# Tamnemng/TAM-GCN

Measured on AMD Instinct MI355X. Metric: skeleton clips/sec (fwd+CE+bwd+grad all-reduce+SGD step), N-UCLA 20-joint x 64-frame, higher is better.
Workload: dtype f32 (exact fp32-input MFMA v_mfma_f32_16x16x4_f32 in every GEMM, forward and backward: the reference's arithmetic); 1 GPU; N-UCLA joint stream, 256 clips/GPU x (3,64,20,1), models.ctrgcn.Model fwd+CE+bwd+grad-allreduce+SGD step, train-mode BN; global_batch=256, streams=1, parallelism=dp1, launch=hipgraph, model_streams=0, rehearsal=False, allreduce=one flat bucket after backward

## Files before the change

include/tamgcn.h:

```cpp
#ifndef TAMGCN_H
#define TAMGCN_H

#ifdef __cplusplus
extern "C" {
#endif

#define TAMGCN_VERSION 401
#define TAMGCN_MAX_SUBSETS 3
#define TAMGCN_MAX_V 32

typedef struct tamgcn_src {
    const float* x1;
    const float* x2;
    const float* coef;
    int ctot;
    int coff;
    int act;
} tamgcn_src;

int         tamgcn_version(void);
const char* tamgcn_last_error(void);
const char* tamgcn_last_kernel(void);
int         tamgcn_get_split_mode(void);
int         tamgcn_set_split_mode(int mode);

int         tamgcn_ctrgc_lds_bytes(int S, int V, int R);

typedef struct tamgcn_conv_desc {
    tamgcn_src src;
    int N, K, T_in, V;
    const float* w;
    const float* bias;
    int M, KT, dil, stride, pad;
    int wmode;
    int up;
    float* y;
    int yctot, ycoff;
    int T_out;
    int T_y;
    int ostride;
    const float* add1;
    const float* add2;
    const float* bcast;
    float bcast_scale;
    const tamgcn_src* mask;
    const float* aux;
    const float* aux_center;
    int auxctot, auxcoff;
    float* stats_part;
    int stats_ctot, stats_coff;
    const float* post_coef;
    int post_ctot, post_act;
} tamgcn_conv_desc;

int tamgcn_conv_nparts(const tamgcn_conv_desc* d);
int tamgcn_conv(const tamgcn_conv_desc* d, void* stream);

typedef struct tamgcn_wgrad_desc {
    tamgcn_src gy;
    tamgcn_src src;
    int N, M, K, T_in, T_out, V, KT, dil, stride, pad;
    float* part;
    int nsplit;
} tamgcn_wgrad_desc;
int tamgcn_wgrad_max_split(const tamgcn_wgrad_desc* d);
int tamgcn_wgrad(const tamgcn_wgrad_desc* d, void* stream);

typedef struct tamgcn_conv_pair_desc {
    int N, T, V;
    int stride;
    tamgcn_src src;
    int K, M0, M1;
    const float* w0; const float* w1;
    const float* bias0; const float* bias1;
    float* y0; int yctot0, ycoff0;
    float* y1; int yctot1, ycoff1;
    float* stats_part0; int stats_ctot0, stats_coff0;
    float* stats_part1; int stats_ctot1, stats_coff1;
} tamgcn_conv_pair_desc;
int tamgcn_conv_pair(const tamgcn_conv_pair_desc* d, void* stream);

typedef struct tamgcn_wgrad_pair_desc {
    tamgcn_src gy0, gy1, src;
    int N, M0, M1, K, T, V;
    int stride;
    float* part;
    int nsplit;
} tamgcn_wgrad_pair_desc;
int tamgcn_wgrad_pair(const tamgcn_wgrad_pair_desc* d, void* stream);

typedef struct tamgcn_reduce_desc {
    const float* part; float* out;
    int nsplit, accumulate;
    long long stride_s, count;
    float scale;
} tamgcn_reduce_desc;
int tamgcn_reduce_multi(const tamgcn_reduce_desc* descs, int n, void* stream);

int tamgcn_reduce_sum(float* part, int nsplit, long long stride_s, long long count,
                      float scale, int accumulate, float* out, void* stream);

int tamgcn_bn_fwd_finalize(const float* part, int part_ctot, int part_coff, int nparts, double count,
                           const float* gamma, const float* beta,
                           float* running_mean, float* running_var, long long* num_batches_tracked,
                           float momentum, float eps, int training,
                           float* coef, float* save, int coef_ctot, int coef_coff, int C, void* stream);

int tamgcn_coef_diff(const float* coef_d, const float* coef_y, float* out, int C, int mode, void* stream);

int tamgcn_bn_bwd_finalize(const float* part, int part_ctot, int part_coff, int nparts, double count,
// ... 17 lines not shown

int tamgcn_tmean(const tamgcn_src* src, int N, int C, int T, int V, float* xbar, void* stream);

typedef struct tamgcn_ctrgc_desc {
    int N, Cin, Cout, S, R, T, V;
    tamgcn_src x;
    const float* pq;
    const float* w3;
    const float* b3;
    const float* w4;
    const float* b4;
    const float* A;
    const float* alpha;
    const float* E;
} tamgcn_ctrgc_desc;

int tamgcn_ctrgc_build_e(const tamgcn_ctrgc_desc* d, float* E, void* stream);

int tamgcn_ctrgc_fwd(const tamgcn_ctrgc_desc* d, float* y, float* stats_part, float* x3_out, void* stream);

int tamgcn_ctrgc_bwd_dx3(const tamgcn_ctrgc_desc* d, const tamgcn_src* dy,
                         float* dx3, float* db3_part, void* stream);

int tamgcn_ctrgc_bwd_de_acc(const tamgcn_ctrgc_desc* d, const tamgcn_src* dy, const float* x3,
                            float* dE, void* stream);
int tamgcn_ctrgc_bwd_de_tail(const tamgcn_ctrgc_desc* d, const float* dE,
                             float* dA_part, float* dw4_part, float* db4_part,
                             float* dalpha_part, float* dpq, int groups, void* stream);

int tamgcn_ctrgc_tiled_supported(int V);
int tamgcn_ctrgc_tiled_chunks(int V);
int tamgcn_ctrgc_tiled_build_e(const tamgcn_ctrgc_desc* d, float* E, void* stream);
int tamgcn_ctrgc_tiled_agg_fwd(const tamgcn_ctrgc_desc* d, const float* x3, const float* E, float* y, float* stats_part, void* stream);
int tamgcn_ctrgc_tiled_agg_bwd(const tamgcn_ctrgc_desc* d, const tamgcn_src* dy, const float* E, float* dx3, float* db3_part, void* stream);
int tamgcn_ctrgc_tiled_de_acc(const tamgcn_ctrgc_desc* d, const tamgcn_src* dy, const float* x3, float* dE, void* stream);
int tamgcn_ctrgc_tiled_de_tail(const tamgcn_ctrgc_desc* d, const float* dE, float* dA_part, float* dw4_part, float* db4_part,
                               float* dalpha_part, float* dpq, void* stream);

int tamgcn_vgen_supported(int V);
int tamgcn_vgen_lds_bytes(int S, int V, int R);
int tamgcn_vgen_build_e(const tamgcn_ctrgc_desc* d, float* E, void* stream);
int tamgcn_vgen_agg_fwd(const tamgcn_ctrgc_desc* d, const float* x3, const float* E, float* y, float* stats_part, void* stream);
int tamgcn_vgen_agg_bwd(const tamgcn_ctrgc_desc* d, const tamgcn_src* dy, const float* E, float* dx3, float* db3_part, void* stream);
int tamgcn_vgen_de_acc(const tamgcn_ctrgc_desc* d, const tamgcn_src* dy, const float* x3, float* dE, void* stream);
int tamgcn_vgen_de_tail(const tamgcn_ctrgc_desc* d, const float* dE, float* dA_part, float* dw4_part, float* db4_part,
                        float* dalpha_part, float* dpq, int groups, void* stream);

int tamgcn_ew_nparts(int N, int C, int T, int V);

int tamgcn_gcn_tail_fwd(const tamgcn_src* y, const tamgcn_src* o, const tamgcn_src* res,
                        int N, int C, int T, int V, float* g, void* stream);
int tamgcn_gcn_tail_bwd(const float* dg, const float* g, const tamgcn_src* o, const float* o_save,
                        int N, int C, int T, int V, float* dsum, float* doz, float* part, void* stream);
int tamgcn_gcn_mid_bwd(const float* dsum, const float* ddiff, const float* y_pre, const float* y_save,
                       const float* r_pre, const float* r_save,
                       int N, int C, int T, int V, float* dyb, float* dres, float* part, void* stream);

#define TAMGCN_TCONV_MAXB 6
typedef struct tamgcn_tconv_desc {
    tamgcn_src src;
    int N, T_in, T_out, V, Cb, nb, KT, stride, pool;
    int dil[TAMGCN_TCONV_MAXB];
    const float* w[TAMGCN_TCONV_MAXB];
    const float* bias[TAMGCN_TCONV_MAXB];
    float* y; int yctot, ycoff;
    float* stats_part; int stats_ctot;
    const tamgcn_src* mask; const float* center;
} tamgcn_tconv_desc;
int tamgcn_tconv_supported(int V, int Cb, int KT, int nb, const int* dil, int stride, int T_in);
int tamgcn_tconv_nparts(const tamgcn_tconv_desc* d, int backward);
int tamgcn_tconv_fwd(const tamgcn_tconv_desc* d, void* stream);
int tamgcn_tconv_bwd(const tamgcn_tconv_desc* d, void* stream);
int tamgcn_tconv_wgrad_max_split(const tamgcn_tconv_desc* d);
int tamgcn_tconv_wgrad(const tamgcn_tconv_desc* d, void* stream);

int tamgcn_maxpool_fwd(const tamgcn_src* src, int N, int C, int T_in, int V, int stride,
                       float* y, int yctot, int ycoff, int T_out, float* stats_part, void* stream);
int tamgcn_maxpool_post_fwd(const tamgcn_src* src, int N, int C, int T_in, int V, int stride,
                            float* y, int yctot, int ycoff, int T_out, const float* coef, const float* add, int relu, void* stream);
int tamgcn_maxpool_bwd(const tamgcn_src* gy, const tamgcn_src* src, const float* src_save, int N, int C, int T_in, int T_out, int V,
                       int stride, float* d, int dctot, int dcoff, float* part, void* stream);

int tamgcn_add_act_fwd(const tamgcn_src* a, const tamgcn_src* res, int relu,
                       int N, int C, int T, int V, float* out, float* rowmean, float* xbar, void* stream);
int tamgcn_add_act_bwd(const float* dout, const float* out, int relu, const float* a_pre, const float* a_save,
                       const float* r_pre, const float* r_save,
                       int N, int C, int T, int V, float* dz, float* part, void* stream);

int tamgcn_apply(const tamgcn_src* src, int N, int C, int T, int V, float* y, int yctot, int ycoff, void* stream);

int tamgcn_stem_stats(const float* x, const float* dout, const float* center, int N, int C, int T, int V, int M,
                      float* part, void* stream);
int tamgcn_stem_apply(const float* x, const float* dout, const float* coef, int N, int C, int T, int V, int M,
                      float* out, void* stream);
int tamgcn_head_pool_fwd(const float* x, int N, int C, int T, int V, int M, float* pooled, void* stream);
int tamgcn_head_pool_bwd(const float* dpooled, int N, int C, int T, int V, int M, float* dx, void* stream);
int tamgcn_head_fc_fwd(const float* pooled, const float* W, const float* b, int N, int C, int K, float* logits, void* stream);
int tamgcn_head_fc_bwd(const float* dlogits, const float* pooled, const float* W, int N, int C, int K,
                       float* dW, float* db, float* dpooled, void* stream);

int tamgcn_ce_fwd(const float* logits, const long long* labels, int N, int K, float* loss, float* g, void* stream);
int tamgcn_ce_bwd(const float* g, const float* dloss, int N, int K, float* dlogits, void* stream);

int tamgcn_score_fuse(const float* scores, const float* weights, int S, int N, int K, int softmax,
                      const long long* labels, float* fused, long long* pred, int* class_stats, void* stream);

#define TAMGCN_EVAL_MAX_TOPK 4
#define TAMGCN_SWEEP_MAX_ALPHAS 16
int tamgcn_eval_accumulate(const float* logits, const long long* labels, const long long* index, int B, int K,
                           int valid, const int* valid_dev, const int* topk, int nk, long long base, long long num_samples,
                           long long* counts, double* sums, int* confusion, float* scores, void* stream);
int tamgcn_score_sweep(const float* a, const float* b, const float* alphas, int A, int N, int K, int softmax,
                       const long long* labels, int* correct, void* stream);

int tamgcn_stream_derive(const float* x, int N, int C, int T, int V, int M, const int* parent, int mode, float* out, void* stream);
int tamgcn_feeder_transform(const double* raw, const long long* offsets, const double* rot, const int* idx, const int* parent,
                            int N, int V, int time_steps, int center_joint, int mode, float* out, void* stream);

int tamgcn_feeder_draw(const long long* offsets, long long n_clips, const long long* clip_ids, int B, const long long* labels,
                       long long* state, const double* cossin, int time_steps, int train, double* view, double* rot, int* idx,
                       long long* labels_out, void* stream);
int tamgcn_feeder_transform_indexed(const double* raw, const long long* offsets, long long n_clips, const long long* clip_ids,
                                    const double* rot, const int* idx, const int* parent, int B, int V, int time_steps,
                                    int center_joint, int mode, float* out, void* stream);

typedef struct tamgcn_f2_gcn_desc {
    int N, Cin, Cout, T, V, S, R, res_mode;
    const float* x;
    const float* w12; const float* b12;
    const float* w4; const float* b4;
    const float* A; const float* alpha;
    const float* w3; const float* b3;
    const float* sy; const float* ty;
    const float* wd; const float* bd;
    float* E;
    float* sum; float* diff;
    const float* xpart;
} tamgcn_f2_gcn_desc;
int tamgcn_f2_e(const tamgcn_f2_gcn_desc* d, void* stream);
int tamgcn_f2_gcn(const tamgcn_f2_gcn_desc* d, void* stream);
// ... 101 lines not shown
```

tam_gcn_amd/_lib.py:

```python
import ctypes as C
import os

_HERE = os.path.dirname(os.path.abspath(__file__))
LIB_PATH = os.path.join(_HERE, 'libtamgcn.so')

c_float_p = C.c_void_p


class Src(C.Structure):
    _fields_ = [('x1', C.c_void_p), ('x2', C.c_void_p), ('coef', C.c_void_p),
                ('ctot', C.c_int), ('coff', C.c_int), ('act', C.c_int)]


class ConvDesc(C.Structure):
    _fields_ = [('src', Src),
                ('N', C.c_int), ('K', C.c_int), ('T_in', C.c_int), ('V', C.c_int),
                ('w', C.c_void_p), ('bias', C.c_void_p),
                ('M', C.c_int), ('KT', C.c_int), ('dil', C.c_int), ('stride', C.c_int), ('pad', C.c_int),
                ('wmode', C.c_int), ('up', C.c_int),
                ('y', C.c_void_p), ('yctot', C.c_int), ('ycoff', C.c_int),
                ('T_out', C.c_int), ('T_y', C.c_int), ('ostride', C.c_int),
                ('add1', C.c_void_p), ('add2', C.c_void_p), ('bcast', C.c_void_p), ('bcast_scale', C.c_float),
                ('mask', C.POINTER(Src)),
                ('aux', C.c_void_p), ('aux_center', C.c_void_p), ('auxctot', C.c_int), ('auxcoff', C.c_int),
# ... 79 lines not shown
class F2TcnDesc(C.Structure):
    _fields_ = [(k, C.c_int) for k in ('N', 'Cin', 'Cout', 'T', 'V', 'stride', 'Cb', 'nb', 'ks', 'res_mode')] + \
               [('dil', C.c_int * 4), ('h', C.c_void_p), ('wt', C.c_void_p * 4), ('bt', C.c_void_p * 4)] + \
               [(k, C.c_void_p) for k in ('sp', 'tp', 'x', 'wr', 'br', 'out', 'xpart')]


class F2sGcnDesc(C.Structure):
    _fields_ = [(k, C.c_int) for k in ('N', 'Cin', 'Cout', 'T', 'V', 'K')] + \
               [(k, C.c_void_p) for k in ('x', 'Ae', 'wg', 'bg', 'h')]


class F2sTcnDesc(C.Structure):
    _fields_ = [(k, C.c_int) for k in ('N', 'Cin', 'Cout', 'T', 'V', 'KT', 'stride', 'res_mode')] + \
               [(k, C.c_void_p) for k in ('h', 'wt', 'bt', 'x', 'wr', 'br', 'out')]


class F2sTcnBwdDesc(C.Structure):
    _fields_ = [(k, C.c_int) for k in ('N', 'Cout', 'T', 'V', 'KT', 'stride')] + \
               [(k, C.c_void_p) for k in ('gout', 'out', 'h', 'wtb', 'dh')]


class F2sGcnBwdDesc(C.Structure):
    _fields_ = [(k, C.c_int) for k in ('N', 'Cin', 'Cout', 'T', 'V', 'K', 'stride', 'res_mode')] + \
               [(k, C.c_void_p) for k in ('dh', 'Ae', 'wgb', 'gout', 'out', 'wrb', 'dx')]


class OptimDesc(C.Structure):
    _fields_ = [('n', C.c_longlong),
                ('p', C.c_void_p), ('g', C.c_void_p), ('s0', C.c_void_p), ('s1', C.c_void_p),
                ('lr', C.c_void_p), ('step', C.c_void_p), ('scal', C.c_void_p),
                ('mode', C.c_int), ('nesterov', C.c_int),
                ('momentum', C.c_float), ('dampening', C.c_float), ('weight_decay', C.c_float), ('eps', C.c_float),
                ('beta1', C.c_double), ('beta2', C.c_double)]


class GradGuard(C.Structure):
    _fields_ = [('max_norm', C.c_float), ('skip_nonfinite', C.c_int), ('partial', C.c_void_p), ('n_partial', C.c_int),
                ('stat', C.c_void_p), ('skipped', C.c_void_p)]


_i, _p, _d, _f, _ll = C.c_int, C.c_void_p, C.c_double, C.c_float, C.c_longlong
_SP = C.POINTER(Src)
SIGNATURES = {
    'tamgcn_version': (_i, []),
    'tamgcn_last_error': (C.c_char_p, []),
    'tamgcn_last_kernel': (C.c_char_p, []),
    'tamgcn_ctrgc_lds_bytes': (_i, [_i, _i, _i]),
    'tamgcn_get_split_mode': (_i, []),
    'tamgcn_set_split_mode': (_i, [_i]),
    'tamgcn_conv_nparts': (_i, [C.POINTER(ConvDesc)]),
    'tamgcn_conv': (_i, [C.POINTER(ConvDesc), _p]),
    'tamgcn_wgrad_max_split': (_i, [C.POINTER(WgradDesc)]),
    'tamgcn_wgrad': (_i, [C.POINTER(WgradDesc), _p]),
    'tamgcn_conv_pair': (_i, [C.POINTER(ConvPairDesc), _p]),
    'tamgcn_wgrad_pair': (_i, [C.POINTER(WgradPairDesc), _p]),
    'tamgcn_stem_stats': (_i, [_p, _p, _p, _i, _i, _i, _i, _i, _p, _p]),
    'tamgcn_stem_apply': (_i, [_p, _p, _p, _i, _i, _i, _i, _i, _p, _p]),
    'tamgcn_head_pool_fwd': (_i, [_p, _i, _i, _i, _i, _i, _p, _p]),
    'tamgcn_head_pool_bwd': (_i, [_p, _i, _i, _i, _i, _i, _p, _p]),
    'tamgcn_head_fc_fwd': (_i, [_p, _p, _p, _i, _i, _i, _p, _p]),
    'tamgcn_head_fc_bwd': (_i, [_p, _p, _p, _i, _i, _i, _p, _p, _p, _p]),
    'tamgcn_reduce_multi': (_i, [C.POINTER(ReduceDesc), _i, _p]),
    'tamgcn_reduce_sum': (_i, [_p, _i, _ll, _ll, _f, _i, _p, _p]),
    'tamgcn_bn_fwd_finalize': (_i, [_p, _i, _i, _i, _d, _p, _p, _p, _p, _p, _f, _f, _i, _p, _p, _i, _i, _i, _p]),
    'tamgcn_bn_bwd_finalize': (_i, [_p, _i, _i, _i, _d, _p, _p, _i, _i, _i, _p, _p, _p, _p, _i, _i, _i, _p]),
    'tamgcn_bn_fwd_finalize_multi': (_i, [C.POINTER(BnFwdDesc), _i, _p]),
    'tamgcn_coef_diff': (_i, [_p, _p, _p, _i, _i, _p]),
    'tamgcn_bn_bwd_finalize_multi': (_i, [C.POINTER(BnBwdDesc), _i, _p]),
    'tamgcn_tmean': (_i, [_SP, _i, _i, _i, _i, _p, _p]),
    'tamgcn_ctrgc_build_e': (_i, [C.POINTER(CtrgcDesc), _p, _p]),
    'tamgcn_ctrgc_fwd': (_i, [C.POINTER(CtrgcDesc), _p, _p, _p, _p]),
    'tamgcn_ctrgc_bwd_dx3': (_i, [C.POINTER(CtrgcDesc), _SP, _p, _p, _p]),
    'tamgcn_ctrgc_bwd_de_acc': (_i, [C.POINTER(CtrgcDesc), _SP, _p, _p, _p]),
    'tamgcn_ctrgc_bwd_de_tail': (_i, [C.POINTER(CtrgcDesc), _p, _p, _p, _p, _p, _p, _i, _p]),
    'tamgcn_ctrgc_tiled_supported': (_i, [_i]),
    'tamgcn_ctrgc_tiled_chunks': (_i, [_i]),
    'tamgcn_ctrgc_tiled_build_e': (_i, [C.POINTER(CtrgcDesc), _p, _p]),
    'tamgcn_ctrgc_tiled_agg_fwd': (_i, [C.POINTER(CtrgcDesc), _p, _p, _p, _p, _p]),
    'tamgcn_ctrgc_tiled_agg_bwd': (_i, [C.POINTER(CtrgcDesc), _SP, _p, _p, _p, _p]),
    'tamgcn_ctrgc_tiled_de_acc': (_i, [C.POINTER(CtrgcDesc), _SP, _p, _p, _p]),
    'tamgcn_ctrgc_tiled_de_tail': (_i, [C.POINTER(CtrgcDesc), _p, _p, _p, _p, _p, _p, _p]),
    'tamgcn_vgen_supported': (_i, [_i]),
    'tamgcn_vgen_lds_bytes': (_i, [_i, _i, _i]),
    'tamgcn_vgen_build_e': (_i, [C.POINTER(CtrgcDesc), _p, _p]),
    'tamgcn_vgen_agg_fwd': (_i, [C.POINTER(CtrgcDesc), _p, _p, _p, _p, _p]),
    'tamgcn_vgen_agg_bwd': (_i, [C.POINTER(CtrgcDesc), _SP, _p, _p, _p, _p]),
    'tamgcn_vgen_de_acc': (_i, [C.POINTER(CtrgcDesc), _SP, _p, _p, _p]),
    'tamgcn_vgen_de_tail': (_i, [C.POINTER(CtrgcDesc), _p, _p, _p, _p, _p, _p, _i, _p]),
    'tamgcn_ew_nparts': (_i, [_i, _i, _i, _i]),
    'tamgcn_gcn_tail_fwd': (_i, [_SP, _SP, _SP, _i, _i, _i, _i, _p, _p]),
    'tamgcn_gcn_tail_bwd': (_i, [_p, _p, _SP, _p, _i, _i, _i, _i, _p, _p, _p, _p]),
    'tamgcn_gcn_mid_bwd': (_i, [_p, _p, _p, _p, _p, _p, _i, _i, _i, _i, _p, _p, _p, _p]),
    'tamgcn_tconv_supported': (_i, [_i, _i, _i, _i, C.POINTER(C.c_int), _i, _i]),
    'tamgcn_tconv_nparts': (_i, [C.POINTER(TconvDesc), _i]),
    'tamgcn_tconv_fwd': (_i, [C.POINTER(TconvDesc), _p]),
    'tamgcn_tconv_bwd': (_i, [C.POINTER(TconvDesc), _p]),
    'tamgcn_tconv_wgrad_max_split': (_i, [C.POINTER(TconvDesc)]),
    'tamgcn_tconv_wgrad': (_i, [C.POINTER(TconvDesc), _p]),
    'tamgcn_maxpool_fwd': (_i, [_SP, _i, _i, _i, _i, _i, _p, _i, _i, _i, _p, _p]),
    'tamgcn_maxpool_post_fwd': (_i, [_SP, _i, _i, _i, _i, _i, _p, _i, _i, _i, _p, _p, _i, _p]),
    'tamgcn_maxpool_bwd': (_i, [_SP, _SP, _p, _i, _i, _i, _i, _i, _i, _p, _i, _i, _p, _p]),
    'tamgcn_add_act_fwd': (_i, [_SP, _SP, _i, _i, _i, _i, _i, _p, _p, _p, _p]),
    'tamgcn_add_act_bwd': (_i, [_p, _p, _i, _p, _p, _p, _p, _i, _i, _i, _i, _p, _p, _p]),
    'tamgcn_apply': (_i, [_SP, _i, _i, _i, _i, _p, _i, _i, _p]),
    'tamgcn_score_fuse': (_i, [_p, _p, _i, _i, _i, _i, _p, _p, _p, _p, _p]),
    'tamgcn_ce_fwd': (_i, [_p, _p, _i, _i, _p, _p, _p]),
    'tamgcn_ce_bwd': (_i, [_p, _p, _i, _i, _p, _p]),
    'tamgcn_eval_accumulate': (_i, [_p, _p, _p, _i, _i, _i, _p, C.POINTER(C.c_int), _i, _ll, _ll, _p, _p, _p, _p, _p]),
    'tamgcn_score_sweep': (_i, [_p, _p, C.POINTER(C.c_float), _i, _i, _i, _i, _p, _p, _p]),
    'tamgcn_stream_derive': (_i, [_p, _i, _i, _i, _i, _i, _p, _i, _p, _p]),
    'tamgcn_feeder_transform': (_i, [_p, _p, _p, _p, _p, _i, _i, _i, _i, _i, _p, _p]),
    'tamgcn_feeder_draw': (_i, [_p, _ll, _p, _i, _p, _p, _p, _i, _i, _p, _p, _p, _p, _p]),
    'tamgcn_feeder_transform_indexed': (_i, [_p, _p, _ll, _p, _p, _p, _p, _i, _i, _i, _i, _i, _p, _p]),
    'tamgcn_f2_e': (_i, [C.POINTER(F2GcnDesc), _p]),
    'tamgcn_f2_gcn': (_i, [C.POINTER(F2GcnDesc), _p]),
    'tamgcn_f2_gemm': (_i, [C.POINTER(F2GemmDesc), _p]),
    'tamgcn_f2_tcn': (_i, [C.POINTER(F2TcnDesc), _p]),
    'tamgcn_f2v_e': (_i, [C.POINTER(F2GcnDesc), _p]),
    'tamgcn_f2v_gcn': (_i, [C.POINTER(F2GcnDesc), _p]),
    'tamgcn_f2v_gemm': (_i, [C.POINTER(F2GemmDesc), _p]),
    'tamgcn_f2v_tcn': (_i, [C.POINTER(F2TcnDesc), _p]),
    'tamgcn_f2_e_grouped': (_i, [C.POINTER(F2GcnDesc), _i, _p]),
    'tamgcn_f2_gcn_grouped': (_i, [C.POINTER(F2GcnDesc), _i, _p]),
    'tamgcn_f2_gemm_grouped': (_i, [C.POINTER(F2GemmDesc), _i, _p]),
    'tamgcn_f2_tcn_grouped': (_i, [C.POINTER(F2TcnDesc), _i, _p]),
    'tamgcn_f2v_e_grouped': (_i, [C.POINTER(F2GcnDesc), _i, _p]),
    'tamgcn_f2v_gcn_grouped': (_i, [C.POINTER(F2GcnDesc), _i, _p]),
    'tamgcn_f2v_gemm_grouped': (_i, [C.POINTER(F2GemmDesc), _i, _p]),
    'tamgcn_f2v_tcn_grouped': (_i, [C.POINTER(F2TcnDesc), _i, _p]),
    'tamgcn_f2s_supported': (_i, [_i, _i, _i, _i, _i, _i]),
    'tamgcn_f2s_gcn': (_i, [C.POINTER(F2sGcnDesc), _p]),
    'tamgcn_f2s_tcn': (_i, [C.POINTER(F2sTcnDesc), _p]),
    'tamgcn_f2s_tcn_bwd': (_i, [C.POINTER(F2sTcnBwdDesc), _p]),
    'tamgcn_f2s_gcn_bwd': (_i, [C.POINTER(F2sGcnBwdDesc), _p]),
    'tamgcn_saliency_joints': (_i, [_p, _p, _i, _i, _i, _i, _i, _p, _p, _p]),
    'tamgcn_saliency_accumulate': (_i, [_p, _p, _i, _i, _p, _p, _i, _i, _i, _p, _p, _p]),
    'tamgcn_stem_streams_eval': (_i, [_p, _p, _p, _p, _i, _i, _i, _i, _i, _i, _p, _p]),
    'tamgcn_head_fc_grouped': (_i, [_p, _p, _p, _i, _i, _i, _i, _p, _p]),
    'tamgcn_optim_step': (_i, [C.POINTER(OptimDesc), _p]),
    'tamgcn_optim_step_guarded': (_i, [C.POINTER(OptimDesc), C.POINTER(GradGuard), _p]),
}


class TamgcnLibraryError(RuntimeError):
    pass


_lib = None
ABI_VERSION = 401


def load():
    global _lib
    if _lib is not None:
        return _lib
    import torch
# ... 27 lines not shown
```

tam_gcn_amd/csrc/conv.hip:

```cpp
#include "common.h"

namespace {

constexpr int BM = 64;
constexpr int BK = 16;
constexpr int BKP = BK + 1;
constexpr int MAXCW = 5;
constexpr int MAXCOLS = 320;

TG_TRACE_DEFINE(tamgcn_trace_read)

struct ConvArgs {
    SrcDev src;
    int N, K, T_in, V;
    const float* w; const float* bias;
    int M, KT, dil, stride, pad;
    long long ws_m, ws_k, ws_t, w_off;
    int up, wmode;
    float* y; int yctot, ycoff, T_out, T_y, ostride;
    const float* add1; const float* add2; const float* bcast; float bcast_scale;
    SrcDev mask; int has_mask;
    const float* aux; const float* aux_center; int auxctot, auxcoff;
    float* stats_part; int stats_ctot, stats_coff, nparts;
    const float* post_coef; int post_ctot, post_act;
    int BT;
    int CW;
    int TIN;
    int lstride;
    int sB;
    int LB;
    int pitchB;
    int Vs, Vp, nsl;
};

struct PairArgs {
    int M0;
    const float* w1; const float* bias1;
    float* y1; int yctot1, ycoff1;
    float* stats1; int sctot1, scoff1;
};

__device__ __forceinline__ void conv_epilogue(const ConvArgs& a, f32x4 (&acc)[4][MAXCW], float* Ss, int n, int m0, int t0,
                                              int ncols, int cw0, int mt_act, int c_act, const int (&tl)[MAXCW],
                                              const int (&vv)[MAXCW], int j, int kq, int wave, int tid) {
    const int V = a.V;
    float s1[4][4], s2[4][4];
#pragma unroll
    for (int mt = 0; mt < 4; ++mt)
#pragma unroll
        for (int r = 0; r < 4; ++r) { s1[mt][r] = 0.f; s2[mt][r] = 0.f; }
#pragma unroll
    for (int mt = 0; mt < 4; ++mt) {
        if (mt >= mt_act) continue;
#pragma unroll
        for (int c = 0; c < MAXCW; ++c) {
            if (c >= c_act) continue;
            int col = (cw0 + c) * 16 + j;
            if (col >= ncols) continue;
            int t = (t0 + tl[c]) * a.ostride;
#pragma unroll
            for (int r = 0; r < 4; ++r) {
                int m = m0 + mt * 16 + kq * 4 + r;
                if (m >= a.M) continue;
                float val = acc[mt][c][r];
                if (a.bias) val += a.bias[m];
                if (a.post_coef) val = fmaf(a.post_coef[a.ycoff + m], val, a.post_coef[2 * a.post_ctot + a.ycoff + m]);
                long long idx = (((long long)n * a.yctot + a.ycoff + m) * a.T_y + t) * V + vv[c];
                if (a.bcast) val = fmaf(a.bcast[((long long)m * a.N + n) * V + vv[c]], a.bcast_scale, val);
                if (a.add1) val += a.add1[idx];
                if (a.add2) val += a.add2[idx];
                if (a.post_act == 1) val = fmaxf(val, 0.f);
                if (a.has_mask) {
                    int mch = a.mask.coff + m;
                    long long midx = (((long long)n * a.mask.ctot + mch) * a.T_y + t) * V + vv[c];
                    if (!(src_value(a.mask, midx, mch) > 0.f)) val = 0.f;
                }
                acc[mt][c][r] = val;
                if (a.stats_part) {
                    float x2 = val;
                    if (a.aux) x2 = a.aux[(((long long)n * a.auxctot + a.auxcoff + m) * a.T_y + t) * V + vv[c]] - a.aux_center[a.auxcoff + m];
                    s1[mt][r] += val;
                    s2[mt][r] = fmaf(val, x2, s2[mt][r]);
                }
            }
        }
    }
#pragma unroll
    for (int mt = 0; mt < 4; ++mt) {
        if (mt >= mt_act) continue;
#pragma unroll
        for (int c = 0; c < MAXCW; ++c) {
            if (c >= c_act) continue;
            int col = (cw0 + c) * 16 + j;
// ... 76 lines not shown
            int kk = e & (BK - 1);
            int i = (e >> 4) & (BM - 1);
            int tap = e >> 10;
            int m = m0 + i, k = k0 + kk;
            float wv = 0.f;
            if (m < a.M && k < a.K) wv = a.w[m * a.ws_m + k * a.ws_k + tap * a.ws_t + a.w_off];
            As[(tap * BM + i) * BKP + kk] = wv;
        }
        for (int pos = tid; pos < a.LB; pos += NTHREADS) {
            int slot = pos / V;
            int v = pos - slot * V;
            int th = tin0 + slot * a.lstride;
            bool ok = th >= 0;
            if (a.up > 1) { ok = ok && (th % a.up == 0); th /= a.up; }
            ok = ok && th < a.T_in;
            long long goff = src_n + (long long)th * V + v;
#pragma unroll 4
            for (int kk = 0; kk < BK; ++kk) {
                int k = k0 + kk;
                float xv = 0.f;
                if (ok && k < a.K) {
                    int ch = a.src.coff + k;
                    xv = src_value(a.src, goff + ch * chan_stride, ch);
                }
                Bs[kk * a.pitchB + pos] = xv;
            }
        }
        __syncthreads();
        for (int tap = 0; tap < a.KT; ++tap) {
            const int tapoff = tap * a.dil * V;
#pragma unroll
            for (int k4 = 0; k4 < BK / 4; ++k4) {
                float av[4];
#pragma unroll
                for (int mt = 0; mt < 4; ++mt)
                    av[mt] = As[(tap * BM + mt * 16 + j) * BKP + k4 * 4 + kq];
                const float* brow = Bs + (k4 * 4 + kq) * a.pitchB + tapoff;
#pragma unroll
                for (int c = 0; c < MAXCW; ++c) {
                    if (c < c_act) {
                        float bv = brow[boff[c]];
#pragma unroll
                        for (int mt = 0; mt < 4; ++mt)
                            if (mt < mt_act) acc[mt][c] = mfma16(av[mt], bv, acc[mt][c]);
                    }
                }
            }
        }
    }

    conv_epilogue(a, acc, Ss, n, m0, t0, ncols, cw0, mt_act, c_act, tl, vv, j, kq, wave, tid);
}

template <int NTH, bool PR = false>
__device__ __forceinline__ void staged_rows(const ConvArgs& a, const float* Tt, int PT, int RP, int r0, int BMT, int m0, int n, int t0,
                                            int ncols, float* Ss, int Vs, int v0, const PairArgs* pa = nullptr) {
    const int tid = threadIdx.x, V = a.V;
    const int TPR = NTH / RP;
    const int row = tid / TPR, seg = tid - row * TPR;
    const int m = m0 + r0 + row;
    const bool flat = Vs == V && a.ostride == 1;
    const bool vecok = flat || (Vs & 3) == 0;
    float p1 = 0.f, p2 = 0.f;
    const bool rowok = r0 + row < BMT && m < a.M;
    if (rowok) {
        float bia = a.bias ? a.bias[m] : 0.f;
        float* yp = a.y;
        const float ctr = a.aux ? a.aux_center[a.auxcoff + m] : 0.f;
        const float pc1 = a.post_coef ? a.post_coef[a.ycoff + m] : 1.f, pc0 = a.post_coef ? a.post_coef[2 * a.post_ctot + a.ycoff + m] : 0.f;
        const float plo = a.post_act == 1 ? 0.f : -__builtin_inff();
        long long ybase = ((long long)n * a.yctot + a.ycoff + m) * a.T_y * V;
        if constexpr (PR) {
            if (m >= pa->M0) {
                const int m1 = m - pa->M0;
                bia = pa->bias1 ? pa->bias1[m1] : 0.f; yp = pa->y1;
                ybase = ((long long)n * pa->yctot1 + pa->ycoff1 + m1) * a.T_y * V;
            }
        }
        const long long mbase = a.has_mask ? ((long long)n * a.mask.ctot + a.mask.coff + m) * a.T_y * V : 0;
        const long long abase = a.aux ? ((long long)n * a.auxctot + a.auxcoff + m) * a.T_y * V : 0;
        const float* bc = a.bcast ? a.bcast + ((long long)m * a.N + n) * V : nullptr;
        float mc1 = 1.f, mc2 = 0.f, mc0 = 0.f;
        if (a.has_mask && a.mask.coef) {
            int mch = a.mask.coff + m;
            mc1 = a.mask.coef[mch]; mc0 = a.mask.coef[2 * a.mask.ctot + mch];
            if (a.mask.x2) mc2 = a.mask.coef[a.mask.ctot + mch];
        }
        const int nc4 = (ncols + 3) >> 2;
        for (int c4 = seg; c4 < nc4; c4 += TPR) {
            const int col = c4 << 2;
            const int fr = col / Vs, v = col - fr * Vs;
            if ((vecok || v + 4 <= Vs) && col + 4 <= ncols) {
                const long long off = (long long)(t0 + fr) * a.ostride * V + v0 + v;
                float4 val = *reinterpret_cast<const float4*>(Tt + row * PT + col);
                val.x = fmaf(pc1, val.x + bia, pc0); val.y = fmaf(pc1, val.y + bia, pc0);
                val.z = fmaf(pc1, val.z + bia, pc0); val.w = fmaf(pc1, val.w + bia, pc0);
                if (bc) {
                    float4 b;
                    if ((V & 3) == 0) b = *reinterpret_cast<const float4*>(bc + v0 + v);
                    else { const int j0 = (v0 + v) % V; b = make_float4(bc[j0], bc[(j0 + 1) % V], bc[(j0 + 2) % V], bc[(j0 + 3) % V]); }
                    val.x = fmaf(b.x, a.bcast_scale, val.x); val.y = fmaf(b.y, a.bcast_scale, val.y);
                    val.z = fmaf(b.z, a.bcast_scale, val.z); val.w = fmaf(b.w, a.bcast_scale, val.w);
                }
                if (a.add1) { float4 t = *reinterpret_cast<const float4*>(a.add1 + ybase + off); val.x += t.x; val.y += t.y; val.z += t.z; val.w += t.w; }
                if (a.add2) { float4 t = *reinterpret_cast<const float4*>(a.add2 + ybase + off); val.x += t.x; val.y += t.y; val.z += t.z; val.w += t.w; }
                val.x = fmaxf(val.x, plo); val.y = fmaxf(val.y, plo); val.z = fmaxf(val.z, plo); val.w = fmaxf(val.w, plo);
                if (a.has_mask) {
                    float4 q = *reinterpret_cast<const float4*>(a.mask.x1 + mbase + off);
                    float4 q2 = make_float4(0.f, 0.f, 0.f, 0.f);
                    if (a.mask.x2) q2 = *reinterpret_cast<const float4*>(a.mask.x2 + mbase + off);
                    if (!(fmaf(mc1, q.x, fmaf(mc2, q2.x, mc0)) > 0.f)) val.x = 0.f;
                    if (!(fmaf(mc1, q.y, fmaf(mc2, q2.y, mc0)) > 0.f)) val.y = 0.f;
                    if (!(fmaf(mc1, q.z, fmaf(mc2, q2.z, mc0)) > 0.f)) val.z = 0.f;
                    if (!(fmaf(mc1, q.w, fmaf(mc2, q2.w, mc0)) > 0.f)) val.w = 0.f;
                }
                if (a.stats_part) {
                    float4 x2 = val;
                    if (a.aux) {
                        x2 = *reinterpret_cast<const float4*>(a.aux + abase + off);
                        x2.x -= ctr; x2.y -= ctr; x2.z -= ctr; x2.w -= ctr;
                    }
                    p1 += (val.x + val.y) + (val.z + val.w);
                    p2 = fmaf(val.x, x2.x, fmaf(val.y, x2.y, fmaf(val.z, x2.z, fmaf(val.w, x2.w, p2))));
                }
                *reinterpret_cast<float4*>(yp + ybase + off) = val;
            } else {
                for (int i = 0; i < 4 && col + i < ncols; ++i) {
                    const int ci = col + i, fi = ci / Vs, vi = ci - fi * Vs;
                    const long long off = (long long)(t0 + fi) * a.ostride * V + v0 + vi;
                    float val = fmaf(pc1, Tt[row * PT + ci] + bia, pc0);
                    if (bc) val = fmaf(bc[(v0 + vi) % V], a.bcast_scale, val);
                    if (a.add1) val += a.add1[ybase + off];
                    if (a.add2) val += a.add2[ybase + off];
                    val = fmaxf(val, plo);
                    if (a.has_mask) {
                        const float q = a.mask.x1[mbase + off], q2 = a.mask.x2 ? a.mask.x2[mbase + off] : 0.f;
                        if (!(fmaf(mc1, q, fmaf(mc2, q2, mc0)) > 0.f)) val = 0.f;
                    }
                    if (a.stats_part) {
                        const float x2 = a.aux ? a.aux[abase + off] - ctr : val;
                        p1 += val;
                        p2 = fmaf(val, x2, p2);
                    }
                    yp[ybase + off] = val;
                }
            }
        }
    }
    if (a.stats_part) {
        for (int o = 1; o < TPR; o <<= 1) { p1 += __shfl_xor(p1, o); p2 += __shfl_xor(p2, o); }
        if (seg == 0 && rowok) { Ss[r0 + row] = p1; Ss[4 * BM + r0 + row] = p2; }
    }
}

template <int BKV, int MT, int CWT>
__global__ __launch_bounds__(NTHREADS) void conv_kernel_vec(const ConvArgs a) {
    extern __shared__ __attribute__((aligned(16))) float smem[];
    constexpr int BKVP = BKV + 2;
    constexpr int BMT = MT * 16;
    constexpr int NPF = (BKV == 32) ? 10 : 8;
    float* As = smem;
    float* Bs = As + ((a.KT * BMT * BKVP + 3) & ~3);
    float* Ss = Bs + BKV * a.pitchB;
    float* cf = Ss + 2 * 4 * BM;

    const int tid = threadIdx.x, lane = tid & 63, wave = tid >> 6;
    const int j = lane & 15, kq = lane >> 4;
    const int tti = blockIdx.x / a.nsl, sl = blockIdx.x - tti * a.nsl;
    const int n = blockIdx.z, m0 = blockIdx.y * BMT, t0 = tti * a.BT;
    const int V = a.V, Vs = a.Vs, Vp = a.Vp, v0 = sl * Vs;
    const int bt = min(a.BT, a.T_out - t0);
    const int ncols = bt * Vs;
    const int cw0 = wave * CWT;

    for (int e = tid; e < a.K; e += NTHREADS) {
        int ch = a.src.coff + e;
        cf[e] = a.src.coef ? a.src.coef[ch] : 1.f;
        cf[a.K + e] = (a.src.coef && a.src.x2) ? a.src.coef[a.src.ctot + ch] : 0.f;
        cf[2 * a.K + e] = a.src.coef ? a.src.coef[2 * a.src.ctot + ch] : 0.f;
    }

    int boff[CWT], tl[CWT], vv[CWT];
#pragma unroll
    for (int c = 0; c < CWT; ++c) {
        int col = (cw0 + c) * 16 + j;
        if (col < ncols) { tl[c] = col / Vs; vv[c] = col - tl[c] * Vs; boff[c] = tl[c] * a.sB * Vp + vv[c]; }
        else { tl[c] = 0; vv[c] = 0; boff[c] = 0; }
    }
    f32x4 acc[MT][CWT];
#pragma unroll
    for (int mt = 0; mt < MT; ++mt)
// ... 134 lines not shown
            }
        }
        TG_T(tf); TG_ACC(6, tf - te);
    }
    TG_T(tg0);

    __syncthreads();
    float* Tt = smem;
    constexpr int PT = CWT * 64 + 4;
    const int avail = ((a.KT * BMT * BKVP + 3) & ~3) + BKV * a.pitchB;
    int RP = (avail / PT) & ~15;
    if (RP > BMT) RP = BMT;
    if (RP == 48) RP = 32;
    if (a.stats_part) {
        for (int e = tid; e < 2 * 4 * BM; e += NTHREADS) Ss[e] = 0.f;
    }
    for (int r0 = 0; r0 < BMT; r0 += RP) {
        __syncthreads();
#pragma unroll
        for (int mt = 0; mt < MT; ++mt) {
            const int rl = mt * 16 + kq * 4 - r0;
            if (rl >= 0 && rl < RP) {
#pragma unroll
                for (int c = 0; c < CWT; ++c) {
                    const int col = (cw0 + c) * 16 + j;
#pragma unroll
                    for (int r = 0; r < 4; ++r) Tt[(rl + r) * PT + col] = acc[mt][c][r];
                }
            }
        }
        __syncthreads();
        staged_rows<NTHREADS>(a, Tt, PT, RP, r0, BMT, m0, n, t0, ncols, Ss, Vs, v0);
    }
    if (a.stats_part) {
        __syncthreads();
        if (tid < 2 * BMT) {
            int st = tid / BMT, row = tid - st * BMT;
            int m = m0 + row;
            if (m < a.M) {
                int part = n * gridDim.x + blockIdx.x;
                a.stats_part[((long long)st * a.stats_ctot + a.stats_coff + m) * a.nparts + part] = Ss[st * 4 * BM + row];
            }
        }
    }
}



#ifndef TG_KO
#define TG_KO 0
#endif
constexpr int G_NT = 512, G_BMT = 64, G_PA = 80, G_PBMAX = 320, G_NST = 3, G_CWT = 5;

template <int NSRC, int BK, bool PRO, int NW, int PAIR = 0>
__global__ __launch_bounds__(NW * 64, NW == 8 ? 4 : 2) void conv1x1_glds_kernel(const ConvArgs a, int ntt, int nmt, const PairArgs pa) {
    constexpr int G_NT = NW * 64, G_MT = 16 / NW;
    extern __shared__ __attribute__((aligned(16))) float smem[];
    constexpr int STG = BK * G_PBMAX * NSRC + BK * G_PA;
    constexpr int NAI = BK / NW;
    constexpr int MAXB = (NSRC * (BK / 4) * 5 + NW - 1) / NW;
    float* cf = smem + G_NST * STG;
    float* Ss = cf + (PRO ? 3 * a.K : 0);

    const int tid = threadIdx.x, lane = tid & 63, wave = tid >> 6;
    const int j = lane & 15, kq = lane >> 4, wm = wave >> 2, wn = wave & 3;
    const int V = a.V, K = a.K, LB = a.LB;
    const int rot = ((LB & 31) + 16) & 31;
    int g, mtile;
    {
        const int L = blockIdx.x, ng = a.N * ntt;
        if ((ng & 7) == 0) { const int xcd = L & 7, i = L >> 3; mtile = i % nmt; g = (i / nmt) * 8 + xcd; }
        else { g = L / nmt; mtile = L - g * nmt; }
    }
    const int n = g / ntt, tt = g - n * ntt;
    const int m0 = mtile * G_BMT, t0 = tt * a.BT;
    const int bt = min(a.BT, a.T_out - t0);
    const int ncols = bt * V;
    const long long TV = (long long)a.T_in * V;

    const int NQ = (LB + 63) >> 6;
    const int ls = a.lstride;
    const float rV_ = 1.0f / (float)V;
    const int NI1 = (BK / 4) * NQ;
    int b_rel[MAXB], b_dst[MAXB];
    bool b_ok[MAXB], b_on[MAXB];
    int nissue = 0;
#pragma unroll
    for (int i = 0; i < MAXB; ++i) {
        const int id = wave + i * NW;
        const bool idok = id < NSRC * NI1;
        const int src = idok ? id / NI1 : 0;
        const int rem = id - src * NI1;
        const int grp = rem / NQ, q = rem - grp * NQ;
        const int f = q * 256 + lane * 4;
        const int r = f / LB, off = f - r * LB;
        int col = off + (r & 1) * rot;
        if (col >= LB) col -= LB;
        b_ok[i] = idok && r < 4 && col < ncols;
        const int scol = ls > 1 ? col + tg_rcp_div(col, rV_) * (ls - 1) * V : col;
        b_rel[i] = (int)((grp * 4 + r) * TV) + scol + src * 0x40000000;
        b_dst[i] = src * (BK * G_PBMAX) + grp * 4 * LB + q * 256;
        b_on[i] = __ballot(b_ok[i]) != 0ull;
        nissue += b_on[i] ? 1 : 0;
    }
    const float* xb1 = a.src.x1 + ((long long)n * a.src.ctot + a.src.coff) * TV + (long long)t0 * ls * V;
    const float* xb2 = NSRC == 2 ? a.src.x2 + ((long long)n * a.src.ctot + a.src.coff) * TV + (long long)t0 * ls * V : nullptr;
    constexpr int RPP = 256 / BK;
    constexpr int NAP0 = G_BMT / RPP;
// ... 169 lines not shown
        for (int s_ = 0; s_ + 1 < NK; ++s_) {
            rd((s_ & 1) ^ 1, stg, k0, s_ + 1);
            mm(s_ & 1);
            fin((s_ & 1) ^ 1);
        }
        tg_wait_vmcnt<15>(c + 2 < nch ? nissue : 0);
        asm volatile("s_waitcnt lgkmcnt(0)\n\ts_barrier" ::: "memory");
        if (c + 3 < nch) issue(c + 3);
        stg = stg == G_NST - 1 ? 0 : stg + 1;
        rd(NK & 1, stg, k0 + BK, 0);
        mm((NK - 1) & 1);
        fin(NK & 1);
    }
    {
        const int k0 = (nch - 1) * BK;
#pragma unroll
        for (int s_ = 0; s_ < NK; ++s_) {
            if (s_ + 1 < NK) rd((s_ & 1) ^ 1, stg, k0, s_ + 1);
            mm(s_ & 1);
            if (s_ + 1 < NK) fin((s_ & 1) ^ 1);
        }
    }
    TG_T(tg0);

#if TG_KO & 1
    {
        float ssum = 0.f;
        for (int mt = 0; mt < G_MT; ++mt)
            for (int c = 0; c < G_CWT; ++c) ssum += acc[mt][c][0] + acc[mt][c][1] + acc[mt][c][2] + acc[mt][c][3];
        if (ssum == 123.456f) a.y[tid] = ssum;
        return;
    }
#endif
    constexpr int PT = G_CWT * 64 + 4, RP = 32;
    float* Tt = smem;
    if (a.stats_part) {
        for (int e = tid; e < 2 * 4 * BM; e += G_NT) Ss[e] = 0.f;
    }
    for (int r0 = 0; r0 < G_BMT; r0 += RP) {
        __syncthreads();
#pragma unroll
        for (int mt = 0; mt < G_MT; ++mt) {
            const int rl = wm * (G_MT * 16) + mt * 16 - r0;
            if (rl >= 0 && rl < RP) {
#pragma unroll
                for (int c = 0; c < G_CWT; ++c) {
                    const int col = (wn * G_CWT + c) * 16 + j;
#pragma unroll
                    for (int r = 0; r < 4; ++r) Tt[(rl + kq * 4 + r) * PT + col] = acc[mt][c][r];
                }
            }
        }
        __syncthreads();
        staged_rows<G_NT, PAIR == 1>(a, Tt, PT, RP, r0, G_BMT, m0, n, t0, ncols, Ss, V, 0, &pa);
    }
    if (a.stats_part) {
        __syncthreads();
        if (tid < 2 * G_BMT) {
            int stt = tid / G_BMT, row = tid - stt * G_BMT;
            int m = m0 + row;
            if (PAIR == 1 && m < a.M && m >= pa.M0) pa.stats1[((long long)stt * pa.sctot1 + pa.scoff1 + m - pa.M0) * a.nparts + g] = Ss[stt * 4 * BM + row];
            else if (m < a.M) a.stats_part[((long long)stt * a.stats_ctot + a.stats_coff + m) * a.nparts + g] = Ss[stt * 4 * BM + row];
        }
    }
    TG_T(tg1); TG_ACC(7, tg1 - tg0); TG_ACC(8, tg1 - tt0); TG_ACC(9, 1);
}


constexpr int GS_BK = 32, GS_NST = 2;

template <int TERMS, bool WM0, int MT>
__global__ __launch_bounds__(G_NT) void conv1x1_glds_split_kernel(const ConvArgs a, int ntt, int nmt) {
    constexpr int GS_MT = MT, GS_BMT = 32 * MT, WROWS = 16 * MT;
    extern __shared__ __attribute__((aligned(16))) float smem[];
    constexpr int BK = GS_BK;
    constexpr int STG = BK * G_PBMAX + BK * GS_BMT;
    constexpr int MAXB = ((BK / 4) * 5 + 7) / 8;
    constexpr int NAP = BK * GS_BMT / 256 / 8;
    constexpr int QR = GS_BMT / 4, RPP = 64 / QR;
    float* cf = smem + GS_NST * STG;
    float* Ss = cf + 3 * a.K;
    float* Bc = Ss + 2 * 4 * BM;

    TG_T(tt0);
    const int tid = threadIdx.x, lane = tid & 63, wave = tid >> 6;
    const int j = lane & 15, kq = lane >> 4, wm = wave >> 2, wn = wave & 3;
    const int V = a.V, K = a.K, LB = a.LB;
    const int rot = ((LB & 31) + 16) & 31;
    int g, mtile;
    {
        const int L = blockIdx.x, ng = a.N * ntt;
        if ((ng & 7) == 0) { const int xcd = L & 7, i = L >> 3; mtile = i % nmt; g = (i / nmt) * 8 + xcd; }
        else { g = L / nmt; mtile = L - g * nmt; }
    }
    const int n = g / ntt, tt = g - n * ntt;
    const int m0 = mtile * GS_BMT, t0 = tt * a.BT;
    const int bt = min(a.BT, a.T_out - t0);
    const int ncols = bt * V;
    const long long TV = (long long)a.T_in * V;

    for (int e = tid; e < K; e += G_NT) {
        int ch = a.src.coff + e;
        cf[e] = a.src.coef ? a.src.coef[ch] : 1.f;
        cf[K + e] = (a.src.coef && a.src.x2) ? a.src.coef[a.src.ctot + ch] : 0.f;
        cf[2 * K + e] = a.src.coef ? a.src.coef[2 * a.src.ctot + ch] : 0.f;
    }
    const bool plain = !a.src.coef;
    const int nsrc = a.src.x2 ? 2 : 1;

    const int NQ = (LB + 63) >> 6, NI1 = (BK / 4) * NQ;
    int b_rel[MAXB], b_dst[MAXB];
    bool b_ok[MAXB], b_on[MAXB];
    int nissue = 0;
#pragma unroll
    for (int i = 0; i < MAXB; ++i) {
// ... 191 lines not shown
    const int q = 4 / gcd_i(V, 4);
    if (p->flat && q > 1 && BT >= q) BT -= BT % q;
    for (;;) {
        p->BT = BT;
        p->lstride = (d->KT == 1) ? d->stride : 1;
        p->sB = (d->KT == 1) ? 1 : d->stride;
        p->TIN = (d->KT == 1) ? BT : (BT - 1) * d->stride + (d->KT - 1) * d->dil + 1;
        p->LB = p->TIN * p->Vp;
        int pitch = p->LB;
        pitch += ((16 - (pitch & 31)) + 32) & 31;
        p->pitchB = pitch;
        p->CW = ceil_div(ceil_div(BT * p->Vs, 16), 4);
        p->vec = false; p->bk = BK;
        bool slots_short = false;
        if (vec_try && (p->LB & 3) == 0) {
            int lb4 = p->LB / 4;
            int bk = (d->KT == 1 && 32 * lb4 <= 10 * NTHREADS) ? 32 : 16;
            if (bk * lb4 <= ((bk == 32) ? 10 : 8) * NTHREADS) { p->vec = true; p->bk = bk; }
            else slots_short = true;
        }
        p->mt = d->M <= 16 ? 1 : d->M <= 32 ? 2 : (d->M % 64 == 0 ? 4 : (d->M % 48 == 0 ? 3 : 4));
        if (d->KT > 1 && p->mt == 4) p->mt = 2;
        p->cwt = p->CW <= 3 ? 3 : 5;
        if (p->vec) {
            size_t avail = (((size_t)d->KT * p->mt * 16 * (p->bk + 2) + 3) & ~(size_t)3) + (size_t)p->bk * pitch;
            if (avail < (size_t)16 * (p->cwt * 64 + 4)) p->vec = false;
        }
        p->lds = p->vec ? sizeof(float) * ((((size_t)d->KT * p->mt * 16 * (p->bk + 2) + 3) & ~(size_t)3) + (size_t)p->bk * pitch +
                                           2 * 4 * BM + 3 * (size_t)d->K)
                        : sizeof(float) * ((size_t)d->KT * BM * (BK + 1) + (size_t)BK * pitch + 2 * 4 * BM);
        if (slots_short && BT > 1) { BT = BT > 4 ? BT - 2 : BT - 1; if (p->flat && q > 1 && BT >= q) BT -= BT % q; continue; }
        if (p->lds <= 64 * 1024 || BT == 1) break;
        BT = (BT + 1) / 2;
        if (p->flat && q > 1 && BT >= q) BT -= BT % q;
    }
    if (!p->vec) { p->Vs = V; p->nsl = 1; if (p->Vp != V) {
        p->Vp = V; p->LB = p->TIN * V; int pitch = p->LB; pitch += ((16 - (pitch & 31)) + 32) & 31; p->pitchB = pitch;
        p->CW = ceil_div(ceil_div(p->BT * V, 16), 4);
        p->lds = sizeof(float) * ((size_t)d->KT * BM * (BK + 1) + (size_t)BK * pitch + 2 * 4 * BM); } }
    if (p->lds > 160 * 1024 || p->CW > MAXCW) return -1;
    p->ntt = ceil_div(d->T_out, p->BT);
    return 0;
}

}


extern "C" int tamgcn_conv_nparts(const tamgcn_conv_desc* d) {
    ConvPlan p;
    if (!d || plan_conv(d, &p)) return -1;
    return d->N * p.ntt * p.nsl;
}

extern "C" int tamgcn_conv(const tamgcn_conv_desc* d, void* stream) {
    TG_CHECK(d && d->src.x1 && d->w && d->y, "tamgcn_conv: null pointer");
    TG_CHECK(d->N > 0 && d->K > 0 && d->M > 0 && d->T_in > 0 && d->T_out > 0 && d->V > 0,
             "tamgcn_conv: bad dims N=%d K=%d M=%d T_in=%d T_out=%d V=%d", d->N, d->K, d->M, d->T_in, d->T_out, d->V);
    TG_CHECK(d->KT >= 1 && d->KT <= 9 && d->dil >= 1 && d->stride >= 1 && d->up >= 1 && d->ostride >= 1,
             "tamgcn_conv: bad taps KT=%d dil=%d stride=%d up=%d", d->KT, d->dil, d->stride, d->up);
    TG_CHECK(d->src.coff + d->K <= d->src.ctot && d->ycoff + d->M <= d->yctot, "tamgcn_conv: channel slice out of range");
    TG_CHECK((d->T_out - 1) * d->ostride < d->T_y, "tamgcn_conv: T_out*ostride exceeds T_y");
    TG_CHECK(!(d->N > 65535), "tamgcn_conv: N too large for grid.z");
    TG_CHECK((long long)d->N * d->yctot * d->T_y * d->V < (1LL << 32), "tamgcn_conv: output tensor exceeds 2^32 elements");
    ConvPlan p;
    TG_CHECK(plan_conv(d, &p) == 0, "tamgcn_conv: no tiling for V=%d KT=%d dil=%d stride=%d", d->V, d->KT, d->dil, d->stride);
    ConvArgs a;
    a.src = make_src(d->src);
    a.N = d->N; a.K = d->K; a.T_in = d->T_in; a.V = d->V;
    a.w = d->w; a.bias = d->bias; a.M = d->M; a.KT = d->KT; a.dil = d->dil; a.stride = d->stride; a.pad = d->pad;
    if (d->wmode == 0) { a.ws_m = (long long)d->K * d->KT; a.ws_k = d->KT; a.ws_t = 1; a.w_off = 0; }
    else { a.ws_m = d->KT; a.ws_k = (long long)d->M * d->KT; a.ws_t = -1; a.w_off = d->KT - 1; }
    a.up = d->up; a.wmode = d->wmode;
    a.y = d->y; a.yctot = d->yctot; a.ycoff = d->ycoff; a.T_out = d->T_out; a.T_y = d->T_y; a.ostride = d->ostride;
    a.add1 = d->add1; a.add2 = d->add2; a.bcast = d->bcast; a.bcast_scale = d->bcast_scale;
    a.has_mask = d->mask != nullptr; a.mask = d->mask ? make_src(*d->mask) : null_src();
    a.aux = d->aux; a.aux_center = d->aux_center; a.auxctot = d->auxctot; a.auxcoff = d->auxcoff;
    TG_CHECK(!d->aux || d->aux_center, "tamgcn_conv: aux needs aux_center");
    a.stats_part = d->stats_part; a.stats_ctot = d->stats_ctot; a.stats_coff = d->stats_coff;
    a.post_coef = d->post_coef; a.post_ctot = d->post_ctot; a.post_act = d->post_act;
    TG_CHECK(!d->post_coef || d->post_ctot >= d->ycoff + d->M, "tamgcn_conv: post_coef has %d channels, need %d", d->post_ctot, d->ycoff + d->M);
    a.nparts = d->N * p.ntt * p.nsl;
    a.BT = p.BT; a.CW = p.CW; a.TIN = p.TIN; a.lstride = p.lstride; a.sB = p.sB; a.LB = p.LB; a.pitchB = p.pitchB;
    a.Vs = p.Vs; a.Vp = p.Vp; a.nsl = p.nsl;
    dim3 grid(p.ntt, ceil_div(d->M, BM), d->N);
    const bool aligned16 = (((uintptr_t)d->src.x1 | (uintptr_t)(d->src.x2 ? d->src.x2 : d->src.x1) | (uintptr_t)d->w) & 15) == 0;
    const bool strided1x1 = d->KT == 1 && d->stride == 2 && d->up == 1 && d->pad == 0 && (d->V & 3) == 0 && d->T_out == (d->T_in - 1) / 2 + 1 &&
                            p.lstride == 2 && p.TIN == p.BT && p.nsl == 1 && p.Vp == d->V && !d->mask && !d->aux;
    const bool glds = p.vec && (p.flat || strided1x1) && d->K % 16 == 0 && p.LB >= 64 && p.LB <= G_PBMAX && (p.LB & 3) == 0 &&
                      aligned16 && (long long)d->K * d->T_in * d->V < (1LL << 30);
    const size_t lds_split = sizeof(float) * ((size_t)GS_NST * (GS_BK * G_PBMAX + GS_BK * 128) + 3 * (size_t)d->K + 2 * 4 * BM + 128);
    const bool big = glds && tamgcn_split_mode() >= 1 && d->src.act == 0 && d->M >= 128 && d->M % 4 == 0 && d->K % GS_BK == 0 &&
                     lds_split <= 160 * 1024 && !d->post_coef && d->wmode == 1 && !d->stats_part;
    if (big) {
        const int nmt = ceil_div(d->M, 128);
        const unsigned nblk = (unsigned)(d->N * p.ntt * nmt);
        tg_launch_lds<conv1x1_glds_split_kernel<2, false, 4>>(160 * 1024, dim3(nblk), dim3(G_NT), lds_split, (hipStream_t)stream, a, p.ntt, nmt);
        tamgcn_note_kernel("conv1x1_glds_split_kernel<2, false, 4>");
    } else if (glds) {
        const int nmt = ceil_div(d->M, G_BMT);
        const unsigned nblk = (unsigned)(d->N * p.ntt * nmt);
        static int nw_env = -1;
        if (nw_env < 0) { const char* e = getenv("TAMGCN_CONV_WAVES"); nw_env = e ? atoi(e) : 8; }
        const bool pro = d->src.coef || d->src.x2 || d->src.act;
#define TG_GLDS_CASE(NS_, BK_, PRO_, NW_)                                                                                 \
        {                                                                                                                   \
            tg_launch_lds<conv1x1_glds_kernel<NS_, BK_, PRO_, NW_>>(160 * 1024, dim3(nblk), dim3(NW_ * 64), glds_lds_bytes<NS_, BK_>(d->K, PRO_), \
                                                                    (hipStream_t)stream, a, p.ntt, nmt, PairArgs{});        \
            tamgcn_note_kernel("conv1x1_glds_kernel<%d, %d, %s, %d>", NS_, BK_, PRO_ ? "true" : "false", NW_);              \
        }
        if (nw_env != 4) {
            if (d->src.x2) TG_GLDS_CASE(2, 8, true, 8) else if (pro) TG_GLDS_CASE(1, 16, true, 8) else TG_GLDS_CASE(1, 16, false, 8)
        } else {
            if (d->src.x2) TG_GLDS_CASE(2, 8, true, 4) else if (pro) TG_GLDS_CASE(1, 16, true, 4) else TG_GLDS_CASE(1, 16, false, 4)
        }
#undef TG_GLDS_CASE
    } else if (p.vec) {
        dim3 gridv(p.ntt * p.nsl, ceil_div(d->M, 16 * p.mt), d->N);
#define TG_CONV_CASE(BKV_, MT_, CW_)                                                                              \
        if (p.bk == BKV_ && p.mt == MT_ && p.cwt == CW_) {                                                         \
            tg_launch_lds<conv_kernel_vec<BKV_, MT_, CW_>>(160 * 1024, gridv, dim3(NTHREADS), p.lds, (hipStream_t)stream, a); \
            tamgcn_note_kernel("conv_kernel_vec<%d, %d, %d>", BKV_, MT_, CW_);                                      \
        } else
        TG_CONV_CASE(32, 4, 5) TG_CONV_CASE(32, 3, 5) TG_CONV_CASE(32, 2, 5) TG_CONV_CASE(32, 1, 5)
        TG_CONV_CASE(32, 4, 3) TG_CONV_CASE(32, 3, 3) TG_CONV_CASE(32, 2, 3) TG_CONV_CASE(32, 1, 3)
        TG_CONV_CASE(16, 4, 5) TG_CONV_CASE(16, 3, 5) TG_CONV_CASE(16, 2, 5) TG_CONV_CASE(16, 1, 5)
        TG_CONV_CASE(16, 4, 3) TG_CONV_CASE(16, 3, 3) TG_CONV_CASE(16, 2, 3) TG_CONV_CASE(16, 1, 3)
        { tamgcn_set_error("tamgcn_conv: no instantiation bk=%d mt=%d cw=%d", p.bk, p.mt, p.cwt); return -1; }
#undef TG_CONV_CASE
    } else {
        tg_launch_lds<conv_kernel>(160 * 1024, grid, dim3(NTHREADS), p.lds, (hipStream_t)stream, a);
        tamgcn_note_kernel("conv_kernel");
    }
    TG_LAUNCH_CHECK("tamgcn_conv");
    return 0;
}


extern "C" int tamgcn_conv_pair(const tamgcn_conv_pair_desc* d, void* stream) {
    TG_CHECK(d, "tamgcn_conv_pair: null descriptor");
    TG_CHECK(d->src.x1 && d->w0 && d->w1 && d->y0 && d->y1, "tamgcn_conv_pair: null pointer");
    TG_CHECK(d->N > 0 && d->T > 0 && d->V > 0 && d->K > 0 && d->M0 > 0 && d->M1 >= 0,
             "tamgcn_conv_pair: bad dims N=%d T=%d V=%d K=%d M0=%d M1=%d", d->N, d->T, d->V, d->K, d->M0, d->M1);
    TG_CHECK(d->M1 > 0, "tamgcn_conv_pair: M1 = 0: nothing to pair (use tamgcn_conv)");
    TG_CHECK(d->stride == 1, "tamgcn_conv_pair: stride %d: only stride-1 1x1 convolutions pair up", d->stride);
    const bool two = d->src.x2 != nullptr;
    const int bk = two ? 8 : 16;
    TG_CHECK(d->K % 16 == 0, "tamgcn_conv_pair: K=%d is not a multiple of the chunk (%d rows; the kernel takes whole 16)", d->K, bk);
    TG_CHECK(d->src.coff >= 0 && d->src.coff + d->K <= d->src.ctot, "tamgcn_conv_pair: source channel slice out of range");
    TG_CHECK(d->ycoff0 >= 0 && d->ycoff0 + d->M0 <= d->yctot0 && d->ycoff1 >= 0 && d->ycoff1 + d->M1 <= d->yctot1,
             "tamgcn_conv_pair: destination slice out of range");
    TG_CHECK((d->stats_part0 != nullptr) == (d->stats_part1 != nullptr), "tamgcn_conv_pair: moments go with both parts or with neither");
    if (d->stats_part0) TG_CHECK(d->stats_coff0 >= 0 && d->stats_coff0 + d->M0 <= d->stats_ctot0 && d->stats_coff1 >= 0 && d->stats_coff1 + d->M1 <= d->stats_ctot1,
                                 "tamgcn_conv_pair: moment slice out of range");
    const int yct = d->yctot0 > d->yctot1 ? d->yctot0 : d->yctot1;
    TG_CHECK((long long)d->N * yct * d->T * d->V < (1LL << 32), "tamgcn_conv_pair: output tensor exceeds 2^32 elements");
    const int K = d->K, M = d->M0 + d->M1;
    tamgcn_conv_desc cd = {};
    cd.src = d->src; cd.N = d->N; cd.K = K; cd.T_in = d->T; cd.V = d->V; cd.w = d->w0; cd.M = M; cd.KT = 1; cd.dil = 1; cd.stride = 1;
    cd.wmode = 0; cd.up = 1; cd.y = d->y0; cd.yctot = d->yctot0; cd.T_out = d->T; cd.T_y = d->T; cd.ostride = 1;
    ConvPlan p;
    TG_CHECK(plan_conv(&cd, &p) == 0, "tamgcn_conv_pair: no tiling for V=%d", d->V);
    const uintptr_t al = (uintptr_t)d->src.x1 | (uintptr_t)(two ? d->src.x2 : d->src.x1) | (uintptr_t)d->w0 | (uintptr_t)d->w1;
    const bool glds = p.vec && p.flat && p.LB >= 64 && p.LB <= G_PBMAX && (p.LB & 3) == 0 && (al & 15) == 0 && K <= 1024 &&
                      (long long)K * d->T * d->V < (1LL << 30);
    TG_CHECK(glds, "tamgcn_conv_pair: V=%d T=%d K=%d is not a shape of the LDS-DMA GEMM (or an operand is not 16-byte aligned)", d->V, d->T, K);
    ConvArgs a = {};
    a.src = make_src(d->src);
    a.N = d->N; a.K = K; a.T_in = d->T; a.V = d->V;
    a.w = d->w0; a.bias = d->bias0; a.M = M; a.KT = 1; a.dil = 1; a.stride = 1; a.pad = 0;
    a.ws_m = K; a.ws_k = 1; a.ws_t = 1; a.w_off = 0;
    a.up = 1; a.wmode = 0;
    a.y = d->y0; a.yctot = d->yctot0; a.ycoff = d->ycoff0; a.T_out = d->T; a.T_y = d->T; a.ostride = 1;
    a.mask = null_src();
    a.stats_part = d->stats_part0; a.stats_ctot = d->stats_ctot0; a.stats_coff = d->stats_coff0;
    a.nparts = d->N * p.ntt * p.nsl;
    a.BT = p.BT; a.CW = p.CW; a.TIN = p.TIN; a.lstride = p.lstride; a.sB = p.sB; a.LB = p.LB; a.pitchB = p.pitchB;
    a.Vs = p.Vs; a.Vp = p.Vp; a.nsl = p.nsl;
    PairArgs pa = {};
    pa.M0 = d->M0; pa.w1 = d->w1; pa.bias1 = d->bias1;
    pa.y1 = d->y1; pa.yctot1 = d->yctot1; pa.ycoff1 = d->ycoff1;
    pa.stats1 = d->stats_part1; pa.sctot1 = d->stats_ctot1; pa.scoff1 = d->stats_coff1;
    const int nmt = ceil_div(M, G_BMT);
    const unsigned nblk = (unsigned)(d->N * p.ntt * nmt);
    const bool pro = d->src.coef || d->src.x2 || d->src.act;
#define TG_PAIR_CASE(NS_, BK_, PRO_)                                                                                      \
    {                                                                                                                   \
        tg_launch_lds<conv1x1_glds_kernel<NS_, BK_, PRO_, 8, 1>>(160 * 1024, dim3(nblk), dim3(8 * 64), glds_lds_bytes<NS_, BK_>(K, PRO_), \
// ... 9 lines not shown
```

tam_gcn_amd/csrc/elementwise.hip:

```cpp
#include "common.h"
#include <stdlib.h>

namespace {

constexpr int EW_THREADS = 256;

struct RowGeo { int tpr, rows; };
__device__ __forceinline__ bool row_coords(const RowGeo& g, int C, int& c, int& n, int& li) {
    const int rpb = EW_THREADS / g.tpr;
    const int row = blockIdx.x * rpb + threadIdx.x / g.tpr;
    li = threadIdx.x & (g.tpr - 1);
    const bool ok = row < g.rows;
    const int r = ok ? row : 0;
    n = r / C; c = r - n * C;
    return ok;
}
__device__ __forceinline__ float row_sum(float v, const RowGeo& g) {
    const int w = g.tpr < 64 ? g.tpr : 64;
    for (int o = 1; o < w; o <<= 1) v += __shfl_xor(v, o);
    if (g.tpr > 64) {
        __shared__ float red[EW_THREADS / 64];
        const int wave = threadIdx.x >> 6, wpr = g.tpr >> 6, first = wave & ~(wpr - 1);
        __syncthreads();
        if ((threadIdx.x & 63) == 0) red[wave] = v;
        __syncthreads();
        float t = red[first];
        for (int k = 1; k < wpr; ++k) t += red[first + k];
        v = t;
    }
    return v;
}
__device__ __forceinline__ void row_store_sums(const float* vals, int nst, float* part, int C, int N, int c, int n,
                                               const RowGeo& g, int li, bool ok) {
    for (int s = 0; s < nst; ++s) {
        const float v = row_sum(vals[s], g);
        if (li == 0 && ok) part[((long long)s * C + c) * N + n] = v;
    }
}

struct RowSrc {
    const float* x1; const float* x2; float c1, c2, c0; int act;
};
__device__ __forceinline__ RowSrc row_src(const SrcDev& s, long long base, int ch) {
    RowSrc r;
    r.x1 = s.x1 + base; r.x2 = s.x2 ? s.x2 + base : nullptr;
    r.c1 = s.coef ? s.coef[ch] : 1.f;
    r.c2 = (s.coef && s.x2) ? s.coef[s.ctot + ch] : 0.f;
    r.c0 = s.coef ? s.coef[2 * s.ctot + ch] : 0.f;
    r.act = s.act;
    return r;
}
__device__ __forceinline__ float row_val(const RowSrc& r, int i) {
    float v = fmaf(r.c1, r.x1[i], fmaf(r.c2, r.x2 ? r.x2[i] : 0.f, r.c0));
    return r.act == 1 ? fmaxf(v, 0.f) : v;
}
__device__ __forceinline__ float4 row_val4(const RowSrc& r, int i4) {
    float4 a = reinterpret_cast<const float4*>(r.x1)[i4];
    float4 b = r.x2 ? reinterpret_cast<const float4*>(r.x2)[i4] : make_float4(0.f, 0.f, 0.f, 0.f);
    float4 o;
    o.x = fmaf(r.c1, a.x, fmaf(r.c2, b.x, r.c0)); o.y = fmaf(r.c1, a.y, fmaf(r.c2, b.y, r.c0));
    o.z = fmaf(r.c1, a.z, fmaf(r.c2, b.z, r.c0)); o.w = fmaf(r.c1, a.w, fmaf(r.c2, b.w, r.c0));
    if (r.act == 1) { o.x = fmaxf(o.x, 0.f); o.y = fmaxf(o.y, 0.f); o.z = fmaxf(o.z, 0.f); o.w = fmaxf(o.w, 0.f); }
    return o;
}

__global__ __launch_bounds__(EW_THREADS) void gcn_tail_fwd_kernel(RowGeo geo, SrcDev y, SrcDev o, SrcDev res, int has_res,
                                                                  int C, int L, float* g) {
    int c, n, li;
    const bool rowok = row_coords(geo, C, c, n, li);
    if (!rowok) L = 0;
    const RowSrc ry = row_src(y, ((long long)n * y.ctot + y.coff + c) * L, y.coff + c);
    const RowSrc ro = row_src(o, ((long long)n * o.ctot + o.coff + c) * L, o.coff + c);
    RowSrc rr = ry;
    if (has_res) rr = row_src(res, ((long long)n * res.ctot + res.coff + c) * L, res.coff + c);
    float* gp = g + ((long long)n * C + c) * L;
    {
        for (int i = li; i < (L >> 2); i += geo.tpr) {
            float4 a = row_val4(ry, i), b = row_val4(ro, i);
            float4 r = has_res ? row_val4(rr, i) : make_float4(0.f, 0.f, 0.f, 0.f);
            float4 v;
            v.x = fmaxf(a.x + tanhf(b.x) + r.x, 0.f); v.y = fmaxf(a.y + tanhf(b.y) + r.y, 0.f);
            v.z = fmaxf(a.z + tanhf(b.z) + r.z, 0.f); v.w = fmaxf(a.w + tanhf(b.w) + r.w, 0.f);
            reinterpret_cast<float4*>(gp)[i] = v;
        }
    }
    {
        for (int i = (L & ~3) + li; i < L; i += geo.tpr) {
            float v = row_val(ry, i) + tanhf(row_val(ro, i));
            if (has_res) v += row_val(rr, i);
            gp[i] = fmaxf(v, 0.f);
        }
    }
}

__global__ __launch_bounds__(EW_THREADS) void gcn_tail_bwd_kernel(RowGeo geo, const float* dg, const float* g, SrcDev o, const float* o_save,
                                                                  int C, int L, int N, float* dsum, float* doz, float* part) {
    int c, n, li;
    const bool rowok = row_coords(geo, C, c, n, li);
    if (!rowok) L = 0;
    const long long b = ((long long)n * C + c) * L;
    const long long bo = ((long long)n * o.ctot + o.coff + c) * L;
    const RowSrc ro = row_src(o, bo, o.coff + c);
    float s[2] = {0.f, 0.f};
    const float mu = o_save[o.coff + c];
    {
        for (int i = li; i < (L >> 2); i += geo.tpr) {
            float4 gg = reinterpret_cast<const float4*>(g + b)[i], dd = reinterpret_cast<const float4*>(dg + b)[i];
            float4 ob = row_val4(ro, i), op = reinterpret_cast<const float4*>(o.x1 + bo)[i];
            float4 d, z;
            float t;
            d.x = gg.x > 0.f ? dd.x : 0.f; t = tanhf(ob.x); z.x = d.x * (1.f - t * t);
            d.y = gg.y > 0.f ? dd.y : 0.f; t = tanhf(ob.y); z.y = d.y * (1.f - t * t);
            d.z = gg.z > 0.f ? dd.z : 0.f; t = tanhf(ob.z); z.z = d.z * (1.f - t * t);
            d.w = gg.w > 0.f ? dd.w : 0.f; t = tanhf(ob.w); z.w = d.w * (1.f - t * t);
            reinterpret_cast<float4*>(dsum + b)[i] = d;
            reinterpret_cast<float4*>(doz + b)[i] = z;
            s[0] += (z.x + z.y) + (z.z + z.w);
            s[1] = fmaf(z.x, op.x - mu, fmaf(z.y, op.y - mu, fmaf(z.z, op.z - mu, fmaf(z.w, op.w - mu, s[1]))));
        }
    }
    {
        for (int i = (L & ~3) + li; i < L; i += geo.tpr) {
            float d = g[b + i] > 0.f ? dg[b + i] : 0.f;
            float off = tanhf(row_val(ro, i));
            float dz = d * (1.f - off * off);
            dsum[b + i] = d;
            doz[b + i] = dz;
            s[0] += dz;
            s[1] = fmaf(dz, o.x1[bo + i] - mu, s[1]);
        }
    }
    row_store_sums(s, 2, part, C, N, c, n, geo, li, rowok);
}

__global__ __launch_bounds__(EW_THREADS) void gcn_mid_bwd_kernel(RowGeo geo, const float* dsum, const float* ddiff, const float* y_pre, const float* y_save,
                                                                 const float* r_pre, const float* r_save, int C, int L, int N,
                                                                 float* dyb, float* dres, float* part) {
    int c, n, li;
    const bool rowok = row_coords(geo, C, c, n, li);
    if (!rowok) L = 0;
    const long long b = ((long long)n * C + c) * L;
    float s[4] = {0.f, 0.f, 0.f, 0.f};
    const float muy = y_save[c], mur = r_pre ? r_save[c] : 0.f;
    {
        for (int i = li; i < (L >> 2); i += geo.tpr) {
            float4 d = reinterpret_cast<const float4*>(dsum + b)[i], dd = reinterpret_cast<const float4*>(ddiff + b)[i];
            float4 yp = reinterpret_cast<const float4*>(y_pre + b)[i];
            float4 rp = r_pre ? reinterpret_cast<const float4*>(r_pre + b)[i] : make_float4(0.f, 0.f, 0.f, 0.f);
            float4 a = make_float4(d.x - dd.x, d.y - dd.y, d.z - dd.z, d.w - dd.w);
            float4 r = make_float4(d.x + dd.x, d.y + dd.y, d.z + dd.z, d.w + dd.w);
            reinterpret_cast<float4*>(dyb + b)[i] = a;
            if (dres) reinterpret_cast<float4*>(dres + b)[i] = r;
            s[0] += (a.x + a.y) + (a.z + a.w);
            s[1] = fmaf(a.x, yp.x - muy, fmaf(a.y, yp.y - muy, fmaf(a.z, yp.z - muy, fmaf(a.w, yp.w - muy, s[1]))));
            if (r_pre) {
                s[2] += (r.x + r.y) + (r.z + r.w);
                s[3] = fmaf(r.x, rp.x - mur, fmaf(r.y, rp.y - mur, fmaf(r.z, rp.z - mur, fmaf(r.w, rp.w - mur, s[3]))));
            }
        }
    }
    {
        for (int i = (L & ~3) + li; i < L; i += geo.tpr) {
            float d = dsum[b + i], dd = ddiff[b + i];
            float a = d - dd, r = d + dd;
            dyb[b + i] = a;
            s[0] += a;
            s[1] = fmaf(a, y_pre[b + i] - muy, s[1]);
            if (dres) dres[b + i] = r;
            if (r_pre) { s[2] += r; s[3] = fmaf(r, r_pre[b + i] - mur, s[3]); }
        }
    }
    row_store_sums(s, r_pre ? 4 : 2, part, C, N, c, n, geo, li, rowok);
}

__global__ __launch_bounds__(EW_THREADS) void maxpool_fwd_kernel(RowGeo geo, SrcDev src, int C, int T_in, int V, int stride,
                                                                 float* y, int yctot, int ycoff, int T_out, int N, float* part) {
    int c, n, li;
    const bool rowok = row_coords(geo, C, c, n, li);
    if (!rowok) T_out = 0;
    const long long bs = ((long long)n * src.ctot + src.coff + c) * T_in * V;
    float* yp = y + ((long long)n * yctot + ycoff + c) * T_out * V;
    float s[2] = {0.f, 0.f};
    for (int i = li; i < T_out * V; i += geo.tpr) {
        int t = i / V, v = i - t * V;
        float best = -INFINITY;
// ... 170 lines not shown
    auto ld4 = [&](const float* base, int start, float (&o)[4]) {
        if (start >= 0 && start + 4 <= L) {
            const float4 t = *reinterpret_cast<const float4*>(base + start);
            o[0] = t.x; o[1] = t.y; o[2] = t.z; o[3] = t.w;
        } else {
#pragma unroll
            for (int e = 0; e < 4; ++e) o[e] = (start + e >= 0 && start + e < L) ? base[start + e] : 0.f;
        }
    };
    float s[2] = {0.f, 0.f};
    for (int g = li; g < ngrp; g += geo.tpr) {
        const int p = g << 2;
        float xr[5][4], ga[3][4], gb[3][4];
#pragma unroll
        for (int k = 0; k < 5; ++k) ld4(sp, p + (k - 2) * V, xr[k]);
#pragma unroll
        for (int w = 0; w < 3; ++w) { ld4(g1p, p + (w - 1) * V, ga[w]); ld4(g2p, p + (w - 1) * V, gb[w]); }
        float xa[5][4];
#pragma unroll
        for (int k = 0; k < 5; ++k)
#pragma unroll
            for (int e = 0; e < 4; ++e) {
                const int q = p + e + (k - 2) * V;
                float val = fmaf(sc1, xr[k][e], sc0);
                if (src.act == 1) val = fmaxf(val, 0.f);
                xa[k][e] = (q >= 0 && q < L) ? val : -INFINITY;
            }
        float o[4] = {0.f, 0.f, 0.f, 0.f};
#pragma unroll
        for (int w = 0; w < 3; ++w)
#pragma unroll
            for (int e = 0; e < 4; ++e) {
                const int q = p + e + (w - 1) * V;
                const float x0 = xa[2][e];
                bool win;
                if (w == 0) win = xa[0][e] < x0 && xa[1][e] < x0;
                else if (w == 1) win = xa[1][e] < x0 && !(xa[3][e] > x0);
                else win = !(xa[3][e] > x0) && !(xa[4][e] > x0);
                if (q >= 0 && q < L && win && x0 > 0.f) o[e] += fmaf(gc1, ga[w][e], fmaf(gc2, gb[w][e], gc0));
            }
        if (p + 4 <= L) *reinterpret_cast<float4*>(dp + p) = make_float4(o[0], o[1], o[2], o[3]);
#pragma unroll
        for (int e = 0; e < 4; ++e)
            if (p + e < L) {
                if (p + 4 > L) dp[p + e] = o[e];
                s[0] += o[e];
                s[1] = fmaf(o[e], xr[2][e] - mu, s[1]);
            }
    }
    if (part) row_store_sums(s, 2, part, dctot, N, dcoff + c, n, geo, li, rowok);
}

__global__ __launch_bounds__(EW_THREADS) void add_act_fwd_kernel(RowGeo geo, SrcDev a, SrcDev res, int has_res, int relu,
                                                                 int C, int L, float* out, float* rowmean) {
    int c, n, li;
    const bool rowok = row_coords(geo, C, c, n, li);
    if (!rowok) L = 0;
    const RowSrc ra = row_src(a, ((long long)n * a.ctot + a.coff + c) * L, a.coff + c);
    RowSrc rr = ra;
    if (has_res) rr = row_src(res, ((long long)n * res.ctot + res.coff + c) * L, res.coff + c);
    float* op = out + ((long long)n * C + c) * L;
    const int Lrow = L;
    float acc = 0.f;
    {
        for (int i = li; i < (L >> 2); i += geo.tpr) {
            float4 v = row_val4(ra, i);
            if (has_res) { float4 r = row_val4(rr, i); v.x += r.x; v.y += r.y; v.z += r.z; v.w += r.w; }
            if (relu) { v.x = fmaxf(v.x, 0.f); v.y = fmaxf(v.y, 0.f); v.z = fmaxf(v.z, 0.f); v.w = fmaxf(v.w, 0.f); }
            reinterpret_cast<float4*>(op)[i] = v;
            acc += (v.x + v.y) + (v.z + v.w);
        }
    }
    {
        for (int i = (L & ~3) + li; i < L; i += geo.tpr) {
            float v = row_val(ra, i);
            if (has_res) v += row_val(rr, i);
            v = relu ? fmaxf(v, 0.f) : v;
            op[i] = v;
            acc += v;
        }
    }
    if (rowmean) {
        acc = row_sum(acc, geo);
        if (li == 0 && rowok) rowmean[(long long)n * C + c] = acc / (float)Lrow;
    }
}

__global__ __launch_bounds__(EW_THREADS) void add_act_bwd_kernel(RowGeo geo, const float* dout, const float* out, int relu,
                                                                 const float* a_pre, const float* a_save,
                                                                 const float* r_pre, const float* r_save,
                                                                 int C, int L, int N, float* dz, float* part) {
    int c, n, li;
    const bool rowok = row_coords(geo, C, c, n, li);
    if (!rowok) L = 0;
    const long long b = ((long long)n * C + c) * L;
    float s[4] = {0.f, 0.f, 0.f, 0.f};
    const float mua = a_pre ? a_save[c] : 0.f, mur = r_pre ? r_save[c] : 0.f;
    {
        for (int i = li; i < (L >> 2); i += geo.tpr) {
            float4 d = reinterpret_cast<const float4*>(dout + b)[i];
            if (relu) {
                float4 o = reinterpret_cast<const float4*>(out + b)[i];
                if (!(o.x > 0.f)) d.x = 0.f;
                if (!(o.y > 0.f)) d.y = 0.f;
                if (!(o.z > 0.f)) d.z = 0.f;
                if (!(o.w > 0.f)) d.w = 0.f;
            }
            if (dz) reinterpret_cast<float4*>(dz + b)[i] = d;
            s[0] += (d.x + d.y) + (d.z + d.w);
            if (a_pre) {
                float4 p = reinterpret_cast<const float4*>(a_pre + b)[i];
                s[1] = fmaf(d.x, p.x - mua, fmaf(d.y, p.y - mua, fmaf(d.z, p.z - mua, fmaf(d.w, p.w - mua, s[1]))));
            }
            if (r_pre) {
                float4 p = reinterpret_cast<const float4*>(r_pre + b)[i];
                s[2] += (d.x + d.y) + (d.z + d.w);
                s[3] = fmaf(d.x, p.x - mur, fmaf(d.y, p.y - mur, fmaf(d.z, p.z - mur, fmaf(d.w, p.w - mur, s[3]))));
            }
        }
    }
    {
        for (int i = (L & ~3) + li; i < L; i += geo.tpr) {
            float d = dout[b + i];
            if (relu && !(out[b + i] > 0.f)) d = 0.f;
            if (dz) dz[b + i] = d;
            s[0] += d;
            if (a_pre) s[1] = fmaf(d, a_pre[b + i] - mua, s[1]);
            if (r_pre) { s[2] += d; s[3] = fmaf(d, r_pre[b + i] - mur, s[3]); }
        }
    }
    row_store_sums(s, r_pre ? 4 : 2, part, C, N, c, n, geo, li, rowok);
}

__global__ __launch_bounds__(EW_THREADS) void apply_kernel(RowGeo geo, SrcDev src, int C, int L, float* y, int yctot, int ycoff) {
    int c, n, li;
    const bool rowok = row_coords(geo, C, c, n, li);
    if (!rowok) L = 0;
    const long long bs = ((long long)n * src.ctot + src.coff + c) * L;
    float* yp = y + ((long long)n * yctot + ycoff + c) * L;
    for (int i = li; i < L; i += geo.tpr) yp[i] = src_value(src, bs + i, src.coff + c);
}

__global__ __launch_bounds__(EW_THREADS) void add_act_fwd_tmean_kernel(SrcDev a, SrcDev res, int has_res, int relu, int N, int C, int T, int V,
                                                                       float* out, float* xbar) {
    const int row = blockIdx.x * (EW_THREADS / 64) + (threadIdx.x >> 6), lane = threadIdx.x & 63;
    const int sub = lane >> 4, l = lane & 15;
    const int V4 = V >> 2, F = 16 / V4;
    const bool rowok = row < N * C;
    const int r = rowok ? row : 0;
    const int n = r / C, c = r - n * C;
    const int f = l / V4, g = l - f * V4;
    const bool lane_on = rowok && f < F;
    const int L = T * V;
    const RowSrc ra = row_src(a, ((long long)n * a.ctot + a.coff + c) * L, a.coff + c);
    RowSrc rr = ra;
    if (has_res) rr = row_src(res, ((long long)n * res.ctot + res.coff + c) * L, res.coff + c);
    float* op = out + ((long long)n * C + c) * L;
    float4 acc = make_float4(0.f, 0.f, 0.f, 0.f);
    if (lane_on) {
        for (int t = f + F * sub; t < T; t += 4 * F) {
            const int i4 = t * V4 + g;
            float4 v = row_val4(ra, i4);
            if (has_res) { const float4 q = row_val4(rr, i4); v.x += q.x; v.y += q.y; v.z += q.z; v.w += q.w; }
            if (relu) { v.x = fmaxf(v.x, 0.f); v.y = fmaxf(v.y, 0.f); v.z = fmaxf(v.z, 0.f); v.w = fmaxf(v.w, 0.f); }
            reinterpret_cast<float4*>(op)[i4] = v;
            acc.x += v.x; acc.y += v.y; acc.z += v.z; acc.w += v.w;
        }
    }
    float4 tot = acc;
    for (int ff = 1; ff < F; ++ff) {
        const int srcl = (lane & 48) + ff * V4 + g;
        const float px = __shfl(acc.x, srcl), py = __shfl(acc.y, srcl), pz = __shfl(acc.z, srcl), pw = __shfl(acc.w, srcl);
        tot.x += px; tot.y += py; tot.z += pz; tot.w += pw;
    }
    tot.x += __shfl_xor(tot.x, 16); tot.y += __shfl_xor(tot.y, 16); tot.z += __shfl_xor(tot.z, 16); tot.w += __shfl_xor(tot.w, 16);
    tot.x += __shfl_xor(tot.x, 32); tot.y += __shfl_xor(tot.y, 32); tot.z += __shfl_xor(tot.z, 32); tot.w += __shfl_xor(tot.w, 32);
    if (lane_on && f == 0 && sub == 0) {
        const float inv = 1.0f / (float)T;
        *reinterpret_cast<float4*>(xbar + ((long long)c * N + n) * V + 4 * g) = make_float4(tot.x * inv, tot.y * inv, tot.z * inv, tot.w * inv);
    }
}

__global__ __launch_bounds__(EW_THREADS) void tmean_kernel(SrcDev src, int N, int C, int T, int V, float* xbar) {
    const int cpb = EW_THREADS / V;
    const int cl = threadIdx.x / V, v = threadIdx.x - cl * V;
    const int c = blockIdx.x * cpb + cl, n = blockIdx.y;
    if (cl >= cpb || c >= C) return;
    const long long b = ((long long)n * src.ctot + src.coff + c) * T * V + v;
    float s = 0.f;
    int t = 0;
    for (; t + 8 <= T; t += 8) {
        float x[8];
#pragma unroll
        for (int k = 0; k < 8; ++k) x[k] = src_value(src, b + (long long)(t + k) * V, src.coff + c);
#pragma unroll
        for (int k = 0; k < 8; ++k) s += x[k];
    }
    for (; t < T; ++t) s += src_value(src, b + (long long)t * V, src.coff + c);
    xbar[((long long)c * N + n) * V + v] = s / (float)T;
}

static bool grid_ok(int N, int C) { return N > 0 && C > 0 && (long long)N * C < (1LL << 31); }

static RowGeo row_geo(int N, int C, int L, bool vec_capable) {
    const int steps = vec_capable ? (L + 3) >> 2 : L;
    int tpr = 16;
    while (tpr < 64 && tpr * 5 < steps) tpr <<= 1;
    static int wide = -1;
    if (wide < 0) { const char* e = getenv("TAMGCN_EW_WIDE"); wide = e ? atoi(e) : 1; }
    if (wide && steps >= 448) tpr = 256;
    RowGeo g; g.tpr = tpr; g.rows = N * C;
    return g;
}
static dim3 row_grid(const RowGeo& g) { return dim3((unsigned)ceil_div(g.rows, EW_THREADS / g.tpr)); }

}

extern "C" int tamgcn_ew_nparts(int N, int C, int T, int V) { (void)C; (void)T; (void)V; return N; }

extern "C" int tamgcn_gcn_tail_fwd(const tamgcn_src* y, const tamgcn_src* o, const tamgcn_src* res,
                                   int N, int C, int T, int V, float* g, void* stream) {
    TG_CHECK(y && o && g && y->x1 && o->x1 && grid_ok(N, C), "tamgcn_gcn_tail_fwd: bad args");
    const RowGeo geo = row_geo(N, C, T * V, true);
    hipLaunchKernelGGL(gcn_tail_fwd_kernel, row_grid(geo), dim3(EW_THREADS), 0, (hipStream_t)stream,
                       geo, make_src(*y), make_src(*o), res ? make_src(*res) : null_src(), res ? 1 : 0, C, T * V, g);
    tamgcn_note_kernel("gcn_tail_fwd_kernel");
    TG_LAUNCH_CHECK("tamgcn_gcn_tail_fwd");
    return 0;
}

extern "C" int tamgcn_gcn_tail_bwd(const float* dg, const float* g, const tamgcn_src* o, const float* o_save,
                                   int N, int C, int T, int V, float* dsum, float* doz, float* part, void* stream) {
    TG_CHECK(dg && g && o && o->x1 && o_save && dsum && doz && part && grid_ok(N, C), "tamgcn_gcn_tail_bwd: bad args");
    const RowGeo geo = row_geo(N, C, T * V, true);
    hipLaunchKernelGGL(gcn_tail_bwd_kernel, row_grid(geo), dim3(EW_THREADS), 0, (hipStream_t)stream,
                       geo, dg, g, make_src(*o), o_save, C, T * V, N, dsum, doz, part);
    tamgcn_note_kernel("gcn_tail_bwd_kernel");
    TG_LAUNCH_CHECK("tamgcn_gcn_tail_bwd");
    return 0;
}

extern "C" int tamgcn_gcn_mid_bwd(const float* dsum, const float* ddiff, const float* y_pre, const float* y_save,
                                  const float* r_pre, const float* r_save,
                                  int N, int C, int T, int V, float* dyb, float* dres, float* part, void* stream) {
    TG_CHECK(dsum && ddiff && y_pre && y_save && dyb && part && grid_ok(N, C) && (!r_pre || r_save), "tamgcn_gcn_mid_bwd: bad args");
    const RowGeo geo = row_geo(N, C, T * V, true);
    hipLaunchKernelGGL(gcn_mid_bwd_kernel, row_grid(geo), dim3(EW_THREADS), 0, (hipStream_t)stream,
                       geo, dsum, ddiff, y_pre, y_save, r_pre, r_save, C, T * V, N, dyb, dres, part);
    tamgcn_note_kernel("gcn_mid_bwd_kernel");
    TG_LAUNCH_CHECK("tamgcn_gcn_mid_bwd");
    return 0;
}

extern "C" int tamgcn_maxpool_fwd(const tamgcn_src* src, int N, int C, int T_in, int V, int stride,
                                  float* y, int yctot, int ycoff, int T_out, float* stats_part, void* stream) {
    TG_CHECK(src && src->x1 && y && grid_ok(N, C) && stride >= 1, "tamgcn_maxpool_fwd: bad args");
    TG_CHECK(T_out == (T_in + 2 - 3) / stride + 1, "tamgcn_maxpool_fwd: T_out=%d inconsistent with T_in=%d stride=%d", T_out, T_in, stride);
    const RowGeo geo = row_geo(N, C, T_out * V, false);
    hipLaunchKernelGGL(maxpool_fwd_kernel, row_grid(geo), dim3(EW_THREADS), 0, (hipStream_t)stream,
                       geo, make_src(*src), C, T_in, V, stride, y, yctot, ycoff, T_out, N, stats_part);
    tamgcn_note_kernel("maxpool_fwd_kernel");
    TG_LAUNCH_CHECK("tamgcn_maxpool_fwd");
    return 0;
}

extern "C" int tamgcn_maxpool_post_fwd(const tamgcn_src* src, int N, int C, int T_in, int V, int stride,
                                       float* y, int yctot, int ycoff, int T_out, const float* coef, const float* add, int relu, void* stream) {
    TG_CHECK(src && src->x1 && y && coef && grid_ok(N, C) && stride >= 1, "tamgcn_maxpool_post_fwd: bad args");
    TG_CHECK(T_out == (T_in + 2 - 3) / stride + 1, "tamgcn_maxpool_post_fwd: T_out=%d inconsistent with T_in=%d stride=%d", T_out, T_in, stride);
    const RowGeo geo = row_geo(N, C, T_out * V, false);
    hipLaunchKernelGGL(maxpool_post_fwd_kernel, row_grid(geo), dim3(EW_THREADS), 0, (hipStream_t)stream,
                       geo, make_src(*src), C, T_in, V, stride, y, yctot, ycoff, T_out, coef, add, relu);
    tamgcn_note_kernel("maxpool_post_fwd_kernel");
    TG_LAUNCH_CHECK("tamgcn_maxpool_post_fwd");
    return 0;
}

extern "C" int tamgcn_maxpool_bwd(const tamgcn_src* gy, const tamgcn_src* src, const float* src_save, int N, int C, int T_in, int T_out, int V,
                                  int stride, float* d, int dctot, int dcoff, float* part, void* stream) {
    TG_CHECK(gy && src && gy->x1 && src->x1 && src_save && d && grid_ok(N, C) && stride >= 1, "tamgcn_maxpool_bwd: bad args");
    const RowGeo geo = row_geo(N, C, T_in * V, false);
    const size_t lds = sizeof(float) * (size_t)(EW_THREADS / geo.tpr) * ((size_t)T_in * V + (size_t)T_out * V);
    const bool al16 = ((((uintptr_t)gy->x1 | (uintptr_t)(gy->x2 ? gy->x2 : gy->x1) | (uintptr_t)src->x1 | (uintptr_t)d) & 15) == 0);
    static int vec_env = -1;
    if (vec_env < 0) { const char* e = getenv("TAMGCN_POOL_VEC"); vec_env = e ? atoi(e) : 1; }
    const bool gy_lin = gy->act == 0;
    if (vec_env && gy_lin && (V & 3) == 0 && (stride == 1 || stride == 2) && al16 && !src->x2 && T_out == (T_in - 1) / stride + 1) {
        if (stride == 1)
            hipLaunchKernelGGL(maxpool_bwd_vec_kernel<1>, row_grid(geo), dim3(EW_THREADS), 0, (hipStream_t)stream,
                               geo, make_src(*gy), make_src(*src), src_save, C, T_in, T_out, V, d, dctot, dcoff, N, part);
        else
            hipLaunchKernelGGL(maxpool_bwd_vec_kernel<2>, row_grid(geo), dim3(EW_THREADS), 0, (hipStream_t)stream,
                               geo, make_src(*gy), make_src(*src), src_save, C, T_in, T_out, V, d, dctot, dcoff, N, part);
        tamgcn_note_kernel("maxpool_bwd_vec_kernel<%d>", stride);
        TG_LAUNCH_CHECK("tamgcn_maxpool_bwd");
        return 0;
    }
    if (vec_env && gy_lin && stride == 1 && !src->x2 && T_out == T_in && (long long)T_in * V < (1LL << 30)) {
        hipLaunchKernelGGL(maxpool_bwd_flat_kernel, row_grid(geo), dim3(EW_THREADS), 0, (hipStream_t)stream,
                           geo, make_src(*gy), make_src(*src), src_save, C, T_in, V, d, dctot, dcoff, N, part);
        tamgcn_note_kernel("maxpool_bwd_flat_kernel");
        TG_LAUNCH_CHECK("tamgcn_maxpool_bwd");
        return 0;
    }
    if (lds <= 64 * 1024)
        hipLaunchKernelGGL(maxpool_bwd_kernel<1>, row_grid(geo), dim3(EW_THREADS), lds, (hipStream_t)stream,
                           geo, make_src(*gy), make_src(*src), src_save, C, T_in, T_out, V, stride, d, dctot, dcoff, N, part);
    else
        hipLaunchKernelGGL(maxpool_bwd_kernel<0>, row_grid(geo), dim3(EW_THREADS), 0, (hipStream_t)stream,
                           geo, make_src(*gy), make_src(*src), src_save, C, T_in, T_out, V, stride, d, dctot, dcoff, N, part);
    tamgcn_note_kernel("maxpool_bwd_kernel<%d>", lds <= 64 * 1024 ? 1 : 0);
    TG_LAUNCH_CHECK("tamgcn_maxpool_bwd");
    return 0;
}

extern "C" int tamgcn_add_act_fwd(const tamgcn_src* a, const tamgcn_src* res, int relu,
                                  int N, int C, int T, int V, float* out, float* rowmean, float* xbar, void* stream) {
    TG_CHECK(a && a->x1 && out && grid_ok(N, C), "tamgcn_add_act_fwd: bad args");
    if (xbar) {
        TG_CHECK(!rowmean && (V & 3) == 0 && V <= 64, "tamgcn_add_act_fwd: the frame-mean output needs V %% 4 == 0, V <= 64 and no row-mean output");
        const bool al16 = (((uintptr_t)a->x1 | (uintptr_t)(a->x2 ? a->x2 : a->x1) | (uintptr_t)out | (uintptr_t)xbar |
                            (uintptr_t)(res ? res->x1 : a->x1) | (uintptr_t)((res && res->x2) ? res->x2 : a->x1)) & 15) == 0;
        TG_CHECK(al16, "tamgcn_add_act_fwd: the frame-mean form needs 16-byte aligned operands");
        hipLaunchKernelGGL(add_act_fwd_tmean_kernel, dim3((unsigned)ceil_div(N * C, EW_THREADS / 64)), dim3(EW_THREADS), 0, (hipStream_t)stream,
                           make_src(*a), res ? make_src(*res) : null_src(), res ? 1 : 0, relu, N, C, T, V, out, xbar);
        tamgcn_note_kernel("add_act_fwd_tmean_kernel");
        TG_LAUNCH_CHECK("tamgcn_add_act_fwd");
        return 0;
    }
    const RowGeo geo = row_geo(N, C, T * V, true);
    hipLaunchKernelGGL(add_act_fwd_kernel, row_grid(geo), dim3(EW_THREADS), 0, (hipStream_t)stream,
                       geo, make_src(*a), res ? make_src(*res) : null_src(), res ? 1 : 0, relu, C, T * V, out, rowmean);
    tamgcn_note_kernel("add_act_fwd_kernel");
    TG_LAUNCH_CHECK("tamgcn_add_act_fwd");
    return 0;
}

extern "C" int tamgcn_add_act_bwd(const float* dout, const float* out, int relu, const float* a_pre, const float* a_save,
                                  const float* r_pre, const float* r_save,
                                  int N, int C, int T, int V, float* dz, float* part, void* stream) {
    TG_CHECK(dout && part && grid_ok(N, C) && (!relu || out) && (!a_pre || a_save) && (!r_pre || r_save), "tamgcn_add_act_bwd: bad args");
    const RowGeo geo = row_geo(N, C, T * V, true);
    hipLaunchKernelGGL(add_act_bwd_kernel, row_grid(geo), dim3(EW_THREADS), 0, (hipStream_t)stream,
                       geo, dout, out, relu, a_pre, a_save, r_pre, r_save, C, T * V, N, dz, part);
    tamgcn_note_kernel("add_act_bwd_kernel");
    TG_LAUNCH_CHECK("tamgcn_add_act_bwd");
    return 0;
}

extern "C" int tamgcn_apply(const tamgcn_src* src, int N, int C, int T, int V, float* y, int yctot, int ycoff, void* stream) {
    TG_CHECK(src && src->x1 && y && grid_ok(N, C), "tamgcn_apply: bad args");
    const RowGeo geo = row_geo(N, C, T * V, false);
    hipLaunchKernelGGL(apply_kernel, row_grid(geo), dim3(EW_THREADS), 0, (hipStream_t)stream,
                       geo, make_src(*src), C, T * V, y, yctot, ycoff);
    tamgcn_note_kernel("apply_kernel");
    TG_LAUNCH_CHECK("tamgcn_apply");
    return 0;
}

extern "C" int tamgcn_tmean(const tamgcn_src* src, int N, int C, int T, int V, float* xbar, void* stream) {
    TG_CHECK(src && src->x1 && xbar && grid_ok(N, C) && V <= EW_THREADS, "tamgcn_tmean: bad args");
    int cpb = EW_THREADS / V;
    hipLaunchKernelGGL(tmean_kernel, dim3(ceil_div(C, cpb), N), dim3(EW_THREADS), 0, (hipStream_t)stream,
                       make_src(*src), N, C, T, V, xbar);
    tamgcn_note_kernel("tmean_kernel");
    TG_LAUNCH_CHECK("tamgcn_tmean");
    return 0;
}
```

tam_gcn_amd/functional.py:

```python
import contextlib
import os
import threading

import torch

from . import ops
from .ops import S, RELU


_SIDE = {}
_SIDE_LOCK = threading.Lock()
USE_SIDE_STREAMS = os.environ.get('TAMGCN_SIDE_STREAMS', '1') != '0'

def _side_streams(device, main, k):
    key = (device.index, main.cuda_stream, k)
    got = _SIDE.get(key)
    if got is None:
        with _SIDE_LOCK:
            got = _SIDE.get(key)
            if got is None:
                taken = {main.cuda_stream}
                for (d, m, _), ss in _SIDE.items():
                    if d == device.index:
                        taken.add(m)
# ... 174 lines not shown
    ev = None
    if EVAL_FUSED and not training and not save:
        bns = [P.bn, P.bno] + ([P.bnd] if P.mode == 'conv' else [])

        def build():
            cy, sy = _eval_coefs([(P.bn, 0)], Cout, x)
            co, so = _eval_coefs([(P.bno, 0)], Cout, x)
            cd, sd_ = _eval_coefs([(P.bnd, 0)], Cout, x) if P.mode == 'conv' else (None, None)
            cdiff = ops.coef_diff(cd, cy, {'conv': 0, 'identity': 1}.get(P.mode, 2))
            return dict(y=(cy, sy), o=(co, so), d=(cd, sd_), diff=cdiff)
        ev = _eval_cached(P.bn.m, 'unit_gcn', bns, build)
    if P.mode == 'conv':
        with fk.on(0):
            d_pre, dpart = ops.conv(xs, K=Cin, w=P.Wd, bias=P.bd, M=Cout, stats=training)
            if ev is not None:
                coef_d, save_d = ev['d']
    xbar = taken_xbar(x, Cin)
    if xbar is None:
        xbar = ops.tmean(xs, Cin)
    pq, _ = ops.conv(S(xbar.view(1, Cin, N, V)), K=Cin, w=P.W12, bias=P.B12, M=S_ * 2 * R)
    pq = pq.view(S_ * 2 * R, N, V)
    E = ops.ctrgc_build_E(xs, pq, P.W3, P.B3, P.W4, P.B4, P.PA, P.alpha, Cin, Cout, S_, R)
    y_pre, ypart, x3 = ops.ctrgc_fwd(xs, pq, P.W3, P.B3, P.W4, P.B4, P.PA, P.alpha, Cin, Cout, S_, R, stats=training,
                                     keep_x3=save, E=E)
    fk.__exit__()
    if ev is not None:
        coef_y, save_y = ev['y']
    else:
        bb = ops.BNBatch()
        coef_y, save_y = _coef(Cout, x)
        P.bn.fwd(ypart, 0, count, training, coef_y, save_y, 0, batch=bb)
        if P.mode == 'conv':
            coef_d, save_d = _coef(Cout, x)
            P.bnd.fwd(dpart, 0, count, training, coef_d, save_d, 0, batch=bb)
        bb.flush()
    if P.mode == 'conv':
        res = S(d_pre, coef=coef_d)
        coef_diff = ev['diff'] if ev is not None else ops.coef_diff(coef_d, coef_y, 0)
        diff = S(d_pre, y_pre, coef_diff)
    elif P.mode == 'identity':
        res = xs
        coef_diff = ev['diff'] if ev is not None else ops.coef_diff(None, coef_y, 1)
        diff = S(x, y_pre, coef_diff)
    else:
        res = None
        coef_diff = ev['diff'] if ev is not None else ops.coef_diff(None, coef_y, 2)
        diff = S(y_pre, None, coef_diff)
    o_pre, opart = ops.conv(diff, K=Cout, w=P.Wo, bias=P.bo, M=Cout, stats=training)
    if ev is not None:
        coef_o, save_o = ev['o']
    else:
        coef_o, save_o = _coef(Cout, x)
        P.bno.fwd(opart, 0, count, training, coef_o, save_o, 0)
    g = ops.gcn_tail_fwd(S(y_pre, coef=coef_y), S(o_pre, coef=coef_o), res)
    sv = None
    if save:
        sv = dict(x=x, xbar=xbar, pq=pq, x3=x3, E=E, y_pre=y_pre, d_pre=d_pre, o_pre=o_pre, g=g, coef_y=coef_y, save_y=save_y,
                  coef_d=coef_d, save_d=save_d, coef_o=coef_o, save_o=save_o, coef_diff=coef_diff,
                  training=training)
    return g, sv


def gcn_backward(P, sv, dg, need_dx=True, extra_dx=None):
    with ops.ReduceBatch():
        return _gcn_backward(P, sv, dg, need_dx, extra_dx)


def _gcn_backward(P, sv, dg, need_dx=True, extra_dx=None):
    x, xbar, pq, y_pre, d_pre, o_pre, g = sv['x'], sv['xbar'], sv['pq'], sv['y_pre'], sv['d_pre'], sv['o_pre'], sv['g']
    training = sv['training']
    N, Cin, T, V = x.shape
    S_, R, Cout = P.S, P.R, P.Cout
    count = N * T * V
    G = {}
    fk = Fork(x.device, 2)
    fk.__enter__()
    dsum, doz, part_o = ops.gcn_tail_bwd(dg, g, S(o_pre, coef=sv['coef_o']), sv['save_o'])
    coefb_o = torch.empty(3, Cout, device=x.device)
    G['bno.w'], G['bno.b'], G['bo'] = P.bno.bwd(part_o, 0, count, sv['save_o'], 0, training, coefb_o, 0, want_dbias=True)
    gyo = S(doz, o_pre, coefb_o)
    ddiff, _ = ops.conv(gyo, K=Cout, w=P.Wo, bias=None, M=Cout, wmode=1)
    if P.mode == 'conv':
        diff = S(d_pre, y_pre, sv['coef_diff'])
    elif P.mode == 'identity':
        diff = S(x, y_pre, sv['coef_diff'])
    else:
        diff = S(y_pre, None, sv['coef_diff'])
    with fk.on(0):
        G['Wo'] = ops.wgrad(gyo, diff, M=Cout, K=Cout)
    dyb, dres, part2 = ops.gcn_mid_bwd(dsum, ddiff, y_pre, sv['save_y'], d_pre if P.mode == 'conv' else None,
                                       sv['save_d'], want_dres=P.mode != 'zero')
    coefb_y = torch.empty(3, Cout, device=x.device)
    bb = ops.BNBatch()
    G['bn.w'], G['bn.b'], _ = P.bn.bwd(part2, 0, count, sv['save_y'], 0, training, coefb_y, 0, batch=bb)
    coefb_d = None
    if P.mode == 'conv':
        coefb_d = torch.empty(3, Cout, device=x.device)
        G['bnd.w'], G['bnd.b'], G['bd'] = P.bnd.bwd(part2[2:4], 0, count, sv['save_d'], 0, training, coefb_d, 0,
                                                     want_dbias=True, batch=bb)
    bb.flush()
    dy = S(dyb, y_pre, coefb_y)
    xs = S(x)
    cargs = (xs, pq, P.W3, P.B3, P.W4, P.B4, P.PA, P.alpha, Cin, Cout, S_, R, dy)
    fk.refork()
    with fk.on(1):
        G['PA'], G['W4'], G['B4'], G['alpha'], dpq = ops.ctrgc_bwd_de(*cargs, x3=sv['x3'], per_subset=True)
        dpq4 = S(dpq.view(1, S_ * 2 * R, N, V))
        G['W12'] = ops.wgrad(dpq4, S(xbar.view(1, Cin, N, V)), M=S_ * 2 * R, K=Cin, rows=[R] * (2 * S_))
        G['B12'] = dpq.sum((1, 2))
        dxbar = None
        if need_dx:
            dxbar, _ = ops.conv(dpq4, K=S_ * 2 * R, w=P.W12, bias=None, M=Cin, wmode=1)
    dx3, G['B3'] = ops.ctrgc_bwd_dx3(*cargs, E=sv['E'], per_subset=True)
    fk.refork()
    with fk.on(0):
        G['W3'] = ops.wgrad(S(dx3), xs, M=S_ * Cout, K=Cin, rows=[Cout] * S_)
    fk.join(1)
    dx = None
    if need_dx:
        dx, _ = ops.conv(S(dx3), K=S_ * Cout, w=P.W3, bias=None, M=Cin, wmode=1,
                         bcast=dxbar.view(Cin, N, V), bcast_scale=1.0 / T,
                         add1=dres if P.mode == 'identity' else None, add2=extra_dx)
    if P.mode == 'conv':
        gyd = S(dres, d_pre, coefb_d)
        fk.refork()
        with fk.on(0):
            G['Wd'] = ops.wgrad(gyd, xs, M=Cout, K=Cin)
        if need_dx:
            ops.conv(gyd, K=Cout, w=P.Wd, bias=None, M=Cin, wmode=1, add1=dx, y=dx)
    fk.__exit__()
# ... 39 lines not shown
    fk = Fork(g.device, 2)
    fk.__enter__()
    cat_pre = ops.empty(N, Cout, T2, V, like=g)
    coef_c, save_c = _coef(Cout, g)
    bo = ops.BNBatch()
    pair = ops.TCN_PAIR and s == 1 and Ch + Cb == Cout and ops.pair_supported((g, P.Win, P.Wl, cat_pre), N, (Cin, Cout), T, V)
    if pair:
        h_pre, hpart, _, lpart = ops.conv_pair(gs, P.Win, P.Wl, bias0=P.bin, bias1=P.bl, y1=cat_pre, ycoff1=Ch, stats=training)
        P.bn_l.fwd(lpart, Ch, cnt2, training, coef_c, save_c, Ch, batch=bo)
    else:
        with fk.on(1):
            _, lpart = ops.conv(gs, K=Cin, w=P.Wl, bias=P.bl, M=Cb, stride=s, y=cat_pre, ycoff=(nb + 1) * Cb, T_out=T2,
                                stats=training)
            P.bn_l.fwd(lpart, (nb + 1) * Cb, cnt2, training, coef_c, save_c, (nb + 1) * Cb, batch=bo)
        h_pre, hpart = ops.conv(gs, K=Cin, w=P.Win, bias=P.bin, M=Ch, stats=training)
    coef_h, save_h = _coef(Ch, g)
    bi = ops.BNBatch()
    for b in range(nb + 1):
        P.bn_in[b].fwd(hpart, b * Cb, cnt1, training, coef_h, save_h, b * Cb, batch=bi)
    bi.flush()
    fk.refork()
    if ops.tconv_supported(V, Cb, P.ks, P.dils, s, T):
        part = ops.tconv_fwd(S(h_pre, coef=coef_h, act=RELU), Cb, P.ks[0], P.dils, s, P.Wt, P.bt, True, cat_pre, 0, stats=training)
        for b in range(nb):
            P.bn_t[b].fwd(part, b * Cb, cnt2, training, coef_c, save_c, b * Cb, batch=bo)
        P.bn_pool.fwd(part, nb * Cb, cnt2, training, coef_c, save_c, nb * Cb, batch=bo)
    else:
        for b in range(nb):
            k, d = P.ks[b], P.dils[b]
            with (fk.on(b) if b > 0 else contextlib.nullcontext()):
                _, part = ops.conv(S(h_pre, coef=coef_h, coff=b * Cb, act=RELU), K=Cb, w=P.Wt[b], bias=P.bt[b], M=Cb,
                                   KT=k, dil=d, stride=s, pad=_tpad(k, d), y=cat_pre, ycoff=b * Cb, T_out=T2,
                                   stats=training)
                P.bn_t[b].fwd(part, b * Cb, cnt2, training, coef_c, save_c, b * Cb, batch=bo)
        with fk.on(0):
            part = ops.maxpool_fwd(S(h_pre, coef=coef_h, coff=nb * Cb, act=RELU), Cb, s, cat_pre, nb * Cb, stats=training)
            P.bn_pool.fwd(part, nb * Cb, cnt2, training, coef_c, save_c, nb * Cb, batch=bo)
    r_pre = coef_r = save_r = None
    if xres is None:
        xres = g
    if P.rmode == 'identity':
        res = S(xres)
    elif P.rmode == 'conv':
        rk = P.rk
        r_pre, rpart = ops.conv(S(xres), K=xres.shape[1], w=P.Wr, bias=P.br, M=Cout, KT=rk, stride=s,
                                pad=(rk - 1) // 2, T_out=T2, stats=training)
        coef_r, save_r = _coef(Cout, g)
        P.bnr.fwd(rpart, 0, cnt2, training, coef_r, save_r, 0, batch=bo)
        res = S(r_pre, coef=coef_r)
    else:
        res = None
    fk.__exit__()
    bo.flush()
    if pool is not None:
        out, rm = ops.add_act_fwd(S(cat_pre, coef=coef_c), res, P.relu, Cout, rowmean=True)
        pool.append(rm)
    else:
        if training or save:
            out, xb = ops.add_act_fwd(S(cat_pre, coef=coef_c), res, P.relu, Cout, xbar=True)
            attach_xbar(out, xb)
        else:
            out = ops.add_act_fwd(S(cat_pre, coef=coef_c), res, P.relu, Cout)
    sv = None
    if save:
        sv = dict(g=g, xres=xres, h_pre=h_pre, cat_pre=cat_pre, r_pre=r_pre, out=out, coef_h=coef_h, save_h=save_h,
                  coef_c=coef_c, save_c=save_c, coef_r=coef_r, save_r=save_r, training=training)
    return out, sv


def _tcn_forward_eval(g, P, xres):
    N, Cin, T, V = g.shape
    Cb, nb, s, Cout = P.Cb, P.nb, P.stride, P.Cout
    T2 = (T - 1) // s + 1
    Ch = (nb + 1) * Cb
    gs = S(g)
    bns = list(P.bn_in) + list(P.bn_t) + [P.bn_pool, P.bn_l] + ([P.bnr] if P.rmode == 'conv' else [])

    def build():
        ch, _ = _eval_coefs([(P.bn_in[b], b * Cb) for b in range(nb + 1)], Ch, g)
        cc, _ = _eval_coefs([(P.bn_t[b], b * Cb) for b in range(nb)] + [(P.bn_pool, nb * Cb), (P.bn_l, (nb + 1) * Cb)], Cout, g)
        cr = _eval_coefs([(P.bnr, 0)], Cout, g)[0] if P.rmode == 'conv' else None
        return ch, cc, cr
    coef_h, coef_c, coef_r = _eval_cached(P.bn_l.m, 'ms_tcn', bns, build)
    if xres is None:
        xres = g
    res = None
    if P.rmode == 'identity':
        res = xres
    elif P.rmode == 'conv':
        rk = P.rk
        res, _ = ops.conv(S(xres), K=xres.shape[1], w=P.Wr, bias=P.br, M=Cout, KT=rk, stride=s, pad=(rk - 1) // 2, T_out=T2,
                          post_coef=coef_r)
    h_pre, _ = ops.conv(gs, K=Cin, w=P.Win, bias=P.bin, M=Ch)
    out = ops.empty(N, Cout, T2, V, like=g)
    fk = Fork(g.device, 2)
    fk.__enter__()
    with fk.on(1):
        ops.conv(gs, K=Cin, w=P.Wl, bias=P.bl, M=Cb, stride=s, y=out, ycoff=(nb + 1) * Cb, T_out=T2, post_coef=coef_c,
                 post_act=P.relu, add1=res)
    for b in range(nb):
        k, d = P.ks[b], P.dils[b]
        with (fk.on(b) if b > 0 else contextlib.nullcontext()):
            ops.conv(S(h_pre, coef=coef_h, coff=b * Cb, act=RELU), K=Cb, w=P.Wt[b], bias=P.bt[b], M=Cb, KT=k, dil=d, stride=s,
                     pad=_tpad(k, d), y=out, ycoff=b * Cb, T_out=T2, post_coef=coef_c, post_act=P.relu, add1=res)
    with fk.on(0):
        ops.maxpool_post_fwd(S(h_pre, coef=coef_h, coff=nb * Cb, act=RELU), Cb, s, out, nb * Cb, coef_c, res, P.relu)
    fk.__exit__()
    return out


def tcn_backward(P, sv, dout, need_dg=True, need_dxres=True):
    with ops.ReduceBatch():
        return _tcn_backward(P, sv, dout, need_dg, need_dxres)


def _tcn_backward(P, sv, dout, need_dg=True, need_dxres=True):
    g, xres, h_pre, cat_pre, r_pre, out = sv['g'], sv['xres'], sv['h_pre'], sv['cat_pre'], sv['r_pre'], sv['out']
    training = sv['training']
    N, Cin, T, V = g.shape
    Cb, nb, s, Cout = P.Cb, P.nb, P.stride, P.Cout
    T2 = cat_pre.shape[2]
    cnt1, cnt2 = N * T * V, N * T2 * V
    Ch = (nb + 1) * Cb
    G = {}
    fk = Fork(g.device, 2)
    fk.__enter__()
    dz, part = ops.add_act_bwd(dout, out, P.relu, cat_pre, sv['save_c'], r_pre, sv['save_r'], want_dz=bool(P.relu))
    if dz is None:
        dz = dout
    coefb_c = torch.empty(3, Cout, device=g.device)
    bo = ops.BNBatch()
    G['bn_t'] = []
    G['bt'] = []
    for b in range(nb):
        dgam, dbet, dbias = P.bn_t[b].bwd(part, b * Cb, cnt2, sv['save_c'], b * Cb, training, coefb_c, b * Cb, True, batch=bo)
        G['bn_t'].append((dgam, dbet))
        G['bt'].append(dbias)
    dgam, dbet, _ = P.bn_pool.bwd(part, nb * Cb, cnt2, sv['save_c'], nb * Cb, training, coefb_c, nb * Cb, batch=bo)
    G['bn_pool'] = (dgam, dbet)
    dgam, dbet, G['bl'] = P.bn_l.bwd(part, (nb + 1) * Cb, cnt2, sv['save_c'], (nb + 1) * Cb, training, coefb_c,
                                     (nb + 1) * Cb, True, batch=bo)
    G['bn_l'] = (dgam, dbet)
    coefb_r = None
    if P.rmode == 'conv':
        coefb_r = torch.empty(3, Cout, device=g.device)
        dgam, dbet, G['br'] = P.bnr.bwd(part[2:4], 0, cnt2, sv['save_r'], 0, training, coefb_r, 0, True, batch=bo)
        G['bnr'] = (dgam, dbet)
    bo.flush()

    def gcat(coff):
        return S(dz, cat_pre, coefb_c, coff=coff)

    dh = ops.empty(N, Ch, T, V, like=g)
    coefb_h = torch.empty(3, Ch, device=g.device)
    G['Wt'] = []
    G['bn_in'] = []
    dbin = []
    marks = []
    bi = ops.BNBatch()
    fused = ops.tconv_supported(V, Cb, P.ks, P.dils, s, T)
    fused_w = fused and ops.tconv_wgrad_pays(V, Cb, s)
    if fused:
        hp_all = ops.tconv_bwd(gcat(0), Cb, P.ks[0], P.dils, s, P.Wt, S(h_pre, coef=sv['coef_h']), sv['save_h'], dh, 0)
    for b in range(nb):
        k, d = P.ks[b], P.dils[b]
        pad = _tpad(k, d)
        if fused:
            hp = hp_all
        else:
            with (fk.on(b) if b > 0 else contextlib.nullcontext()):
                _, hp = ops.conv(gcat(b * Cb), K=Cb, w=P.Wt[b], bias=None, M=Cb, KT=k, dil=d, stride=1,
                                 pad=(k - 1) * d - pad, wmode=1, up=s, y=dh, ycoff=b * Cb, T_out=T,
                                 mask=S(h_pre, coef=sv['coef_h'], coff=b * Cb), aux=h_pre, aux_center=sv['save_h'], auxcoff=b * Cb,
                                 stats=True)
        dgam, dbet, dbias = P.bn_in[b].bwd(hp, b * Cb, cnt1, sv['save_h'], b * Cb, training, coefb_h, b * Cb, True, batch=bi)
        if b > 0 and not fused:
            marks.append(fk.mark(b))
        G['bn_in'].append((dgam, dbet))
        dbin.append(dbias)
        if not fused_w:
            with fk.on(b):
                G['Wt'].append(ops.wgrad(gcat(b * Cb), S(h_pre, coef=sv['coef_h'], coff=b * Cb, act=RELU), M=Cb, K=Cb,
                                         KT=k, dil=d, stride=s, pad=pad))
    if fused_w:
        with fk.on(0):
            G['Wt'] = ops.tconv_wgrad(gcat(0), S(h_pre, coef=sv['coef_h'], act=RELU), Cb, P.ks[0], P.dils, s)
    hp = ops.maxpool_bwd(gcat(nb * Cb), S(h_pre, coef=sv['coef_h'], coff=nb * Cb, act=RELU), sv['save_h'], Cb, s, dh,
                         nb * Cb)
    dgam, dbet, dbias = P.bn_in[nb].bwd(hp, nb * Cb, cnt1, sv['save_h'], nb * Cb, training, coefb_h, nb * Cb, True, batch=bi)
    G['bn_in'].append((dgam, dbet))
    dbin.append(dbias)
    for ev in marks:
        fk.wait(ev)
    bi.flush()
    G['bin'] = dbin
    gs = S(g)
    gyh = S(dh, h_pre, coefb_h)
    fk.refork()
    nsp = None
    if ops.TCN_PAIR and s == 1 and Ch + Cb == Cout and Ch % 8 == 0 and \
            ops.pair_supported((g, dh, h_pre, dz, cat_pre), N, (Cin, Cout), T, V):
        nsp = ops.wgrad_pair_nsplit(gyh, gcat(Ch), gs, Ch, Cb, Cin)
    if nsp is not None:
        with fk.on(0):
            gw = ops.wgrad_pair(gyh, gcat(Ch), gs, Ch, Cb, Cin, rows=[Cb] * (nb + 2), nsplit=nsp)
            G['Win'], G['Wl'] = gw[:nb + 1], gw[nb + 1]
    else:
        with fk.on(0):
            G['Win'] = ops.wgrad(gyh, gs, M=Ch, K=Cin, rows=[Cb] * (nb + 1))
        with fk.on(1):
            G['Wl'] = ops.wgrad(gcat((nb + 1) * Cb), gs, M=Cb, K=Cin, stride=s)
    dg = None
    if need_dg:
        dg, _ = ops.conv(gyh, K=Ch, w=P.Win, bias=None, M=Cin, wmode=1)
        ops.conv(gcat((nb + 1) * Cb), K=Cb, w=P.Wl, bias=None, M=Cin, wmode=1, y=dg, T_out=T2, ostride=s, add1=dg)
    dxres = None
    if P.rmode == 'identity':
        dxres = dz
    elif P.rmode == 'conv':
        gyr = S(dz, r_pre, coefb_r)
        rk = P.rk
        rpad = (rk - 1) // 2
        fk.refork()
        with fk.on(1):
            G['Wr'] = ops.wgrad(gyr, S(xres), M=Cout, K=xres.shape[1], KT=rk, stride=s, pad=rpad)
        if need_dxres:
            Tx = xres.shape[2]
            if rk == 1:
                dxres = ops.zeros_like(xres) if s > 1 else ops.empty_like(xres)
                ops.conv(gyr, K=Cout, w=P.Wr, bias=None, M=xres.shape[1], wmode=1, y=dxres, T_out=T2, ostride=s)
            else:
                dxres, _ = ops.conv(gyr, K=Cout, w=P.Wr, bias=None, M=xres.shape[1], KT=rk, stride=1,
                                    pad=(rk - 1) - rpad, wmode=1, up=s, T_out=Tx)
    fk.__exit__()
    return dg, dxres, G


_CALL = threading.local()


class _Fn(torch.autograd.Function):
    @classmethod
    def run(cls, *args):
        prev = getattr(_CALL, 'grad', True)
        _CALL.grad = torch.is_grad_enabled()
        try:
            return cls.apply(*args)
        finally:
            _CALL.grad = prev


def _needs(ctx):
    return getattr(_CALL, 'grad', True) and any(ctx.needs_input_grad)


class UnitGCNFn(_Fn):
    @staticmethod
    def forward(ctx, mod, x, *params):
        P = mod._pack(params)
        g, sv = gcn_forward(x, P, mod.training, save=_needs(ctx))
        ctx.mod, ctx.P, ctx.sv = mod, P, sv
        return g

    @staticmethod
    def backward(ctx, dg):
        dx, G = gcn_backward(ctx.P, ctx.sv, dg.contiguous(), need_dx=ctx.needs_input_grad[1])
        ctx.sv = None
        return (None, dx) + tuple(ctx.mod._route(G))


class MSTCNFn(_Fn):
    @staticmethod
    def forward(ctx, mod, x, *params):
        P = mod._pack(params)
        out, sv = tcn_forward(x, P, mod.training, save=_needs(ctx))
        ctx.mod, ctx.P, ctx.sv = mod, P, sv
        return out

    @staticmethod
    def backward(ctx, dout):
        need = ctx.needs_input_grad[1]
        dg, dxres, G = tcn_backward(ctx.P, ctx.sv, dout.contiguous(), need_dg=need, need_dxres=need)
        ctx.sv = None
        if need and dxres is not None:
            dg = dg + dxres
        return (None, dg) + tuple(ctx.mod._route(G))


class TCNGCNUnitFn(_Fn):

    @staticmethod
    def forward(ctx, mod, x, ngcn, emit, *params):
        Pg = mod.gcn1._pack(params[:ngcn])
        Pt = mod._pack_tcn(params[ngcn:])
        save = _needs(ctx)
        training = mod.training
        g, svg = gcn_forward(x, Pg, training, save)
        pool = [] if emit else None
        out, svt = tcn_forward(g, Pt, training, save, xres=x, pool=pool)
        ctx.mod, ctx.Pg, ctx.Pt, ctx.svg, ctx.svt, ctx.ngcn = mod, Pg, Pt, svg, svt, ngcn
        if not emit:
            return out
        rm = pool[0] if pool else out.new_empty(0, out.shape[1])
        ctx.mark_non_differentiable(rm)
        return out, rm

    @staticmethod
    def backward(ctx, dout, _drm=None):
        need_dx = ctx.needs_input_grad[1]
        dg, dxres, Gt = tcn_backward(ctx.Pt, ctx.svt, dout.contiguous(), need_dg=True, need_dxres=need_dx)
        ctx.svt = None
        dx, Gg = gcn_backward(ctx.Pg, ctx.svg, dg, need_dx=need_dx, extra_dx=dxres)
        ctx.svg = None
        return (None, dx, None, None) + tuple(ctx.mod.gcn1._route(Gg)) + tuple(ctx.mod._route_tcn(Gt))


class CTRGCFn(_Fn):
    @staticmethod
    def forward(ctx, x, A, alpha, w1, b1, w2, b2, w3, b3, w4, b4):
        N, Cin, T, V = x.shape
        Cout, R = w3.shape[0], w1.shape[0]
        W12 = torch.cat((w1.reshape(R, Cin), w2.reshape(R, Cin)))
        B12 = torch.cat((b1, b2))
        W3, W4 = w3.reshape(Cout, Cin), w4.reshape(1, Cout, R)
        A3 = A.reshape(1, V, V).contiguous()
        al = alpha.reshape(1).to(torch.float32).contiguous()
        xs = S(x)
        xbar = ops.tmean(xs, Cin)
        pq, _ = ops.conv(S(xbar.view(1, Cin, N, V)), K=Cin, w=W12, bias=B12, M=2 * R)
        pq = pq.view(2 * R, N, V)
        save = _needs(ctx)
        E = ops.ctrgc_build_E(xs, pq, W3, b3, W4, b4.reshape(1, Cout), A3, al, Cin, Cout, 1, R)
        y, _, x3 = ops.ctrgc_fwd(xs, pq, W3, b3, W4, b4.reshape(1, Cout), A3, al, Cin, Cout, 1, R, stats=False, keep_x3=save, E=E)
        ctx.sv = (x, xbar, pq, W12, W3, b3, W4, b4.reshape(1, Cout), A3, al, E, x3) if save else None
        ctx.shapes = (A.shape, alpha.shape, w1.shape, w3.shape, w4.shape)
        return y

    @staticmethod
    def backward(ctx, dy):
        x, xbar, pq, W12, W3, b3, W4, b4, A3, al, E, x3 = ctx.sv
        ctx.sv = None
        N, Cin, T, V = x.shape
        Cout, R = W3.shape[0], W4.shape[2]
        xs = S(x)
        dx3, db3, dA, dW4, db4, dal, dpq = ops.ctrgc_bwd(xs, pq, W3, b3, W4, b4, A3, al, Cin, Cout, 1, R,
                                                         S(dy.contiguous()), x3=x3, E=E)
        dpq4 = S(dpq.view(1, 2 * R, N, V))
        dW12 = ops.wgrad(dpq4, S(xbar.view(1, Cin, N, V)), M=2 * R, K=Cin)
        dB12 = dpq.sum((1, 2))
        dW3 = ops.wgrad(S(dx3), xs, M=Cout, K=Cin)
        dx = None
        if ctx.needs_input_grad[0]:
            dxbar, _ = ops.conv(dpq4, K=2 * R, w=W12, bias=None, M=Cin, wmode=1)
            dx, _ = ops.conv(S(dx3), K=Cout, w=W3, bias=None, M=Cin, wmode=1, bcast=dxbar.view(Cin, N, V),
                             bcast_scale=1.0 / T)
        As, als, w1s, w3s, w4s = ctx.shapes
        return (dx, dA.reshape(As), dal.reshape(als), dW12[:R].reshape(w1s), dB12[:R], dW12[R:].reshape(w1s),
                dB12[R:], dW3.reshape(w3s), db3, dW4.reshape(w4s), db4.reshape(Cout))


class ConvBNFn(_Fn):
    @staticmethod
    def forward(ctx, cfg, x, w, b, gamma, beta):
        k, s, d, pad, bnmod = cfg
        bn = BN(bnmod)
# ... 279 lines not shown
```

tam_gcn_amd/ops.py:

```python
import ctypes as C
import os
import threading

import torch

from . import _lib
from ._lib import Src, ConvDesc, WgradDesc, CtrgcDesc, ReduceDesc, TconvDesc, TCONV_MAXB

RELU = 1


def _stream():
    return C.c_void_p(torch.cuda.current_stream().cuda_stream)


def _ptr(t):
    if t is None:
        return None
    if not (t.is_cuda and t.is_contiguous()):
        raise RuntimeError('tam_gcn_amd: expected a contiguous HIP (cuda) tensor; there is no CPU path')
    if t.dtype not in (torch.float32, torch.int64, torch.int32, torch.float64):
        raise RuntimeError(f'tam_gcn_amd: unsupported dtype {t.dtype}')
    return t.data_ptr()


class S:
    __slots__ = ('x1', 'x2', 'coef', 'coff', 'act', 'ctot')

    def __init__(self, x1, x2=None, coef=None, coff=0, act=0):
        self.x1, self.x2, self.coef, self.coff, self.act = x1, x2, coef, coff, act
        self.ctot = x1.shape[1]
        if x2 is not None and x2.shape != x1.shape:
            raise RuntimeError('tam_gcn_amd: x1/x2 geometry mismatch')
        if coef is not None and tuple(coef.shape) != (3, self.ctot):
            raise RuntimeError(f'tam_gcn_amd: coef shape {tuple(coef.shape)} != (3,{self.ctot})')

    def c(self):
        return Src(_ptr(self.x1), _ptr(self.x2), _ptr(self.coef), self.ctot, self.coff, self.act)


def _lib_():
    return _lib.load()


CHUNK_ELEMS = int(os.environ.get("TAMGCN_CHUNK_ELEMS", str(2 ** 32 - 1)))


def n_chunks(N, per_clip):
    c = max(1, CHUNK_ELEMS // max(1, per_clip))
    return [(i, min(N, i + c)) for i in range(0, N, c)]


def _slice_src(src, n0, n1):
    return S(src.x1[n0:n1], None if src.x2 is None else src.x2[n0:n1], src.coef, src.coff, src.act)


SLACK = 4


def empty(*shape, like):
    n = 1
    for d_ in shape:
        n *= d_
    return torch.empty(n + SLACK, device=like.device, dtype=torch.float32)[:n].view(shape)


def empty_like(t):
    return empty(*t.shape, like=t)


def zeros_like(t):
    return empty(*t.shape, like=t).zero_()


def with_slack(t):
    if t is None or t.shape[-1] % 4 == 0:
        return t
    st = t.untyped_storage()
    if st.nbytes() - (t.storage_offset() + t.numel()) * t.element_size() >= 4 * SLACK:
        return t
    out = empty(*t.shape, like=t)
    out.copy_(t)
    return out


def conv(src, K, w, bias, M, KT=1, dil=1, stride=1, pad=0, wmode=0, up=1,
         y=None, ycoff=0, T_out=None, T_y=None, ostride=1, add1=None, add2=None,
         bcast=None, bcast_scale=0.0, mask=None, aux=None, aux_center=None, auxcoff=0, stats=False,
         post_coef=None, post_act=0):
    if src.x1.shape[-1] % 4:
        src = S(with_slack(src.x1), with_slack(src.x2), src.coef, src.coff, src.act)
    x = src.x1
    N, _, T_in, V = x.shape
    if T_out is None:
        T_out = (T_in + 2 * pad - dil * (KT - 1) - 1) // stride + 1
    if y is None:
        if T_y is None:
            T_y = T_out
        y = empty(N, M, T_y, V, like=x)
    else:
        T_y = y.shape[2]
    per_clip = max(x.shape[1] * T_in * V, y.shape[1] * T_y * V)
    if N > 1 and N * per_clip > CHUNK_ELEMS:
        if stats or mask is not None or aux is not None:
            raise RuntimeError('tam_gcn_amd: a convolution over >= 2^31 elements cannot carry BatchNorm moments / a mask')
        for n0, n1 in n_chunks(N, per_clip):
            conv(_slice_src(src, n0, n1), K, w, bias, M, KT, dil, stride, pad, wmode, up, y=y[n0:n1], ycoff=ycoff, T_out=T_out,
                 ostride=ostride, add1=None if add1 is None else add1[n0:n1], add2=None if add2 is None else add2[n0:n1],
                 bcast=None if bcast is None else bcast[:, n0:n1].contiguous(), bcast_scale=bcast_scale,
                 post_coef=post_coef, post_act=post_act)
        return y, None
    d = ConvDesc()
    d.src = src.c()
    d.N, d.K, d.T_in, d.V = N, K, T_in, V
    d.w, d.bias = _ptr(w), _ptr(bias)
    d.M, d.KT, d.dil, d.stride, d.pad = M, KT, dil, stride, pad
    d.wmode, d.up = wmode, up
    d.y, d.yctot, d.ycoff = _ptr(y), y.shape[1], ycoff
    d.T_out, d.T_y, d.ostride = T_out, T_y, ostride
    d.add1, d.add2, d.bcast, d.bcast_scale = _ptr(add1), _ptr(add2), _ptr(bcast), bcast_scale
    mc = None
    if mask is not None:
        mc = mask.c()
        d.mask = C.pointer(mc)
    if aux is not None:
        d.aux, d.aux_center, d.auxctot, d.auxcoff = _ptr(aux), _ptr(aux_center), aux.shape[1], auxcoff
    if post_coef is not None:
        d.post_coef, d.post_ctot = _ptr(post_coef), post_coef.shape[1]
    d.post_act = int(post_act)
    part = None
    lib = _lib_()
    if stats:
        nparts = lib.tamgcn_conv_nparts(C.byref(d))
        if nparts <= 0:
            raise RuntimeError('tamgcn_conv: no tiling for this shape')
        part = empty(2, y.shape[1], nparts, like=x)
        d.stats_part, d.stats_ctot, d.stats_coff = _ptr(part), y.shape[1], ycoff
    _lib.check(lib.tamgcn_conv(C.byref(d), _stream()), 'tamgcn_conv')
    return y, part


TCN_PAIR = os.environ.get('TAMGCN_TCN_PAIR', '1') != '0'


def pair_supported(tensors, N, chans, T, V):
    if V % 4 or V > 32 or T * V < 64 or any(c % 16 or c > 512 for c in chans) or N * max(chans) * T * V > CHUNK_ELEMS:
        return False
    return all(t is None or (t.is_cuda and t.is_contiguous() and t.data_ptr() % 16 == 0) for t in tensors)


def conv_pair(src, w0, w1, bias0=None, bias1=None, y0=None, ycoff0=0, y1=None, ycoff1=0, stats=False):
    x = src.x1
    N, _, T, V = x.shape
    M0, M1, K = w0.shape[0], w1.shape[0], w0.shape[1]
    if w1.shape[1] != K:
        raise RuntimeError('tamgcn_conv_pair: the two weight matrices have the same K')
    d = _lib.ConvPairDesc()
    d.N, d.T, d.V, d.stride = N, T, V, 1
    d.src = src.c()
    d.w0, d.w1 = _ptr(w0), _ptr(w1)
    d.K, d.M0, d.M1 = K, M0, M1
    d.bias0, d.bias1 = _ptr(bias0), _ptr(bias1)
    if y0 is None:
        y0 = empty(N, M0, T, V, like=x)
    if y1 is None:
        y1 = empty(N, M1, T, V, like=x)
    if y0.shape[2:] != x.shape[2:] or y1.shape[2:] != x.shape[2:]:
        raise RuntimeError('tamgcn_conv_pair: destination geometry differs from the source (stride-1 1x1 only)')
    d.y0, d.yctot0, d.ycoff0 = _ptr(y0), y0.shape[1], ycoff0
    d.y1, d.yctot1, d.ycoff1 = _ptr(y1), y1.shape[1], ycoff1
    lib = _lib_()
    part0 = part1 = None
    if stats:
        cd = ConvDesc()
        cd.src = d.src
        cd.N, cd.K, cd.T_in, cd.V, cd.M, cd.KT, cd.dil, cd.stride, cd.up = N, K, T, V, M0 + M1, 1, 1, 1, 1
        cd.T_out, cd.T_y, cd.ostride = T, T, 1
        nparts = lib.tamgcn_conv_nparts(C.byref(cd))
        if nparts <= 0:
            raise RuntimeError('tamgcn_conv_pair: no tiling for this shape')
        part0 = empty(2, y0.shape[1], nparts, like=x)
        part1 = empty(2, y1.shape[1], nparts, like=x)
        d.stats_part0, d.stats_ctot0, d.stats_coff0 = _ptr(part0), y0.shape[1], ycoff0
        d.stats_part1, d.stats_ctot1, d.stats_coff1 = _ptr(part1), y1.shape[1], ycoff1
    _lib.check(lib.tamgcn_conv_pair(C.byref(d), _stream()), 'tamgcn_conv_pair')
    return y0, part0, y1, part1


def _wgrad_desc(gy, src, M, K, KT=1, dil=1, stride=1, pad=0):
    d = WgradDesc()
    d.gy, d.src = gy.c(), src.c()
    d.N, d.M, d.K, d.T_in, d.T_out, d.V = gy.x1.shape[0], M, K, src.x1.shape[2], gy.x1.shape[2], gy.x1.shape[3]
# ... 415 lines not shown
    return dE


def ctrgc_bwd_de_tail(dE, pq, w4, b4, alpha, R, per_subset=False, groups=1):
    N, S, Cout, V, _ = dE.shape
    d = CtrgcDesc()
    d.N, d.Cout, d.S, d.R, d.V = N, Cout, S, R, V
    d.pq, d.w4, d.b4, d.alpha = _ptr(pq), _ptr(w4), _ptr(b4), _ptr(alpha)
    like = dE
    ps = per_subset
    if ctrgc_route(V) == 'tiled':
        if groups != 1:
            raise RuntimeError('tam_gcn_amd: the tiled dE tail (V in {32, 64}) has no channel groups')
        NUC = _lib_().tamgcn_ctrgc_tiled_chunks(V)
        dA_part = empty(N, S, V, V, like=like)
        dw4_part = empty(N * NUC, S, Cout, R, like=like)
        db4_part = empty(N * NUC, S, Cout, like=like)
        dal_part = empty(N * S * NUC, 1, like=like)
        dpq = empty(NUC, S * 2 * R, N, V, like=like)
        _lib.check(_lib_().tamgcn_ctrgc_tiled_de_tail(C.byref(d), _ptr(dE), _ptr(dA_part), _ptr(dw4_part), _ptr(db4_part), _ptr(dal_part),
                                                      _ptr(dpq), _stream()), 'tamgcn_ctrgc_tiled_de_tail')
        return (reduce_sum(dA_part, N), reduce_sum(dw4_part, N * NUC, chunks=[(Cout, R, 1, 1)] * S if ps else None),
                reduce_sum(db4_part, N * NUC, chunks=[(Cout,)] * S if ps else None), reduce_sum(dal_part, N * S * NUC),
                reduce_sum(dpq, NUC, immediate=True))
    if R > 32:
        raise RuntimeError('tam_gcn_amd: CTRGC with R > 32 rel-channels is not built')
    G = groups
    dA_part = empty(N * G, S, V, V, like=like)
    dw4_part = empty(N, S, Cout, R, like=like)
    db4_part = empty(N, S, Cout, like=like)
    dal_part = empty(N * S * G, 1, like=like)
    dpq = empty(G, S * 2 * R, N, V, like=like)
    name = 'tamgcn_vgen_de_tail' if ctrgc_route(V) == 'vgen' else 'tamgcn_ctrgc_bwd_de_tail'
    _lib.check(getattr(_lib_(), name)(C.byref(d), _ptr(dE), _ptr(dA_part), _ptr(dw4_part), _ptr(db4_part),
                                      _ptr(dal_part), _ptr(dpq), G, _stream()), name)
    dpq = dpq[0] if G == 1 else reduce_sum(dpq, G, immediate=True)
    return (reduce_sum(dA_part, N * G), reduce_sum(dw4_part, N, chunks=[(Cout, R, 1, 1)] * S if ps else None),
            reduce_sum(db4_part, N, chunks=[(Cout,)] * S if ps else None), reduce_sum(dal_part, N * S * G), dpq)


def ctrgc_bwd_de(x, pq, w3, b3, w4, b4, A, alpha, Cin, Cout, S, R, dy, x3=None, per_subset=False):
    if x3 is None:
        x3 = _x3_gemm(x, w3, b3, Cin, Cout, S)
    dE = ctrgc_bwd_de_acc(dy, x3, Cout, S)
    return ctrgc_bwd_de_tail(dE, pq, w4, b4, alpha, R, per_subset=per_subset)


def ctrgc_bwd(x, pq, w3, b3, w4, b4, A, alpha, Cin, Cout, S, R, dy, x3=None, E=None):
    dx3, db3 = ctrgc_bwd_dx3(x, pq, w3, b3, w4, b4, A, alpha, Cin, Cout, S, R, dy, E=E)
    dA, dw4, db4, dal, dpq = ctrgc_bwd_de(x, pq, w3, b3, w4, b4, A, alpha, Cin, Cout, S, R, dy, x3)
    return dx3, db3, dA, dw4, db4, dal, dpq


def gcn_tail_fwd(y, o, res):
    N, _, T, V = y.x1.shape
    Cc = y.ctot
    g = empty(N, Cc, T, V, like=y.x1)
    yc, oc = y.c(), o.c()
    rc = res.c() if res is not None else None
    _lib.check(_lib_().tamgcn_gcn_tail_fwd(C.byref(yc), C.byref(oc), C.byref(rc) if rc is not None else None,
                                           N, Cc, T, V, _ptr(g), _stream()), 'tamgcn_gcn_tail_fwd')
    return g


def gcn_tail_bwd(dg, g, o, o_save):
    N, Cc, T, V = g.shape
    dsum, doz = empty_like(g), empty_like(g)
    part = empty(2, Cc, N, like=g)
    oc = o.c()
    _lib.check(_lib_().tamgcn_gcn_tail_bwd(_ptr(dg), _ptr(g), C.byref(oc), _ptr(o_save), N, Cc, T, V, _ptr(dsum), _ptr(doz),
                                           _ptr(part), _stream()), 'tamgcn_gcn_tail_bwd')
    return dsum, doz, part


def gcn_mid_bwd(dsum, ddiff, y_pre, y_save, r_pre, r_save, want_dres):
    N, Cc, T, V = dsum.shape
    dyb = empty_like(dsum)
    dres = empty_like(dsum) if want_dres else None
    part = empty(4 if r_pre is not None else 2, Cc, N, like=dsum)
    _lib.check(_lib_().tamgcn_gcn_mid_bwd(_ptr(dsum), _ptr(ddiff), _ptr(y_pre), _ptr(y_save), _ptr(r_pre), _ptr(r_save), N, Cc, T, V,
                                          _ptr(dyb), _ptr(dres), _ptr(part), _stream()), 'tamgcn_gcn_mid_bwd')
    return dyb, dres, part


def maxpool_fwd(src, C_, stride, y, ycoff, stats):
    N, _, T_in, V = src.x1.shape
    T_out = y.shape[2]
    part = empty(2, y.shape[1], N, like=y) if stats else None
    sc = src.c()
    _lib.check(_lib_().tamgcn_maxpool_fwd(C.byref(sc), N, C_, T_in, V, stride, _ptr(y), y.shape[1], ycoff, T_out,
                                          _ptr(part), _stream()), 'tamgcn_maxpool_fwd')
    return part


def maxpool_post_fwd(src, C_, stride, y, ycoff, coef, add, relu):
    N, _, T_in, V = src.x1.shape
    sc = src.c()
    _lib.check(_lib_().tamgcn_maxpool_post_fwd(C.byref(sc), N, C_, T_in, V, stride, _ptr(y), y.shape[1], ycoff, y.shape[2],
                                               _ptr(coef), _ptr(add), int(relu), _stream()), 'tamgcn_maxpool_post_fwd')


def maxpool_bwd(gy, src, src_save, C_, stride, d, dcoff):
    N, _, T_in, V = src.x1.shape
    T_out = gy.x1.shape[2]
    part = empty(2, d.shape[1], N, like=d)
    gc, sc = gy.c(), src.c()
    _lib.check(_lib_().tamgcn_maxpool_bwd(C.byref(gc), C.byref(sc), _ptr(src_save), N, C_, T_in, T_out, V, stride, _ptr(d),
                                          d.shape[1], dcoff, _ptr(part), _stream()), 'tamgcn_maxpool_bwd')
    return part


XBAR_FOLD = os.environ.get('TAMGCN_XBAR_FOLD', '1') != '0'


def add_act_fwd(a, res, relu, C_, rowmean=False, xbar=False):
    N, _, T, V = a.x1.shape
    out = empty(N, C_, T, V, like=a.x1)
    rm = torch.empty(N, C_, device=out.device, dtype=torch.float32) if rowmean else None
    xb = None
    if xbar and not rowmean and XBAR_FOLD and V % 4 == 0 and V <= 64:
        xb = empty(C_, N, V, like=a.x1)
    ac = a.c()
    rc = res.c() if res is not None else None
    _lib.check(_lib_().tamgcn_add_act_fwd(C.byref(ac), C.byref(rc) if rc is not None else None, int(relu),
                                          N, C_, T, V, _ptr(out), _ptr(rm), _ptr(xb), _stream()), 'tamgcn_add_act_fwd')
    if xbar:
        return out, xb
    return (out, rm) if rowmean else out


def add_act_bwd(dout, out, relu, a_pre, a_save, r_pre, r_save, want_dz):
    N, Cc, T, V = dout.shape
    dz = empty_like(dout) if want_dz else None
    part = empty(4 if r_pre is not None else 2, Cc, N, like=dout)
    _lib.check(_lib_().tamgcn_add_act_bwd(_ptr(dout), _ptr(out), int(relu), _ptr(a_pre), _ptr(a_save), _ptr(r_pre), _ptr(r_save), N, Cc, T, V,
                                          _ptr(dz), _ptr(part), _stream()), 'tamgcn_add_act_bwd')
    return dz, part


def apply(src, C_, y=None, ycoff=0):
    N, _, T, V = src.x1.shape
    if y is None:
        y = empty(N, C_, T, V, like=src.x1)
    sc = src.c()
    _lib.check(_lib_().tamgcn_apply(C.byref(sc), N, C_, T, V, _ptr(y), y.shape[1], ycoff, _stream()), 'tamgcn_apply')
    return y


def stem_stats(x5, dout=None, center=None):
    N, C_, T, V, M = x5.shape
    part = empty(2, C_ * V * M, N, like=x5)
    _lib.check(_lib_().tamgcn_stem_stats(_ptr(x5), _ptr(dout), _ptr(center), N, C_, T, V, M, _ptr(part), _stream()), 'tamgcn_stem_stats')
    return part


def stem_apply(x5, coef, dout=None):
    N, C_, T, V, M = x5.shape
    out = empty(N * M, C_, T, V, like=x5) if dout is None else torch.empty_like(x5)
    _lib.check(_lib_().tamgcn_stem_apply(_ptr(x5), _ptr(dout), _ptr(coef), N, C_, T, V, M, _ptr(out), _stream()), 'tamgcn_stem_apply')
    return out


def head_pool_fwd(x, M):
    NM, C_, T, V = x.shape
    pooled = empty(NM // M, C_, like=x)
    _lib.check(_lib_().tamgcn_head_pool_fwd(_ptr(x), NM // M, C_, T, V, M, _ptr(pooled), _stream()), 'tamgcn_head_pool_fwd')
    return pooled


def head_pool_bwd(dpooled, M, T, V):
    N, C_ = dpooled.shape
    dx = empty(N * M, C_, T, V, like=dpooled)
    _lib.check(_lib_().tamgcn_head_pool_bwd(_ptr(dpooled), N, C_, T, V, M, _ptr(dx), _stream()), 'tamgcn_head_pool_bwd')
    return dx


def head_fc_fwd(pooled, W, b):
    N, C_ = pooled.shape
    K = W.shape[0]
    logits = empty(N, K, like=pooled)
    _lib.check(_lib_().tamgcn_head_fc_fwd(_ptr(pooled), _ptr(W), _ptr(b), N, C_, K, _ptr(logits), _stream()), 'tamgcn_head_fc_fwd')
    return logits


def head_fc_grouped(pooled, W, b, G):
    GN, C_ = pooled.shape
    K = W.shape[1]
    scores = empty(G, GN // G, K, like=pooled)
    _lib.check(_lib_().tamgcn_head_fc_grouped(_ptr(pooled), _ptr(W), _ptr(b), G, GN // G, C_, K, _ptr(scores), _stream()), 'tamgcn_head_fc_grouped')
# ... 206 lines not shown
```

Measured before the change: 9264 clips/s.

## Save ReLU sign bitmasks in forward and fuse masking into backward conv epilogue

The forward ReLU kernels (GCN tail and add+act) now also write a packed 1-bit-per-element sign mask. The backward kernels read these bits instead of the full fp32 activation tensor. In addition, the input-gradient conv of the TCN backward applies the GCN-tail ReLU mask directly in its epilogue, so the following elementwise backward pass can skip the masking. The intent is to cut backward memory traffic and one pass over dg, at the cost of extra bit writes in forward, a new kernel template specialization, and shape/env-dependent routing.

New measurement: 9372 clips/s, median of 6. 1.01x the previous value.

```diff
diff --git a/include/tamgcn.h b/include/tamgcn.h
--- a/include/tamgcn.h
+++ b/include/tamgcn.h
@@ -56,6 +56,8 @@
 int tamgcn_conv_nparts(const tamgcn_conv_desc* d);
 int tamgcn_conv(const tamgcn_conv_desc* d, void* stream);
 
+int tamgcn_conv_signmask(const tamgcn_conv_desc* d, const unsigned char* bits, int bctot, int bcoff, void* stream);
+
 typedef struct tamgcn_wgrad_desc {
     tamgcn_src gy;
     tamgcn_src src;
@@ -179,6 +181,10 @@
                         int N, int C, int T, int V, float* g, void* stream);
 int tamgcn_gcn_tail_bwd(const float* dg, const float* g, const tamgcn_src* o, const float* o_save,
                         int N, int C, int T, int V, float* dsum, float* doz, float* part, void* stream);
+int tamgcn_gcn_tail_fwd_bits(const tamgcn_src* y, const tamgcn_src* o, const tamgcn_src* res,
+                             int N, int C, int T, int V, float* g, unsigned char* bits, void* stream);
+int tamgcn_gcn_tail_bwd_bits(const float* dg, const unsigned char* bits, const tamgcn_src* o, const float* o_save,
+                             int N, int C, int T, int V, float* dsum, float* doz, float* part, void* stream);
 int tamgcn_gcn_mid_bwd(const float* dsum, const float* ddiff, const float* y_pre, const float* y_save,
                        const float* r_pre, const float* r_save,
                        int N, int C, int T, int V, float* dyb, float* dres, float* part, void* stream);
@@ -213,6 +219,11 @@
 int tamgcn_add_act_bwd(const float* dout, const float* out, int relu, const float* a_pre, const float* a_save,
                        const float* r_pre, const float* r_save,
                        int N, int C, int T, int V, float* dz, float* part, void* stream);
+int tamgcn_add_act_fwd_bits(const tamgcn_src* a, const tamgcn_src* res,
+                            int N, int C, int T, int V, float* out, float* rowmean, float* xbar, unsigned char* bits, void* stream);
+int tamgcn_add_act_bwd_bits(const float* dout, const unsigned char* bits, const float* a_pre, const float* a_save,
+                            const float* r_pre, const float* r_save,
+                            int N, int C, int T, int V, float* dz, float* part, void* stream);
 
 int tamgcn_apply(const tamgcn_src* src, int N, int C, int T, int V, float* y, int yctot, int ycoff, void* stream);
 
diff --git a/tam_gcn_amd/_lib.py b/tam_gcn_amd/_lib.py
--- a/tam_gcn_amd/_lib.py
+++ b/tam_gcn_amd/_lib.py
@@ -155,6 +155,7 @@
     'tamgcn_conv': (_i, [C.POINTER(ConvDesc), _p]),
     'tamgcn_wgrad_max_split': (_i, [C.POINTER(WgradDesc)]),
     'tamgcn_wgrad': (_i, [C.POINTER(WgradDesc), _p]),
+    'tamgcn_conv_signmask': (_i, [C.POINTER(ConvDesc), _p, _i, _i, _p]),
     'tamgcn_conv_pair': (_i, [C.POINTER(ConvPairDesc), _p]),
     'tamgcn_wgrad_pair': (_i, [C.POINTER(WgradPairDesc), _p]),
     'tamgcn_stem_stats': (_i, [_p, _p, _p, _i, _i, _i, _i, _i, _p, _p]),
@@ -193,6 +194,8 @@
     'tamgcn_ew_nparts': (_i, [_i, _i, _i, _i]),
     'tamgcn_gcn_tail_fwd': (_i, [_SP, _SP, _SP, _i, _i, _i, _i, _p, _p]),
     'tamgcn_gcn_tail_bwd': (_i, [_p, _p, _SP, _p, _i, _i, _i, _i, _p, _p, _p, _p]),
+    'tamgcn_gcn_tail_fwd_bits': (_i, [_SP, _SP, _SP, _i, _i, _i, _i, _p, _p, _p]),
+    'tamgcn_gcn_tail_bwd_bits': (_i, [_p, _p, _SP, _p, _i, _i, _i, _i, _p, _p, _p, _p]),
     'tamgcn_gcn_mid_bwd': (_i, [_p, _p, _p, _p, _p, _p, _i, _i, _i, _i, _p, _p, _p, _p]),
     'tamgcn_tconv_supported': (_i, [_i, _i, _i, _i, C.POINTER(C.c_int), _i, _i]),
     'tamgcn_tconv_nparts': (_i, [C.POINTER(TconvDesc), _i]),
@@ -205,6 +208,8 @@
     'tamgcn_maxpool_bwd': (_i, [_SP, _SP, _p, _i, _i, _i, _i, _i, _i, _p, _i, _i, _p, _p]),
     'tamgcn_add_act_fwd': (_i, [_SP, _SP, _i, _i, _i, _i, _i, _p, _p, _p, _p]),
     'tamgcn_add_act_bwd': (_i, [_p, _p, _i, _p, _p, _p, _p, _i, _i, _i, _i, _p, _p, _p]),
+    'tamgcn_add_act_fwd_bits': (_i, [_SP, _SP, _i, _i, _i, _i, _p, _p, _p, _p, _p]),
+    'tamgcn_add_act_bwd_bits': (_i, [_p, _p, _p, _p, _p, _p, _i, _i, _i, _i, _p, _p, _p]),
     'tamgcn_apply': (_i, [_SP, _i, _i, _i, _i, _p, _i, _i, _p]),
     'tamgcn_score_fuse': (_i, [_p, _p, _i, _i, _i, _i, _p, _p, _p, _p, _p]),
     'tamgcn_ce_fwd': (_i, [_p, _p, _i, _i, _p, _p, _p]),
diff --git a/tam_gcn_amd/csrc/conv.hip b/tam_gcn_amd/csrc/conv.hip
--- a/tam_gcn_amd/csrc/conv.hip
+++ b/tam_gcn_amd/csrc/conv.hip
@@ -39,6 +39,9 @@
     float* y1; int yctot1, ycoff1;
     float* stats1; int sctot1, scoff1;
 };
+struct SignArgs {
+    const unsigned char* bits; int ctot, coff;
+};
 
 __device__ __forceinline__ void conv_epilogue(const ConvArgs& a, f32x4 (&acc)[4][MAXCW], float* Ss, int n, int m0, int t0,
                                               int ncols, int cw0, int mt_act, int c_act, const int (&tl)[MAXCW],
@@ -221,9 +224,9 @@
     conv_epilogue(a, acc, Ss, n, m0, t0, ncols, cw0, mt_act, c_act, tl, vv, j, kq, wave, tid);
 }
 
-template <int NTH, bool PR = false>
+template <int NTH, int PR = 0, typename SIDE = PairArgs>
 __device__ __forceinline__ void staged_rows(const ConvArgs& a, const float* Tt, int PT, int RP, int r0, int BMT, int m0, int n, int t0,
-                                            int ncols, float* Ss, int Vs, int v0, const PairArgs* pa = nullptr) {
+                                            int ncols, float* Ss, int Vs, int v0, const SIDE* pa = nullptr) {
     const int tid = threadIdx.x, V = a.V;
     const int TPR = NTH / RP;
     const int row = tid / TPR, seg = tid - row * TPR;
@@ -239,7 +242,7 @@
         const float pc1 = a.post_coef ? a.post_coef[a.ycoff + m] : 1.f, pc0 = a.post_coef ? a.post_coef[2 * a.post_ctot + a.ycoff + m] : 0.f;
         const float plo = a.post_act == 1 ? 0.f : -__builtin_inff();
         long long ybase = ((long long)n * a.yctot + a.ycoff + m) * a.T_y * V;
-        if constexpr (PR) {
+        if constexpr (PR == 1) {
             if (m >= pa->M0) {
                 const int m1 = m - pa->M0;
                 bia = pa->bias1 ? pa->bias1[m1] : 0.f; yp = pa->y1;
@@ -247,6 +250,8 @@
             }
         }
         const long long mbase = a.has_mask ? ((long long)n * a.mask.ctot + a.mask.coff + m) * a.T_y * V : 0;
+        const unsigned char* sb = nullptr;
+        if constexpr (PR == 2) sb = pa->bits + ((long long)n * pa->ctot + pa->coff + m) * ((a.T_y * V + 3) >> 2);
         const long long abase = a.aux ? ((long long)n * a.auxctot + a.auxcoff + m) * a.T_y * V : 0;
         const float* bc = a.bcast ? a.bcast + ((long long)m * a.N + n) * V : nullptr;
         float mc1 = 1.f, mc2 = 0.f, mc0 = 0.f;
@@ -256,7 +261,17 @@
             if (a.mask.x2) mc2 = a.mask.coef[a.mask.ctot + mch];
         }
         const int nc4 = (ncols + 3) >> 2;
-        for (int c4 = seg; c4 < nc4; c4 += TPR) {
+        unsigned snib = 0;
+        if constexpr (PR == 2) {
+            const unsigned char* sp = sb + ((t0 * V) >> 2);
+#pragma unroll
+            for (int k = 0; k < 6; ++k) {
+                const int c = seg + k * TPR;
+                snib |= (unsigned)sp[c < nc4 ? c : nc4 - 1] << (4 * k);
+            }
+        }
+        int it = 0;
+        for (int c4 = seg; c4 < nc4; c4 += TPR, ++it) {
             const int col = c4 << 2;
             const int fr = col / Vs, v = col - fr * Vs;
             if ((vecok || v + 4 <= Vs) && col + 4 <= ncols) {
@@ -282,6 +297,13 @@
                     if (!(fmaf(mc1, q.y, fmaf(mc2, q2.y, mc0)) > 0.f)) val.y = 0.f;
                     if (!(fmaf(mc1, q.z, fmaf(mc2, q2.z, mc0)) > 0.f)) val.z = 0.f;
                     if (!(fmaf(mc1, q.w, fmaf(mc2, q2.w, mc0)) > 0.f)) val.w = 0.f;
+                }
+                if constexpr (PR == 2) {
+                    const unsigned q = it < 6 ? snib >> (4 * it) : sb[off >> 2];
+                    if (!(q & 1u)) val.x = 0.f;
+                    if (!(q & 2u)) val.y = 0.f;
+                    if (!(q & 4u)) val.z = 0.f;
+                    if (!(q & 8u)) val.w = 0.f;
                 }
                 if (a.stats_part) {
                     float4 x2 = val;
@@ -306,6 +328,9 @@
                         const float q = a.mask.x1[mbase + off], q2 = a.mask.x2 ? a.mask.x2[mbase + off] : 0.f;
                         if (!(fmaf(mc1, q, fmaf(mc2, q2, mc0)) > 0.f)) val = 0.f;
                     }
+                    if constexpr (PR == 2) {
+                        if (!((sb[off >> 2] >> (off & 3)) & 1u)) val = 0.f;
+                    }
                     if (a.stats_part) {
                         const float x2 = a.aux ? a.aux[abase + off] - ctr : val;
                         p1 += val;
@@ -546,8 +571,10 @@
 #endif
 constexpr int G_NT = 512, G_BMT = 64, G_PA = 80, G_PBMAX = 320, G_NST = 3, G_CWT = 5;
 
+template <int PAIR> struct GldsSide { typedef PairArgs type; };
+template <> struct GldsSide<2> { typedef SignArgs type; };
 template <int NSRC, int BK, bool PRO, int NW, int PAIR = 0>
-__global__ __launch_bounds__(NW * 64, NW == 8 ? 4 : 2) void conv1x1_glds_kernel(const ConvArgs a, int ntt, int nmt, const PairArgs pa) {
+__global__ __launch_bounds__(NW * 64, NW == 8 ? 4 : 2) void conv1x1_glds_kernel(const ConvArgs a, int ntt, int nmt, const typename GldsSide<PAIR>::type pa) {
     constexpr int G_NT = NW * 64, G_MT = 16 / NW;
     extern __shared__ __attribute__((aligned(16))) float smem[];
     constexpr int STG = BK * G_PBMAX * NSRC + BK * G_PA;
@@ -823,15 +850,19 @@
             }
         }
         __syncthreads();
-        staged_rows<G_NT, PAIR == 1>(a, Tt, PT, RP, r0, G_BMT, m0, n, t0, ncols, Ss, V, 0, &pa);
+        staged_rows<G_NT, PAIR>(a, Tt, PT, RP, r0, G_BMT, m0, n, t0, ncols, Ss, V, 0, &pa);
     }
     if (a.stats_part) {
         __syncthreads();
         if (tid < 2 * G_BMT) {
             int stt = tid / G_BMT, row = tid - stt * G_BMT;
             int m = m0 + row;
-            if (PAIR == 1 && m < a.M && m >= pa.M0) pa.stats1[((long long)stt * pa.sctot1 + pa.scoff1 + m - pa.M0) * a.nparts + g] = Ss[stt * 4 * BM + row];
-            else if (m < a.M) a.stats_part[((long long)stt * a.stats_ctot + a.stats_coff + m) * a.nparts + g] = Ss[stt * 4 * BM + row];
+            if constexpr (PAIR == 1) {
+                if (m < a.M && m >= pa.M0) pa.stats1[((long long)stt * pa.sctot1 + pa.scoff1 + m - pa.M0) * a.nparts + g] = Ss[stt * 4 * BM + row];
+                else if (m < a.M) a.stats_part[((long long)stt * a.stats_ctot + a.stats_coff + m) * a.nparts + g] = Ss[stt * 4 * BM + row];
+            } else {
+                if (m < a.M) a.stats_part[((long long)stt * a.stats_ctot + a.stats_coff + m) * a.nparts + g] = Ss[stt * 4 * BM + row];
+            }
         }
     }
     TG_T(tg1); TG_ACC(7, tg1 - tg0); TG_ACC(8, tg1 - tt0); TG_ACC(9, 1);
@@ -1129,7 +1160,7 @@
     return d->N * p.ntt * p.nsl;
 }
 
-extern "C" int tamgcn_conv(const tamgcn_conv_desc* d, void* stream) {
+static int conv_launch(const tamgcn_conv_desc* d, const SignArgs* sg, void* stream) {
     TG_CHECK(d && d->src.x1 && d->w && d->y, "tamgcn_conv: null pointer");
     TG_CHECK(d->N > 0 && d->K > 0 && d->M > 0 && d->T_in > 0 && d->T_out > 0 && d->V > 0,
              "tamgcn_conv: bad dims N=%d K=%d M=%d T_in=%d T_out=%d V=%d", d->N, d->K, d->M, d->T_in, d->T_out, d->V);
@@ -1168,7 +1199,17 @@
     const size_t lds_split = sizeof(float) * ((size_t)GS_NST * (GS_BK * G_PBMAX + GS_BK * 128) + 3 * (size_t)d->K + 2 * 4 * BM + 128);
     const bool big = glds && tamgcn_split_mode() >= 1 && d->src.act == 0 && d->M >= 128 && d->M % 4 == 0 && d->K % GS_BK == 0 &&
                      lds_split <= 160 * 1024 && !d->post_coef && d->wmode == 1 && !d->stats_part;
-    if (big) {
+    if (sg) {
+        static int nw8 = -1;
+        if (nw8 < 0) { const char* e = getenv("TAMGCN_CONV_WAVES"); nw8 = (e && atoi(e) == 4) ? 0 : 1; }
+        TG_CHECK(glds && !big && p.flat && d->src.x2 && nw8 && (d->V & 3) == 0 && !d->mask && !d->post_coef,
+                 "tamgcn_conv_signmask: not the two-source stride-1 LDS-DMA GEMM with V %% 4 == 0 (K=%d M=%d T=%d V=%d)", d->K, d->M, d->T_in, d->V);
+        const int nmt = ceil_div(d->M, G_BMT);
+        const unsigned nblk = (unsigned)(d->N * p.ntt * nmt);
+        tg_launch_lds<conv1x1_glds_kernel<2, 8, true, 8, 2>>(160 * 1024, dim3(nblk), dim3(8 * 64), glds_lds_bytes<2, 8>(d->K, true),
+                                                             (hipStream_t)stream, a, p.ntt, nmt, *sg);
+        tamgcn_note_kernel("conv1x1_glds_kernel<2, 8, true, 8, 2>");
+    } else if (big) {
         const int nmt = ceil_div(d->M, 128);
         const unsigned nblk = (unsigned)(d->N * p.ntt * nmt);
         tg_launch_lds<conv1x1_glds_split_kernel<2, false, 4>>(160 * 1024, dim3(nblk), dim3(G_NT), lds_split, (hipStream_t)stream, a, p.ntt, nmt);
@@ -1210,6 +1251,16 @@
     }
     TG_LAUNCH_CHECK("tamgcn_conv");
     return 0;
+}
+
+extern "C" int tamgcn_conv(const tamgcn_conv_desc* d, void* stream) { return conv_launch(d, nullptr, stream); }
+
+extern "C" int tamgcn_conv_signmask(const tamgcn_conv_desc* d, const unsigned char* bits, int bctot, int bcoff, void* stream) {
+    TG_CHECK(d && bits, "tamgcn_conv_signmask: null pointer");
+    TG_CHECK(bcoff >= 0 && bcoff + d->M <= bctot, "tamgcn_conv_signmask: mask channel slice out of range");
+    TG_CHECK(d->ostride == 1 && d->T_out == d->T_y, "tamgcn_conv_signmask: the output covers every frame of y (ostride 1)");
+    const SignArgs sg = {bits, bctot, bcoff};
+    return conv_launch(d, &sg, stream);
 }
 
 
diff --git a/tam_gcn_amd/csrc/elementwise.hip b/tam_gcn_amd/csrc/elementwise.hip
--- a/tam_gcn_amd/csrc/elementwise.hip
+++ b/tam_gcn_amd/csrc/elementwise.hip
@@ -38,6 +38,22 @@
     }
 }
 
+__device__ __forceinline__ unsigned sign4(const float4& v) {
+    return (v.x > 0.f ? 1u : 0u) | (v.y > 0.f ? 2u : 0u) | (v.z > 0.f ? 4u : 0u) | (v.w > 0.f ? 8u : 0u);
+}
+__device__ __forceinline__ void sign_tail_store(unsigned tb, unsigned char* brow, int L, int li) {
+    tb |= __shfl_xor(tb, 1);
+    tb |= __shfl_xor(tb, 2);
+    if (li == 0 && (L & 3)) brow[L >> 2] = (unsigned char)tb;
+}
+__device__ __forceinline__ float4 sign_mask4(float4 d, unsigned q) {
+    if (!(q & 1u)) d.x = 0.f;
+    if (!(q & 2u)) d.y = 0.f;
+    if (!(q & 4u)) d.z = 0.f;
+    if (!(q & 8u)) d.w = 0.f;
+    return d;
+}
+
 struct RowSrc {
     const float* x1; const float* x2; float c1, c2, c0; int act;
 };
@@ -65,7 +81,7 @@
 }
 
 __global__ __launch_bounds__(EW_THREADS) void gcn_tail_fwd_kernel(RowGeo geo, SrcDev y, SrcDev o, SrcDev res, int has_res,
-                                                                  int C, int L, float* g) {
+                                                                  int C, int L, float* g, unsigned char* bits) {
     int c, n, li;
     const bool rowok = row_coords(geo, C, c, n, li);
     if (!rowok) L = 0;
@@ -74,6 +90,8 @@
     RowSrc rr = ry;
     if (has_res) rr = row_src(res, ((long long)n * res.ctot + res.coff + c) * L, res.coff + c);
     float* gp = g + ((long long)n * C + c) * L;
+    unsigned char* brow = bits ? bits + ((long long)n * C + c) * ((L + 3) >> 2) : nullptr;
+    unsigned tb = 0;
     {
         for (int i = li; i < (L >> 2); i += geo.tpr) {
             float4 a = row_val4(ry, i), b = row_val4(ro, i);
@@ -82,38 +100,52 @@
             v.x = fmaxf(a.x + tanhf(b.x) + r.x, 0.f); v.y = fmaxf(a.y + tanhf(b.y) + r.y, 0.f);
             v.z = fmaxf(a.z + tanhf(b.z) + r.z, 0.f); v.w = fmaxf(a.w + tanhf(b.w) + r.w, 0.f);
             reinterpret_cast<float4*>(gp)[i] = v;
+            if (brow) brow[i] = (unsigned char)sign4(v);
         }
     }
     {
         for (int i = (L & ~3) + li; i < L; i += geo.tpr) {
             float v = row_val(ry, i) + tanhf(row_val(ro, i));
             if (has_res) v += row_val(rr, i);
-            gp[i] = fmaxf(v, 0.f);
-        }
-    }
-}
-
-__global__ __launch_bounds__(EW_THREADS) void gcn_tail_bwd_kernel(RowGeo geo, const float* dg, const float* g, SrcDev o, const float* o_save,
-                                                                  int C, int L, int N, float* dsum, float* doz, float* part) {
+            v = fmaxf(v, 0.f);
+            gp[i] = v;
+            if (v > 0.f) tb |= 1u << (i & 3);
+        }
+    }
+    if (bits) sign_tail_store(tb, brow, L, li);
+}
+
+template <int SIGN>
+__device__ __forceinline__ void gcn_tail_bwd_body(const RowGeo& geo, const float* dg, const float* g, const unsigned char* bits, const SrcDev& o,
+                                                  const float* o_save, int C, int L, int N, float* dsum, float* doz, float* part) {
     int c, n, li;
     const bool rowok = row_coords(geo, C, c, n, li);
     if (!rowok) L = 0;
     const long long b = ((long long)n * C + c) * L;
     const long long bo = ((long long)n * o.ctot + o.coff + c) * L;
+    const unsigned char* brow = SIGN == 1 ? bits + ((long long)n * C + c) * ((L + 3) >> 2) : nullptr;
     const RowSrc ro = row_src(o, bo, o.coff + c);
     float s[2] = {0.f, 0.f};
     const float mu = o_save[o.coff + c];
     {
         for (int i = li; i < (L >> 2); i += geo.tpr) {
-            float4 gg = reinterpret_cast<const float4*>(g + b)[i], dd = reinterpret_cast<const float4*>(dg + b)[i];
+            float4 dd = reinterpret_cast<const float4*>(dg + b)[i];
             float4 ob = row_val4(ro, i), op = reinterpret_cast<const float4*>(o.x1 + bo)[i];
             float4 d, z;
             float t;
-            d.x = gg.x > 0.f ? dd.x : 0.f; t = tanhf(ob.x); z.x = d.x * (1.f - t * t);
-            d.y = gg.y > 0.f ? dd.y : 0.f; t = tanhf(ob.y); z.y = d.y * (1.f - t * t);
-            d.z = gg.z > 0.f ? dd.z : 0.f; t = tanhf(ob.z); z.z = d.z * (1.f - t * t);
-            d.w = gg.w > 0.f ? dd.w : 0.f; t = tanhf(ob.w); z.w = d.w * (1.f - t * t);
-            reinterpret_cast<float4*>(dsum + b)[i] = d;
+            if (SIGN == 0) {
+                float4 gg = reinterpret_cast<const float4*>(g + b)[i];
+                d.x = gg.x > 0.f ? dd.x : 0.f; d.y = gg.y > 0.f ? dd.y : 0.f; d.z = gg.z > 0.f ? dd.z : 0.f; d.w = gg.w > 0.f ? dd.w : 0.f;
+            } else if (SIGN == 1) {
+                d = sign_mask4(dd, brow[i]);
+            } else {
+                d = dd;
+            }
+            t = tanhf(ob.x); z.x = d.x * (1.f - t * t);
+            t = tanhf(ob.y); z.y = d.y * (1.f - t * t);
+            t = tanhf(ob.z); z.z = d.z * (1.f - t * t);
+            t = tanhf(ob.w); z.w = d.w * (1.f - t * t);
+            if (SIGN != 2) reinterpret_cast<float4*>(dsum + b)[i] = d;
             reinterpret_cast<float4*>(doz + b)[i] = z;
             s[0] += (z.x + z.y) + (z.z + z.w);
             s[1] = fmaf(z.x, op.x - mu, fmaf(z.y, op.y - mu, fmaf(z.z, op.z - mu, fmaf(z.w, op.w - mu, s[1]))));
@@ -121,16 +153,24 @@
     }
     {
         for (int i = (L & ~3) + li; i < L; i += geo.tpr) {
-            float d = g[b + i] > 0.f ? dg[b + i] : 0.f;
+            float d = dg[b + i];
+            if (SIGN == 0) d = g[b + i] > 0.f ? d : 0.f;
+            if (SIGN == 1) d = ((brow[i >> 2] >> (i & 3)) & 1) ? d : 0.f;
             float off = tanhf(row_val(ro, i));
             float dz = d * (1.f - off * off);
-            dsum[b + i] = d;
+            if (SIGN != 2) dsum[b + i] = d;
             doz[b + i] = dz;
             s[0] += dz;
             s[1] = fmaf(dz, o.x1[bo + i] - mu, s[1]);
         }
     }
     row_store_sums(s, 2, part, C, N, c, n, geo, li, rowok);
+}
+__global__ __launch_bounds__(EW_THREADS) void gcn_tail_bwd_kernel(RowGeo geo, const float* dg, const float* g, const unsigned char* bits, SrcDev o,
+                                                                  const float* o_save, int C, int L, int N, float* dsum, float* doz, float* part) {
+    if (g) gcn_tail_bwd_body<0>(geo, dg, g, nullptr, o, o_save, C, L, N, dsum, doz, part);
+    else if (bits) gcn_tail_bwd_body<1>(geo, dg, nullptr, bits, o, o_save, C, L, N, dsum, doz, part);
+    else gcn_tail_bwd_body<2>(geo, dg, nullptr, nullptr, o, o_save, C, L, N, nullptr, doz, part);
 }
 
 __global__ __launch_bounds__(EW_THREADS) void gcn_mid_bwd_kernel(RowGeo geo, const float* dsum, const float* ddiff, const float* y_pre, const float* y_save,
@@ -407,7 +447,7 @@
 }
 
 __global__ __launch_bounds__(EW_THREADS) void add_act_fwd_kernel(RowGeo geo, SrcDev a, SrcDev res, int has_res, int relu,
-                                                                 int C, int L, float* out, float* rowmean) {
+                                                                 int C, int L, float* out, float* rowmean, unsigned char* bits) {
     int c, n, li;
     const bool rowok = row_coords(geo, C, c, n, li);
     if (!rowok) L = 0;
@@ -415,6 +455,8 @@
     RowSrc rr = ra;
     if (has_res) rr = row_src(res, ((long long)n * res.ctot + res.coff + c) * L, res.coff + c);
     float* op = out + ((long long)n * C + c) * L;
+    unsigned char* brow = bits ? bits + ((long long)n * C + c) * ((L + 3) >> 2) : nullptr;
+    unsigned tb = 0;
     const int Lrow = L;
     float acc = 0.f;
     {
@@ -423,6 +465,7 @@
             if (has_res) { float4 r = row_val4(rr, i); v.x += r.x; v.y += r.y; v.z += r.z; v.w += r.w; }
             if (relu) { v.x = fmaxf(v.x, 0.f); v.y = fmaxf(v.y, 0.f); v.z = fmaxf(v.z, 0.f); v.w = fmaxf(v.w, 0.f); }
             reinterpret_cast<float4*>(op)[i] = v;
+            if (brow) brow[i] = (unsigned char)sign4(v);
             acc += (v.x + v.y) + (v.z + v.w);
         }
     }
@@ -432,29 +475,34 @@
             if (has_res) v += row_val(rr, i);
             v = relu ? fmaxf(v, 0.f) : v;
             op[i] = v;
+            if (v > 0.f) tb |= 1u << (i & 3);
             acc += v;
         }
     }
+    if (bits) sign_tail_store(tb, brow, L, li);
     if (rowmean) {
         acc = row_sum(acc, geo);
         if (li == 0 && rowok) rowmean[(long long)n * C + c] = acc / (float)Lrow;
     }
 }
 
-__global__ __launch_bounds__(EW_THREADS) void add_act_bwd_kernel(RowGeo geo, const float* dout, const float* out, int relu,
-                                                                 const float* a_pre, const float* a_save,
-                                                                 const float* r_pre, const float* r_save,
-                                                                 int C, int L, int N, float* dz, float* part) {
+template <bool BITS>
+__device__ __forceinline__ void add_act_bwd_body(const RowGeo& geo, const float* dout, const float* out, const unsigned char* bits, int relu,
+                                                 const float* a_pre, const float* a_save, const float* r_pre, const float* r_save,
+                                                 int C, int L, int N, float* dz, float* part) {
     int c, n, li;
     const bool rowok = row_coords(geo, C, c, n, li);
     if (!rowok) L = 0;
     const long long b = ((long long)n * C + c) * L;
+    const unsigned char* brow = BITS ? bits + ((long long)n * C + c) * ((L + 3) >> 2) : nullptr;
     float s[4] = {0.f, 0.f, 0.f, 0.f};
     const float mua = a_pre ? a_save[c] : 0.f, mur = r_pre ? r_save[c] : 0.f;
     {
         for (int i = li; i < (L >> 2); i += geo.tpr) {
             float4 d = reinterpret_cast<const float4*>(dout + b)[i];
-            if (relu) {
+            if (BITS) {
+                d = sign_mask4(d, brow[i]);
+            } else if (relu) {
                 float4 o = reinterpret_cast<const float4*>(out + b)[i];
                 if (!(o.x > 0.f)) d.x = 0.f;
                 if (!(o.y > 0.f)) d.y = 0.f;
@@ -477,7 +525,8 @@
     {
         for (int i = (L & ~3) + li; i < L; i += geo.tpr) {
             float d = dout[b + i];
-            if (relu && !(out[b + i] > 0.f)) d = 0.f;
+            if (BITS) { if (!((brow[i >> 2] >> (i & 3)) & 1)) d = 0.f; }
+            else if (relu && !(out[b + i] > 0.f)) d = 0.f;
             if (dz) dz[b + i] = d;
             s[0] += d;
             if (a_pre) s[1] = fmaf(d, a_pre[b + i] - mua, s[1]);
@@ -486,6 +535,13 @@
     }
     row_store_sums(s, r_pre ? 4 : 2, part, C, N, c, n, geo, li, rowok);
 }
+__global__ __launch_bounds__(EW_THREADS) void add_act_bwd_kernel(RowGeo geo, const float* dout, const float* out, const unsigned char* bits, int relu,
+                                                                 const float* a_pre, const float* a_save,
+                                                                 const float* r_pre, const float* r_save,
+                                                                 int C, int L, int N, float* dz, float* part) {
+    if (bits) add_act_bwd_body<true>(geo, dout, nullptr, bits, 1, a_pre, a_save, r_pre, r_save, C, L, N, dz, part);
+    else add_act_bwd_body<false>(geo, dout, out, nullptr, relu, a_pre, a_save, r_pre, r_save, C, L, N, dz, part);
+}
 
 __global__ __launch_bounds__(EW_THREADS) void apply_kernel(RowGeo geo, SrcDev src, int C, int L, float* y, int yctot, int ycoff) {
     int c, n, li;
@@ -497,7 +553,7 @@
 }
 
 __global__ __launch_bounds__(EW_THREADS) void add_act_fwd_tmean_kernel(SrcDev a, SrcDev res, int has_res, int relu, int N, int C, int T, int V,
-                                                                       float* out, float* xbar) {
+                                                                       float* out, float* xbar, unsigned char* bits) {
     const int row = blockIdx.x * (EW_THREADS / 64) + (threadIdx.x >> 6), lane = threadIdx.x & 63;
     const int sub = lane >> 4, l = lane & 15;
     const int V4 = V >> 2, F = 16 / V4;
@@ -511,6 +567,7 @@
     RowSrc rr = ra;
     if (has_res) rr = row_src(res, ((long long)n * res.ctot + res.coff + c) * L, res.coff + c);
     float* op = out + ((long long)n * C + c) * L;
+    unsigned char* brow = bits ? bits + ((long long)n * C + c) * (L >> 2) : nullptr;
     float4 acc = make_float4(0.f, 0.f, 0.f, 0.f);
     if (lane_on) {
         for (int t = f + F * sub; t < T; t += 4 * F) {
@@ -519,6 +576,7 @@
             if (has_res) { const float4 q = row_val4(rr, i4); v.x += q.x; v.y += q.y; v.z += q.z; v.w += q.w; }
             if (relu) { v.x = fmaxf(v.x, 0.f); v.y = fmaxf(v.y, 0.f); v.z = fmaxf(v.z, 0.f); v.w = fmaxf(v.w, 0.f); }
             reinterpret_cast<float4*>(op)[i4] = v;
+            if (brow) brow[i4] = (unsigned char)sign4(v);
             acc.x += v.x; acc.y += v.y; acc.z += v.z; acc.w += v.w;
         }
     }
@@ -573,15 +631,24 @@
 
 extern "C" int tamgcn_ew_nparts(int N, int C, int T, int V) { (void)C; (void)T; (void)V; return N; }
 
+static int gcn_tail_fwd_launch(const char* who, const tamgcn_src* y, const tamgcn_src* o, const tamgcn_src* res,
+                               int N, int C, int T, int V, float* g, unsigned char* bits, void* stream) {
+    TG_CHECK(y && o && g && y->x1 && o->x1 && grid_ok(N, C), "%s: bad args", who);
+    const RowGeo geo = row_geo(N, C, T * V, true);
+    hipLaunchKernelGGL(gcn_tail_fwd_kernel, row_grid(geo), dim3(EW_THREADS), 0, (hipStream_t)stream,
+                       geo, make_src(*y), make_src(*o), res ? make_src(*res) : null_src(), res ? 1 : 0, C, T * V, g, bits);
+    tamgcn_note_kernel("gcn_tail_fwd_kernel");
+    TG_LAUNCH_CHECK(who);
+    return 0;
+}
 extern "C" int tamgcn_gcn_tail_fwd(const tamgcn_src* y, const tamgcn_src* o, const tamgcn_src* res,
                                    int N, int C, int T, int V, float* g, void* stream) {
-    TG_CHECK(y && o && g && y->x1 && o->x1 && grid_ok(N, C), "tamgcn_gcn_tail_fwd: bad args");
-    const RowGeo geo = row_geo(N, C, T * V, true);
-    hipLaunchKernelGGL(gcn_tail_fwd_kernel, row_grid(geo), dim3(EW_THREADS), 0, (hipStream_t)stream,
-                       geo, make_src(*y), make_src(*o), res ? make_src(*res) : null_src(), res ? 1 : 0, C, T * V, g);
-    tamgcn_note_kernel("gcn_tail_fwd_kernel");
-    TG_LAUNCH_CHECK("tamgcn_gcn_tail_fwd");
-    return 0;
+    return gcn_tail_fwd_launch("tamgcn_gcn_tail_fwd", y, o, res, N, C, T, V, g, nullptr, stream);
+}
+extern "C" int tamgcn_gcn_tail_fwd_bits(const tamgcn_src* y, const tamgcn_src* o, const tamgcn_src* res,
+                                        int N, int C, int T, int V, float* g, unsigned char* bits, void* stream) {
+    TG_CHECK(bits, "tamgcn_gcn_tail_fwd_bits: no sign-bit output (use tamgcn_gcn_tail_fwd)");
+    return gcn_tail_fwd_launch("tamgcn_gcn_tail_fwd_bits", y, o, res, N, C, T, V, g, bits, stream);
 }
 
 extern "C" int tamgcn_gcn_tail_bwd(const float* dg, const float* g, const tamgcn_src* o, const float* o_save,
@@ -589,9 +656,22 @@
     TG_CHECK(dg && g && o && o->x1 && o_save && dsum && doz && part && grid_ok(N, C), "tamgcn_gcn_tail_bwd: bad args");
     const RowGeo geo = row_geo(N, C, T * V, true);
     hipLaunchKernelGGL(gcn_tail_bwd_kernel, row_grid(geo), dim3(EW_THREADS), 0, (hipStream_t)stream,
-                       geo, dg, g, make_src(*o), o_save, C, T * V, N, dsum, doz, part);
+                       geo, dg, g, (const unsigned char*)nullptr, make_src(*o), o_save, C, T * V, N, dsum, doz, part);
     tamgcn_note_kernel("gcn_tail_bwd_kernel");
     TG_LAUNCH_CHECK("tamgcn_gcn_tail_bwd");
+    return 0;
+}
+
+extern "C" int tamgcn_gcn_tail_bwd_bits(const float* dg, const unsigned char* bits, const tamgcn_src* o, const float* o_save,
+                                        int N, int C, int T, int V, float* dsum, float* doz, float* part, void* stream) {
+    TG_CHECK(dg && o && o->x1 && o_save && doz && part && grid_ok(N, C), "tamgcn_gcn_tail_bwd_bits: bad args");
+    TG_CHECK((bits != nullptr) == (dsum != nullptr),
+             "tamgcn_gcn_tail_bwd_bits: sign bits and dsum go together (both: dg is masked here; neither: dg is dsum already)");
+    const RowGeo geo = row_geo(N, C, T * V, true);
+    hipLaunchKernelGGL(gcn_tail_bwd_kernel, row_grid(geo), dim3(EW_THREADS), 0, (hipStream_t)stream,
+                       geo, dg, (const float*)nullptr, bits, make_src(*o), o_save, C, T * V, N, dsum, doz, part);
+    tamgcn_note_kernel("gcn_tail_bwd_kernel");
+    TG_LAUNCH_CHECK("tamgcn_gcn_tail_bwd_bits");
     return 0;
 }
 
@@ -669,26 +749,35 @@
     return 0;
 }
 
-extern "C" int tamgcn_add_act_fwd(const tamgcn_src* a, const tamgcn_src* res, int relu,
-                                  int N, int C, int T, int V, float* out, float* rowmean, float* xbar, void* stream) {
-    TG_CHECK(a && a->x1 && out && grid_ok(N, C), "tamgcn_add_act_fwd: bad args");
+static int add_act_fwd_launch(const char* who, const tamgcn_src* a, const tamgcn_src* res, int relu,
+                              int N, int C, int T, int V, float* out, float* rowmean, float* xbar, unsigned char* bits, void* stream) {
+    TG_CHECK(a && a->x1 && out && grid_ok(N, C), "%s: bad args", who);
     if (xbar) {
         TG_CHECK(!rowmean && (V & 3) == 0 && V <= 64, "tamgcn_add_act_fwd: the frame-mean output needs V %% 4 == 0, V <= 64 and no row-mean output");
         const bool al16 = (((uintptr_t)a->x1 | (uintptr_t)(a->x2 ? a->x2 : a->x1) | (uintptr_t)out | (uintptr_t)xbar |
                             (uintptr_t)(res ? res->x1 : a->x1) | (uintptr_t)((res && res->x2) ? res->x2 : a->x1)) & 15) == 0;
         TG_CHECK(al16, "tamgcn_add_act_fwd: the frame-mean form needs 16-byte aligned operands");
         hipLaunchKernelGGL(add_act_fwd_tmean_kernel, dim3((unsigned)ceil_div(N * C, EW_THREADS / 64)), dim3(EW_THREADS), 0, (hipStream_t)stream,
-                           make_src(*a), res ? make_src(*res) : null_src(), res ? 1 : 0, relu, N, C, T, V, out, xbar);
+                           make_src(*a), res ? make_src(*res) : null_src(), res ? 1 : 0, relu, N, C, T, V, out, xbar, bits);
         tamgcn_note_kernel("add_act_fwd_tmean_kernel");
-        TG_LAUNCH_CHECK("tamgcn_add_act_fwd");
+        TG_LAUNCH_CHECK(who);
         return 0;
     }
     const RowGeo geo = row_geo(N, C, T * V, true);
     hipLaunchKernelGGL(add_act_fwd_kernel, row_grid(geo), dim3(EW_THREADS), 0, (hipStream_t)stream,
-                       geo, make_src(*a), res ? make_src(*res) : null_src(), res ? 1 : 0, relu, C, T * V, out, rowmean);
+                       geo, make_src(*a), res ? make_src(*res) : null_src(), res ? 1 : 0, relu, C, T * V, out, rowmean, bits);
     tamgcn_note_kernel("add_act_fwd_kernel");
-    TG_LAUNCH_CHECK("tamgcn_add_act_fwd");
-    return 0;
+    TG_LAUNCH_CHECK(who);
+    return 0;
+}
+extern "C" int tamgcn_add_act_fwd(const tamgcn_src* a, const tamgcn_src* res, int relu,
+                                  int N, int C, int T, int V, float* out, float* rowmean, float* xbar, void* stream) {
+    return add_act_fwd_launch("tamgcn_add_act_fwd", a, res, relu, N, C, T, V, out, rowmean, xbar, nullptr, stream);
+}
+extern "C" int tamgcn_add_act_fwd_bits(const tamgcn_src* a, const tamgcn_src* res,
+                                       int N, int C, int T, int V, float* out, float* rowmean, float* xbar, unsigned char* bits, void* stream) {
+    TG_CHECK(bits, "tamgcn_add_act_fwd_bits: no sign-bit output (use tamgcn_add_act_fwd)");
+    return add_act_fwd_launch("tamgcn_add_act_fwd_bits", a, res, 1, N, C, T, V, out, rowmean, xbar, bits, stream);
 }
 
 extern "C" int tamgcn_add_act_bwd(const float* dout, const float* out, int relu, const float* a_pre, const float* a_save,
@@ -697,9 +786,21 @@
     TG_CHECK(dout && part && grid_ok(N, C) && (!relu || out) && (!a_pre || a_save) && (!r_pre || r_save), "tamgcn_add_act_bwd: bad args");
     const RowGeo geo = row_geo(N, C, T * V, true);
     hipLaunchKernelGGL(add_act_bwd_kernel, row_grid(geo), dim3(EW_THREADS), 0, (hipStream_t)stream,
-                       geo, dout, out, relu, a_pre, a_save, r_pre, r_save, C, T * V, N, dz, part);
+                       geo, dout, out, (const unsigned char*)nullptr, relu, a_pre, a_save, r_pre, r_save, C, T * V, N, dz, part);
     tamgcn_note_kernel("add_act_bwd_kernel");
     TG_LAUNCH_CHECK("tamgcn_add_act_bwd");
+    return 0;
+}
+
+extern "C" int tamgcn_add_act_bwd_bits(const float* dout, const unsigned char* bits, const float* a_pre, const float* a_save,
+                                       const float* r_pre, const float* r_save,
+                                       int N, int C, int T, int V, float* dz, float* part, void* stream) {
+    TG_CHECK(dout && bits && part && grid_ok(N, C) && (!a_pre || a_save) && (!r_pre || r_save), "tamgcn_add_act_bwd_bits: bad args");
+    const RowGeo geo = row_geo(N, C, T * V, true);
+    hipLaunchKernelGGL(add_act_bwd_kernel, row_grid(geo), dim3(EW_THREADS), 0, (hipStream_t)stream,
+                       geo, dout, (const float*)nullptr, bits, 1, a_pre, a_save, r_pre, r_save, C, T * V, N, dz, part);
+    tamgcn_note_kernel("add_act_bwd_kernel");
+    TG_LAUNCH_CHECK("tamgcn_add_act_bwd_bits");
     return 0;
 }
 
diff --git a/tam_gcn_amd/functional.py b/tam_gcn_amd/functional.py
--- a/tam_gcn_amd/functional.py
+++ b/tam_gcn_amd/functional.py
@@ -250,21 +250,22 @@
     else:
         coef_o, save_o = _coef(Cout, x)
         P.bno.fwd(opart, 0, count, training, coef_o, save_o, 0)
-    g = ops.gcn_tail_fwd(S(y_pre, coef=coef_y), S(o_pre, coef=coef_o), res)
+    sign = [] if save and ops.SIGNBITS else None
+    g = ops.gcn_tail_fwd(S(y_pre, coef=coef_y), S(o_pre, coef=coef_o), res, sign=sign)
     sv = None
     if save:
         sv = dict(x=x, xbar=xbar, pq=pq, x3=x3, E=E, y_pre=y_pre, d_pre=d_pre, o_pre=o_pre, g=g, coef_y=coef_y, save_y=save_y,
                   coef_d=coef_d, save_d=save_d, coef_o=coef_o, save_o=save_o, coef_diff=coef_diff,
-                  training=training)
+                  training=training, gbits=sign[0] if sign else None)
     return g, sv
 
 
-def gcn_backward(P, sv, dg, need_dx=True, extra_dx=None):
+def gcn_backward(P, sv, dg, need_dx=True, extra_dx=None, dg_masked=False):
     with ops.ReduceBatch():
-        return _gcn_backward(P, sv, dg, need_dx, extra_dx)
-
-
-def _gcn_backward(P, sv, dg, need_dx=True, extra_dx=None):
+        return _gcn_backward(P, sv, dg, need_dx, extra_dx, dg_masked)
+
+
+def _gcn_backward(P, sv, dg, need_dx=True, extra_dx=None, dg_masked=False):
     x, xbar, pq, y_pre, d_pre, o_pre, g = sv['x'], sv['xbar'], sv['pq'], sv['y_pre'], sv['d_pre'], sv['o_pre'], sv['g']
     training = sv['training']
     N, Cin, T, V = x.shape
@@ -273,7 +274,13 @@
     G = {}
     fk = Fork(x.device, 2)
     fk.__enter__()
-    dsum, doz, part_o = ops.gcn_tail_bwd(dg, g, S(o_pre, coef=sv['coef_o']), sv['save_o'])
+    gbits = sv.get('gbits')
+    if dg_masked:
+        dsum, doz, part_o = ops.gcn_tail_bwd_bits(dg, None, S(o_pre, coef=sv['coef_o']), sv['save_o'])
+    elif gbits is not None:
+        dsum, doz, part_o = ops.gcn_tail_bwd_bits(dg, gbits, S(o_pre, coef=sv['coef_o']), sv['save_o'])
+    else:
+        dsum, doz, part_o = ops.gcn_tail_bwd(dg, g, S(o_pre, coef=sv['coef_o']), sv['save_o'])
     coefb_o = torch.empty(3, Cout, device=x.device)
     G['bno.w'], G['bno.b'], G['bo'] = P.bno.bwd(part_o, 0, count, sv['save_o'], 0, training, coefb_o, 0, want_dbias=True)
     gyo = S(doz, o_pre, coefb_o)
@@ -419,19 +426,20 @@
         res = None
     fk.__exit__()
     bo.flush()
+    sign = [] if save and ops.SIGNBITS and P.relu else None
     if pool is not None:
-        out, rm = ops.add_act_fwd(S(cat_pre, coef=coef_c), res, P.relu, Cout, rowmean=True)
+        out, rm = ops.add_act_fwd(S(cat_pre, coef=coef_c), res, P.relu, Cout, rowmean=True, sign=sign)
         pool.append(rm)
     else:
         if training or save:
-            out, xb = ops.add_act_fwd(S(cat_pre, coef=coef_c), res, P.relu, Cout, xbar=True)
+            out, xb = ops.add_act_fwd(S(cat_pre, coef=coef_c), res, P.relu, Cout, xbar=True, sign=sign)
             attach_xbar(out, xb)
         else:
-            out = ops.add_act_fwd(S(cat_pre, coef=coef_c), res, P.relu, Cout)
+            out = ops.add_act_fwd(S(cat_pre, coef=coef_c), res, P.relu, Cout, sign=sign)
     sv = None
     if save:
         sv = dict(g=g, xres=xres, h_pre=h_pre, cat_pre=cat_pre, r_pre=r_pre, out=out, coef_h=coef_h, save_h=save_h,
-                  coef_c=coef_c, save_c=save_c, coef_r=coef_r, save_r=save_r, training=training)
+                  coef_c=coef_c, save_c=save_c, coef_r=coef_r, save_r=save_r, training=training, obits=sign[0] if sign else None)
     return out, sv
 
 
@@ -476,12 +484,18 @@
     return out
 
 
-def tcn_backward(P, sv, dout, need_dg=True, need_dxres=True):
+def signmask_route(stride, have_bits, N, Cb, Cin, T, V, split_mode=0):
+    if not have_bits:
+        return None
+    return 'a' if stride == 1 and ops.signmask_shape_ok(N, Cb, Cin, T, V, split_mode) else 'b'
+
+
+def tcn_backward(P, sv, dout, need_dg=True, need_dxres=True, dg_sign=None, route=None):
     with ops.ReduceBatch():
-        return _tcn_backward(P, sv, dout, need_dg, need_dxres)
-
-
-def _tcn_backward(P, sv, dout, need_dg=True, need_dxres=True):
+        return _tcn_backward(P, sv, dout, need_dg, need_dxres, dg_sign, route)
+
+
+def _tcn_backward(P, sv, dout, need_dg=True, need_dxres=True, dg_sign=None, route=None):
     g, xres, h_pre, cat_pre, r_pre, out = sv['g'], sv['xres'], sv['h_pre'], sv['cat_pre'], sv['r_pre'], sv['out']
     training = sv['training']
     N, Cin, T, V = g.shape
@@ -492,7 +506,10 @@
     G = {}
     fk = Fork(g.device, 2)
     fk.__enter__()
-    dz, part = ops.add_act_bwd(dout, out, P.relu, cat_pre, sv['save_c'], r_pre, sv['save_r'], want_dz=bool(P.relu))
+    if sv.get('obits') is not None:
+        dz, part = ops.add_act_bwd_bits(dout, sv['obits'], cat_pre, sv['save_c'], r_pre, sv['save_r'], want_dz=True)
+    else:
+        dz, part = ops.add_act_bwd(dout, out, P.relu, cat_pre, sv['save_c'], r_pre, sv['save_r'], want_dz=bool(P.relu))
     if dz is None:
         dz = dout
     coefb_c = torch.empty(3, Cout, device=g.device)
@@ -580,7 +597,12 @@
     dg = None
     if need_dg:
         dg, _ = ops.conv(gyh, K=Ch, w=P.Win, bias=None, M=Cin, wmode=1)
-        ops.conv(gcat((nb + 1) * Cb), K=Cb, w=P.Wl, bias=None, M=Cin, wmode=1, y=dg, T_out=T2, ostride=s, add1=dg)
+        masked = signmask_route(s, dg_sign is not None, N, Cb, Cin, T, V, ops._lib_().tamgcn_get_split_mode()) == 'a' and \
+            ops.signmask_supported((dz, cat_pre, P.Wl, dg, dg_sign), N, Cb, Cin, T, V)
+        ops.conv(gcat((nb + 1) * Cb), K=Cb, w=P.Wl, bias=None, M=Cin, wmode=1, y=dg, T_out=T2, ostride=s, add1=dg,
+                 sign=dg_sign if masked else None)
+        if route is not None:
+            route['dg_masked'] = masked
     dxres = None
     if P.rmode == 'identity':
         dxres = dz
@@ -675,9 +697,11 @@
     @staticmethod
     def backward(ctx, dout, _drm=None):
         need_dx = ctx.needs_input_grad[1]
-        dg, dxres, Gt = tcn_backward(ctx.Pt, ctx.svt, dout.contiguous(), need_dg=True, need_dxres=need_dx)
+        route = {}
+        dg, dxres, Gt = tcn_backward(ctx.Pt, ctx.svt, dout.contiguous(), need_dg=True, need_dxres=need_dx,
+                                     dg_sign=ctx.svg.get('gbits'), route=route)
         ctx.svt = None
-        dx, Gg = gcn_backward(ctx.Pg, ctx.svg, dg, need_dx=need_dx, extra_dx=dxres)
+        dx, Gg = gcn_backward(ctx.Pg, ctx.svg, dg, need_dx=need_dx, extra_dx=dxres, dg_masked=route.get('dg_masked', False))
         ctx.svg = None
         return (None, dx, None, None) + tuple(ctx.mod.gcn1._route(Gg)) + tuple(ctx.mod._route_tcn(Gt))
 
diff --git a/tam_gcn_amd/ops.py b/tam_gcn_amd/ops.py
--- a/tam_gcn_amd/ops.py
+++ b/tam_gcn_amd/ops.py
@@ -19,7 +19,7 @@
         return None
     if not (t.is_cuda and t.is_contiguous()):
         raise RuntimeError('tam_gcn_amd: expected a contiguous HIP (cuda) tensor; there is no CPU path')
-    if t.dtype not in (torch.float32, torch.int64, torch.int32, torch.float64):
+    if t.dtype not in (torch.float32, torch.int64, torch.int32, torch.float64, torch.uint8):
         raise RuntimeError(f'tam_gcn_amd: unsupported dtype {t.dtype}')
     return t.data_ptr()
 
@@ -87,7 +87,7 @@
 def conv(src, K, w, bias, M, KT=1, dil=1, stride=1, pad=0, wmode=0, up=1,
          y=None, ycoff=0, T_out=None, T_y=None, ostride=1, add1=None, add2=None,
          bcast=None, bcast_scale=0.0, mask=None, aux=None, aux_center=None, auxcoff=0, stats=False,
-         post_coef=None, post_act=0):
+         post_coef=None, post_act=0, sign=None, sign_coff=0):
     if src.x1.shape[-1] % 4:
         src = S(with_slack(src.x1), with_slack(src.x2), src.coef, src.coff, src.act)
     x = src.x1
@@ -102,7 +102,7 @@
         T_y = y.shape[2]
     per_clip = max(x.shape[1] * T_in * V, y.shape[1] * T_y * V)
     if N > 1 and N * per_clip > CHUNK_ELEMS:
-        if stats or mask is not None or aux is not None:
+        if stats or mask is not None or aux is not None or sign is not None:
             raise RuntimeError('tam_gcn_amd: a convolution over >= 2^31 elements cannot carry BatchNorm moments / a mask')
         for n0, n1 in n_chunks(N, per_clip):
             conv(_slice_src(src, n0, n1), K, w, bias, M, KT, dil, stride, pad, wmode, up, y=y[n0:n1], ycoff=ycoff, T_out=T_out,
@@ -136,8 +136,32 @@
             raise RuntimeError('tamgcn_conv: no tiling for this shape')
         part = empty(2, y.shape[1], nparts, like=x)
         d.stats_part, d.stats_ctot, d.stats_coff = _ptr(part), y.shape[1], ycoff
-    _lib.check(lib.tamgcn_conv(C.byref(d), _stream()), 'tamgcn_conv')
+    if sign is not None:
+        _lib.check(lib.tamgcn_conv_signmask(C.byref(d), _ptr(sign), sign.shape[1], sign_coff, _stream()), 'tamgcn_conv_signmask')
+    else:
+        _lib.check(lib.tamgcn_conv(C.byref(d), _stream()), 'tamgcn_conv')
     return y, part
+
+
+SIGNBITS = os.environ.get('TAMGCN_SIGNBITS', '1') != '0'
+
+
+def sign_empty(N, C_, T, V, like):
+    return torch.empty(N, C_, (T * V + 3) // 4, device=like.device, dtype=torch.uint8)
+
+
+def signmask_shape_ok(N, K, M, T, V, split_mode=0):
+    if V % 4 or V > 32 or T * V < 64 or K % 16 or M % 16 or K > 512 or M > 512 or N * max(K, M) * T * V > CHUNK_ELEMS:
+        return False
+    if os.environ.get('TAMGCN_CONV_WAVES', '8') == '4':
+        return False
+    return split_mode == 0 or M < 128
+
+
+def signmask_supported(tensors, N, K, M, T, V):
+    if not signmask_shape_ok(N, K, M, T, V, _lib_().tamgcn_get_split_mode()):
+        return False
+    return all(t is None or (t.is_cuda and t.is_contiguous() and t.data_ptr() % 16 == 0) for t in tensors)
 
 
 TCN_PAIR = os.environ.get('TAMGCN_TCN_PAIR', '1') != '0'
@@ -659,12 +683,18 @@
     return dx3, db3, dA, dw4, db4, dal, dpq
 
 
-def gcn_tail_fwd(y, o, res):
+def gcn_tail_fwd(y, o, res, sign=None):
     N, _, T, V = y.x1.shape
     Cc = y.ctot
     g = empty(N, Cc, T, V, like=y.x1)
     yc, oc = y.c(), o.c()
     rc = res.c() if res is not None else None
+    if sign is not None:
+        bits = sign_empty(N, Cc, T, V, g)
+        _lib.check(_lib_().tamgcn_gcn_tail_fwd_bits(C.byref(yc), C.byref(oc), C.byref(rc) if rc is not None else None,
+                                                    N, Cc, T, V, _ptr(g), _ptr(bits), _stream()), 'tamgcn_gcn_tail_fwd_bits')
+        sign.append(bits)
+        return g
     _lib.check(_lib_().tamgcn_gcn_tail_fwd(C.byref(yc), C.byref(oc), C.byref(rc) if rc is not None else None,
                                            N, Cc, T, V, _ptr(g), _stream()), 'tamgcn_gcn_tail_fwd')
     return g
@@ -680,6 +710,17 @@
     return dsum, doz, part
 
 
+def gcn_tail_bwd_bits(dg, bits, o, o_save):
+    N, Cc, T, V = dg.shape
+    dsum = empty_like(dg) if bits is not None else None
+    doz = empty_like(dg)
+    part = empty(2, Cc, N, like=dg)
+    oc = o.c()
+    _lib.check(_lib_().tamgcn_gcn_tail_bwd_bits(_ptr(dg), _ptr(bits), C.byref(oc), _ptr(o_save), N, Cc, T, V, _ptr(dsum), _ptr(doz),
+                                                _ptr(part), _stream()), 'tamgcn_gcn_tail_bwd_bits')
+    return (dsum if bits is not None else dg), doz, part
+
+
 def gcn_mid_bwd(dsum, ddiff, y_pre, y_save, r_pre, r_save, want_dres):
     N, Cc, T, V = dsum.shape
     dyb = empty_like(dsum)
@@ -720,7 +761,7 @@
 XBAR_FOLD = os.environ.get('TAMGCN_XBAR_FOLD', '1') != '0'
 
 
-def add_act_fwd(a, res, relu, C_, rowmean=False, xbar=False):
+def add_act_fwd(a, res, relu, C_, rowmean=False, xbar=False, sign=None):
     N, _, T, V = a.x1.shape
     out = empty(N, C_, T, V, like=a.x1)
     rm = torch.empty(N, C_, device=out.device, dtype=torch.float32) if rowmean else None
@@ -729,8 +770,14 @@
         xb = empty(C_, N, V, like=a.x1)
     ac = a.c()
     rc = res.c() if res is not None else None
-    _lib.check(_lib_().tamgcn_add_act_fwd(C.byref(ac), C.byref(rc) if rc is not None else None, int(relu),
-                                          N, C_, T, V, _ptr(out), _ptr(rm), _ptr(xb), _stream()), 'tamgcn_add_act_fwd')
+    if sign is not None and relu:
+        bits = sign_empty(N, C_, T, V, out)
+        _lib.check(_lib_().tamgcn_add_act_fwd_bits(C.byref(ac), C.byref(rc) if rc is not None else None,
+                                                   N, C_, T, V, _ptr(out), _ptr(rm), _ptr(xb), _ptr(bits), _stream()), 'tamgcn_add_act_fwd_bits')
+        sign.append(bits)
+    else:
+        _lib.check(_lib_().tamgcn_add_act_fwd(C.byref(ac), C.byref(rc) if rc is not None else None, int(relu),
+                                              N, C_, T, V, _ptr(out), _ptr(rm), _ptr(xb), _stream()), 'tamgcn_add_act_fwd')
     if xbar:
         return out, xb
     return (out, rm) if rowmean else out
@@ -742,6 +789,15 @@
     part = empty(4 if r_pre is not None else 2, Cc, N, like=dout)
     _lib.check(_lib_().tamgcn_add_act_bwd(_ptr(dout), _ptr(out), int(relu), _ptr(a_pre), _ptr(a_save), _ptr(r_pre), _ptr(r_save), N, Cc, T, V,
                                           _ptr(dz), _ptr(part), _stream()), 'tamgcn_add_act_bwd')
+    return dz, part
+
+
+def add_act_bwd_bits(dout, bits, a_pre, a_save, r_pre, r_save, want_dz):
+    N, Cc, T, V = dout.shape
+    dz = empty_like(dout) if want_dz else None
+    part = empty(4 if r_pre is not None else 2, Cc, N, like=dout)
+    _lib.check(_lib_().tamgcn_add_act_bwd_bits(_ptr(dout), _ptr(bits), _ptr(a_pre), _ptr(a_save), _ptr(r_pre), _ptr(r_save), N, Cc, T, V,
+                                               _ptr(dz), _ptr(part), _stream()), 'tamgcn_add_act_bwd_bits')
     return dz, part
 
 
```
